# chenxuhao/GraphAIBench

Measured on AMD Instinct MI355X. Metric: GCN-layer fwd+bwd aggregated edges/sec, higher is better.
Workload: dtype f32; 1 GPU; ogbn-products-shaped Chung-Lu graph (seed 42), GCN hidden layer 128->128 fwd+bwd (2 SpMM D=128 + 3 dense products + relu/d_relu; 2 of the products ride on the SpMMs); nv=2449029, ne_with_selfloops=125915443, D=128, parallelism=1 GPU

## Files before the change

graphaibench_amd/build.py:

```python
from __future__ import annotations

import os
import shutil
import subprocess
import sys
from pathlib import Path

ROOT = Path(__file__).resolve().parent.parent
PKG = ROOT / "graphaibench_amd"
CSRC = PKG / "csrc"
HOST = PKG / "host"
LIB = PKG / "lib"
INCLUDE = ROOT / "include"
ORACLE = ROOT / "oracle"
REFERENCE = Path("/root/reference")

HIP_SOURCES = ["runtime.hip", "graph.hip", "spmm.hip", "spmm_part.hip", "spmm_gemm_bf16.hip", "gat.hip", "sgemm.hip", "sgemm_skinny.hip", "elementwise.hip", "probe.hip", "comm.hip"]
HIPCC_FLAGS = [
    "--offload-arch=gfx950",
    "-O3",
    "-std=c++17",
    "-fPIC",
    "-ffp-contract=off",
    "-Wall",
    "-Wno-unused-function",
    "-Werror=pass-failed",
]


def _hipcc() -> str:
    for cand in (os.environ.get("HIPCC"), shutil.which("hipcc"), "/opt/rocm/bin/hipcc"):
        if cand and Path(cand).exists():
            return cand
    raise RuntimeError("hipcc not found (need ROCm at /opt/rocm)")


def _run(cmd, cwd=None):
    print("+", " ".join(str(c) for c in cmd), flush=True)
    subprocess.run([str(c) for c in cmd], cwd=cwd, check=True)


def _stale(target: Path, deps) -> bool:
    if not target.exists():
        return True
    t = target.stat().st_mtime
    return any(Path(d).stat().st_mtime > t for d in deps)


def build_hip(force: bool = False) -> Path:
    LIB.mkdir(exist_ok=True)
    out = LIB / "libgaib_hip.so"
    hipcc = _hipcc()
    headers = [CSRC / "common.h", CSRC / "spmm_core.h", CSRC / "spmm_kernels.h", INCLUDE / "gaib.h"]
    objs, jobs = [], []
    for src in HIP_SOURCES:
        s = CSRC / src
        o = LIB / (src + ".o")
        if force or _stale(o, [s, *headers]):
            jobs.append([hipcc, *HIPCC_FLAGS, f"-I{INCLUDE}", f"-I{CSRC}", "-c", s, "-o", o])
        objs.append(o)
    if jobs:
        from concurrent.futures import ThreadPoolExecutor

        with ThreadPoolExecutor(max_workers=min(4, len(jobs))) as pool:
            list(pool.map(_run, jobs))
    if force or _stale(out, objs):
        _run([hipcc, "--offload-arch=gfx950", "-shared", "-fPIC", *objs, "-o", out])
    return out


def build_host(force: bool = False) -> Path | None:
    srcs = sorted(p for p in HOST.glob("*.cpp") if p.name != "train_main.cpp")
    if not srcs:
        return None
    out = LIB / "libgaib_gnn.so"
    hdrs = list(INCLUDE.rglob("*.h")) + list(INCLUDE.rglob("*.hh"))
    if force or _stale(out, [*srcs, *hdrs, LIB / "libgaib_hip.so"]):
        _run(["g++", "-O2", "-std=c++17", "-fPIC", "-shared", "-fopenmp", "-Wall",
              f"-I{INCLUDE}", f"-I{INCLUDE}/gnn", f"-I{INCLUDE}/layers", f"-I{INCLUDE}/utils",
              *srcs, f"-L{LIB}", "-lgaib_hip", "-Wl,-rpath,$ORIGIN", "-o", out])
    build_drivers(force)
    return out


def build_drivers(force: bool = False) -> None:
    bindir = ROOT / "bin"
    bindir.mkdir(exist_ok=True)
    src = HOST / "train_main.cpp"
    hdrs = list(INCLUDE.rglob("*.h")) + list(INCLUDE.rglob("*.hh"))
    for name, flag in (("gcn", None), ("sage", "-DUSE_SAGE"), ("gat", "-DUSE_GAT")):
        exe = bindir / f"gpu_train_{name}"
        if force or _stale(exe, [src, *hdrs, LIB / "libgaib_gnn.so"]):
            cmd = ["g++", "-O2", "-std=c++17", "-fopenmp", "-Wall", f"-I{INCLUDE}", f"-I{INCLUDE}/gnn",
                   f"-I{INCLUDE}/layers", f"-I{INCLUDE}/utils", src, f"-L{LIB}", "-lgaib_gnn", "-lgaib_hip",
                   "-Wl,-rpath,$ORIGIN/../graphaibench_amd/lib", "-o", exe]
            if flag:
                cmd.insert(1, flag)
            _run(cmd)


# ... 24 lines not shown
```

graphaibench_amd/capi.py:

```python
from __future__ import annotations

import ctypes as C
from pathlib import Path

LIB_DIR = Path(__file__).resolve().parent / "lib"
LIB_PATH = LIB_DIR / "libgaib_hip.so"

W_GCN, W_MEAN, W_MEAN_T, W_EDGE, W_EDGE_T = 0, 1, 2, 3, 4

_vp, _i, _i64, _f, _u64 = C.c_void_p, C.c_int, C.c_int64, C.c_float, C.c_uint64
_pp = C.POINTER(C.c_void_p)

SIGNATURES = {
    "gaib_last_error": (C.c_char_p, []),
    "gaib_version": (C.c_char_p, []),
    "gaib_ctx_create": (_i, [_i, _vp, _pp]),
    "gaib_ctx_destroy": (_i, [_vp]),
    "gaib_ctx_set_stream": (_i, [_vp, _vp]),
    "gaib_ctx_own_stream": (_i, [_vp]),
    "gaib_sync": (_i, [_vp]),
    "gaib_capture_begin": (_i, [_vp]),
    "gaib_capture_end": (_i, [_vp, _pp]),
    "gaib_capture_abort": (_i, [_vp]),
    "gaib_exec_launch": (_i, [_vp, _vp]),
    "gaib_exec_nodes": (_i64, [_vp]),
    "gaib_exec_elapsed_ms": (_i, [_vp, _vp]),
    "gaib_exec_destroy": (_i, [_vp]),
    "gaib_host_alloc": (_i, [_vp, C.c_size_t, _pp]),
    "gaib_host_free": (_i, [_vp, _vp]),
    "gaib_memcpy_d2h_async": (_i, [_vp, _vp, _vp, C.c_size_t]),
    "gaib_masked_avg_loss_dev": (_i, [_vp, _i64, _i64, _vp, _vp, _vp]),
    "gaib_masked_accuracy_single_dev": (_i, [_vp, _i64, _i64, _i, _vp, _vp, _vp, _vp]),
    "gaib_masked_f1_counts_dev": (_i, [_vp, _i64, _i64, _i, _vp, _vp, _vp, _vp]),
    "gaib_adam_step_dev": (_i, [_vp, _i64, _vp, _vp, _vp, _vp, _f, _f, _f, _f, _vp]),
    "gaib_side_begin": (_i, [_vp]),
    "gaib_side_end": (_i, [_vp]),
    "gaib_side_wait": (_i, [_vp]),
    "gaib_malloc": (_i, [_vp, C.c_size_t, _pp]),
    "gaib_free": (_i, [_vp, _vp]),
    "gaib_memcpy_h2d": (_i, [_vp, _vp, _vp, C.c_size_t]),
    "gaib_memcpy_d2h": (_i, [_vp, _vp, _vp, C.c_size_t]),
    "gaib_memcpy_d2d": (_i, [_vp, _vp, _vp, C.c_size_t]),
    "gaib_fill_f32": (_i, [_vp, _i64, _f, _vp]),
    "gaib_scale_f32": (_i, [_vp, _i64, _f, _vp]),
    "gaib_cast_f32_bf16": (_i, [_vp, _i64, _vp, _vp]),
    "gaib_cast_bf16_f32": (_i, [_vp, _i64, _vp, _vp]),
    "gaib_graph_create": (_i, [_vp, _i64, _i64, _vp, _i, _vp, _i, _pp]),
    "gaib_graph_create_rect": (_i, [_vp, _i64, _i64, _i64, _vp, _i, _vp, _i, _pp]),
    "gaib_graph_destroy": (_i, [_vp]),
    "gaib_graph_add_selfloop": (_i, [_vp, _vp, _pp]),
    "gaib_graph_nv": (_i64, [_vp]),
    "gaib_graph_ne": (_i64, [_vp]),
    "gaib_graph_nc": (_i64, [_vp]),
    "gaib_graph_rowptr": (_vp, [_vp]),
    "gaib_graph_colidx": (_vp, [_vp]),
    "gaib_graph_compute_vertex_data": (_i, [_vp, _vp]),
    "gaib_graph_vertex_data": (_vp, [_vp]),
    "gaib_graph_compute_edge_data": (_i, [_vp, _vp]),
    "gaib_graph_edge_data": (_vp, [_vp]),
    "gaib_graph_set_vertex_norm": (_i, [_vp, _vp, _vp, _vp, _vp, _vp]),
    "gaib_graph_device_bytes": (_i64, [_vp]),
    "gaib_spmm": (_i, [_vp, _vp, _i, _vp, _i, _vp, _vp]),
    "gaib_spmm_acc": (_i, [_vp, _vp, _i, _vp, _i, _vp, _vp]),
    "gaib_spmm_ex": (_i, [_vp, _vp, _i, _vp, _i, _vp, _vp, _i]),
    "gaib_spmm_gemm": (_i, [_vp, _vp, _i, _vp, _i, _vp, _vp, _vp, _i, _i, _vp, _i]),
    "gaib_spmm_gemm2": (_i, [_vp, _vp, _i, _vp, _i, _vp, _vp, _vp, _i, _vp, _vp, _i, _vp, _i]),
    "gaib_spmm_mh": (_i, [_vp, _vp, _i, _vp, _i, _i, _vp, _vp, _i]),
    "gaib_spmm_bf16": (_i, [_vp, _vp, _i, _vp, _i, _vp, _vp, _i]),
    "gaib_spmm_gemm_bf16": (_i, [_vp, _vp, _i, _vp, _i, _vp, _vp, _vp, _i, _i, _vp, _i]),
    "gaib_spmm_gemm2_bf16": (_i, [_vp, _vp, _i, _vp, _i, _vp, _vp, _vp, _i, _vp, _vp, _i, _vp, _i]),
    "gaib_graph_split_classes": (_i, [_vp, _vp, _vp, _pp, _pp, _pp, _pp, C.POINTER(_i64), C.POINTER(_i64), _i]),
    "gaib_graph_split_pieces": (_i, [_vp, _vp, _i, _i, C.POINTER(_i64), C.POINTER(_i64), C.POINTER(_i), _pp]),
    "gaib_graph_set_row_map": (_i, [_vp, _vp, _vp, _i64]),
    "gaib_graph_row_map": (_vp, [_vp]),
    "gaib_spmm_2t": (_i, [_vp, _vp, _i, _vp, _i, _vp, _vp, _i64, _vp, _i]),
    "gaib_spmm_gemm_2t": (_i, [_vp, _vp, _i, _vp, _i, _vp, _vp, _i64, _vp, _vp, _i, _vp, _vp, _i, _vp, _i]),
    "gaib_spmm_gemm_fusable": (_i, [_vp, _i, _i, _i, _i]),
    "gaib_gat_scores_mh": (_i, [_vp, _vp, _i, _i, _vp, _vp, _vp, _f, _vp, _vp, _vp]),
    "gaib_sddmm_mh": (_i, [_vp, _vp, _i, _i, _vp, _vp, _vp]),
    "gaib_gat_softmax_bwd_alpha_mh": (_i, [_vp, _vp, _i, _i, _vp, _vp, _vp, _vp, _f, _vp, _vp, _vp]),
    "gaib_gat_softmax_bwd_alpha_ex": (_i, [_vp, _vp, _i, _i, _vp, _vp, _vp, _vp, _f, _vp, _vp, _vp, _vp, _vp, _vp]),
    "gaib_gat_softmax_bwd_alpha_re": (_i, [_vp, _vp, _i, _i, _vp, _vp, _vp, _vp, _vp, _f, _vp, _vp, _vp, _vp, _vp, _vp]),
    "gaib_gat_softmax_bwd_rows": (_i, [_vp, _vp, _i, _vp, _vp, _vp, _f, _vp, _vp]),
    "gaib_edge_gather_perm": (_i, [_vp, _i64, _i, _vp, _vp, _vp]),
    "gaib_edge_rowsum": (_i, [_vp, _vp, _i, _vp, _vp]),
    "gaib_gat_alpha_grads": (_i, [_vp, _i64, _i, _i, _vp, _vp, _vp, _vp, _vp]),
    "gaib_gat_backward_fused": (_i, [_vp, _vp, _i, _i, _vp, _vp, _vp, _vp, _vp, _vp, _vp, _f, _vp, _vp, _vp]),
    "gaib_gat_forward_fused": (_i, [_vp, _vp, _i, _i, _vp, _vp, _vp, _f, _i, _vp, _vp]),
    "gaib_edge_transpose_mh": (_i, [_vp, _vp, _i, _vp, _vp]),
    "gaib_gat_scores": (_i, [_vp, _vp, _i, _vp, _vp, _vp, _f, _vp, _vp, _vp]),
    "gaib_sddmm": (_i, [_vp, _vp, _i, _vp, _vp, _vp]),
    "gaib_gat_softmax_bwd_alpha": (_i, [_vp, _vp, _i, _vp, _vp, _vp, _vp, _f, _vp, _vp, _vp]),
    "gaib_edge_transpose": (_i, [_vp, _vp, _vp, _vp]),
    "gaib_sgemm": (_i, [_vp, _i, _i, _i64, _i64, _i64, _vp, _vp, _i, _vp]),
    "gaib_sgemm_drelu": (_i, [_vp, _i64, _i64, _i64, _vp, _vp, _vp, _i, _vp]),
    "gaib_sgemm_ex": (_i, [_vp, _i, _i, _i64, _i64, _i64, _vp, _vp, _i, _vp]),
    "gaib_bias_add": (_i, [_vp, _i64, _i, _vp, _vp]),
    "gaib_colsum": (_i, [_vp, _i64, _i, _vp, _vp]),
    "gaib_rng_uniform": (_i, [_vp, _i64, _f, _f, _u64, _vp]),
    "gaib_csr2csc": (_i, [_vp, _i, _i, _i, _vp, _vp, _vp, _vp, _vp, _vp]),
    "gaib_relu": (_i, [_vp, _i64, _vp, _vp]),
    "gaib_d_relu": (_i, [_vp, _i64, _vp, _vp, _vp]),
    "gaib_dropout": (_i, [_vp, _i64, _f, _f, _u64, _vp, _vp, _vp]),
    "gaib_d_dropout": (_i, [_vp, _i64, _f, _vp, _vp, _vp]),
    "gaib_softmax_xent": (_i, [_vp, _i, _i64, _i64, _vp, _vp, _vp, _vp, _vp]),
    "gaib_d_softmax_xent": (_i, [_vp, _i, _i64, _i64, _vp, _vp, _vp, _vp]),
    "gaib_sigmoid_xent": (_i, [_vp, _i, _i64, _i64, _vp, _vp, _vp, _vp, _vp]),
    "gaib_d_sigmoid_xent": (_i, [_vp, _i, _i64, _i64, _vp, _vp, _vp, _vp]),
    "gaib_masked_f1_micro": (_i, [_vp, _i64, _i64, _i, _vp, _vp, _vp, C.POINTER(_f), C.POINTER(_i64)]),
    "gaib_masked_avg_loss": (_i, [_vp, _i64, _i64, _vp, _vp, C.POINTER(_f)]),
    "gaib_masked_accuracy_single": (_i, [_vp, _i64, _i64, _i, _vp, _vp, _vp, C.POINTER(_f)]),
    "gaib_l2norm": (_i, [_vp, _i64, _i, _vp, _vp]),
    "gaib_d_l2norm": (_i, [_vp, _i64, _i, _vp, _vp, _vp]),
    "gaib_adam_step": (_i, [_vp, _i64, _vp, _vp, _vp, _vp, _f, _f, _f, _f, _f, _f]),
    "gaib_gather_rows": (_i, [_vp, _i64, _vp, _i, _vp, _vp]),
    "gaib_prof_enable": (_i, [_vp, _i]),
    "gaib_prof_reset": (_i, [_vp]),
    "gaib_prof_get": (_i, [_vp, C.c_char_p, C.POINTER(_i64), C.POINTER(C.c_double)]),
    "gaib_prof_get_work": (_i, [_vp, C.c_char_p, C.POINTER(_i64), C.POINTER(C.c_double), C.POINTER(C.c_double),
                                C.POINTER(C.c_double), C.POINTER(C.c_double)]),
    "gaib_prof_table": (_i, [_vp, C.c_char_p, C.c_size_t, C.POINTER(C.c_size_t)]),
    "gaib_gat_score_signs": (_i, [_vp, _vp, _i, _i, _vp, _vp, _vp, _vp]),
    "gaib_gat_forward_fused_rect": (_i, [_vp, _vp, _i, _i, _vp, _vp, _vp, C.c_float, _i, _vp, _vp, _i]),
    "gaib_gat_backward_rec": (_i, [_vp, _i64, _i, _i, _vp, _vp, _vp, _vp]),
    "gaib_gat_backward_fused_rect": (_i, [_vp, _vp, _i, _i, _vp, _vp, _vp, _vp, _vp, C.c_float, _vp, _vp, _vp, _i]),
    "gaib_gather_scatter_rows": (_i, [_vp, _i64, _vp, _vp, _i, _vp, _vp]),
    "gaib_graph_reorder": (_i, [_vp, _vp, _i, _pp, _vp, _vp]),
    "gaib_graph_sort_rows": (_i, [_vp, _vp]),
    "gaib_graph_locality": (_i, [_vp, _vp, C.POINTER(C.c_float)]),
    "gaib_graph_stats": (_i, [_vp, _vp, C.POINTER(_i64), C.POINTER(_i64), C.POINTER(_i64)]),
    "gaib_set_option": (_i, [_vp, C.c_char_p, _i64]),
    "gaib_get_option": (_i, [_vp, C.c_char_p, C.POINTER(_i64)]),
    "gaib_device_count": (_i, [C.POINTER(_i)]),
    "gaib_comm_transport_available": (_i, [_i]),
    "gaib_comm_unique_id": (_i, [_i, _vp]),
    "gaib_comm_init": (_i, [_vp, _i, _i, _vp, _i, _pp]),
    "gaib_comm_destroy": (_i, [_vp]),
    "gaib_comm_rank": (_i, [_vp]),
    "gaib_comm_size": (_i, [_vp]),
    "gaib_comm_barrier": (_i, [_vp]),
    "gaib_allreduce_f32": (_i, [_vp, _vp, _i64]),
    "gaib_allreduce_host_f64": (_i, [_vp, C.POINTER(C.c_double), _i]),
    "gaib_halo_create": (_i, [_vp, C.POINTER(_i64), _vp, _i, C.POINTER(_i64), _pp]),
    "gaib_halo_destroy": (_i, [_vp]),
    "gaib_halo_rows": (_i64, [_vp]),
    "gaib_halo_send_rows": (_i64, [_vp]),
    "gaib_halo_bytes_sent": (_i64, [_vp]),
    "gaib_halo_send_stats": (_i, [_vp, C.POINTER(_i64), C.POINTER(_i64), C.POINTER(_i)]),
    "gaib_halo_link_rows": (_i64, [_vp]),
    "gaib_halo_exchange_begin": (_i, [_vp, _i, _vp]),
    "gaib_halo_exchange_end": (_i, [_vp, _pp]),
# ... 279 lines not shown
        _check(load().gaib_probe_stream_copy(self.h, nbytes, iters, C.byref(v)), "gaib_probe_stream_copy")
        return v.value

    def graph_stats(self, g: "Graph"):
        a, b, c = _i64(), _i64(), _i64()
        _check(self.lib.gaib_graph_stats(self.h, g.h, C.byref(a), C.byref(b), C.byref(c)), "gaib_graph_stats")
        return dict(n_heavy=a.value, heavy_edges=b.value, max_degree=c.value)

    def graph(self, rowptr, colidx, ncols: int | None = None) -> "Graph":
        return Graph(self, rowptr, colidx, ncols)

    def spmm(self, g: "Graph", kind: int, x, out, edge_w=None, accumulate: bool = False, relu: bool = False,
             heads: int = 1):
        assert x.is_contiguous() and out.is_contiguous() and x.dim() == 2
        flags = (1 if accumulate else 0) | (2 if relu else 0)
        _check(self.lib.gaib_spmm_mh(self.h, g.h, kind, _ptr(edge_w), heads, x.shape[1], _ptr(x), _ptr(out), flags),
               "gaib_spmm")
        return out

    def cast_f32_bf16(self, x, out=None):
        import torch

        assert x.is_contiguous() and x.dtype == torch.float32
        if out is None:
            out = torch.empty(x.shape, dtype=torch.bfloat16, device=x.device)
        assert out.is_contiguous() and out.dtype == torch.bfloat16 and out.numel() == x.numel()
        _check(self.lib.gaib_cast_f32_bf16(self.h, x.numel(), _ptr(x), _ptr(out)), "gaib_cast_f32_bf16")
        return out

    def cast_bf16_f32(self, x, out=None):
        import torch

        assert x.is_contiguous() and x.dtype == torch.bfloat16
        if out is None:
            out = torch.empty(x.shape, dtype=torch.float32, device=x.device)
        assert out.is_contiguous() and out.dtype == torch.float32 and out.numel() == x.numel()
        _check(self.lib.gaib_cast_bf16_f32(self.h, x.numel(), _ptr(x), _ptr(out)), "gaib_cast_bf16_f32")
        return out

    def spmm_bf16(self, g: "Graph", kind: int, x, out, edge_w=None, accumulate: bool = False, relu: bool = False):
        import torch

        assert x.is_contiguous() and out.is_contiguous() and x.dim() == 2 and x.dtype == torch.bfloat16
        flags = (1 if accumulate else 0) | (2 if relu else 0)
        _check(self.lib.gaib_spmm_bf16(self.h, g.h, kind, _ptr(edge_w), x.shape[1], _ptr(x), _ptr(out), flags),
               "gaib_spmm_bf16")
        return out

    def spmm_gemm(self, g: "Graph", kind: int, x, agg, W, out, transW: bool = False, relu: bool = False,
                  agg_scratch: bool = False, edge_w=None, accumulate: bool = False, rows2=None, W2=None):
        assert x.is_contiguous() and agg.is_contiguous() and W.is_contiguous() and out.is_contiguous()
        len_in, len_out = agg.shape[1], out.shape[1]
        assert tuple(W.shape) == ((len_out, len_in) if transW else (len_in, len_out))
        flags = (2 if relu else 0) | (4 if agg_scratch else 0) | (1 if accumulate else 0)
        if rows2 is not None:
            assert rows2.is_contiguous() and W2.is_contiguous() and W2.shape == W.shape and rows2.shape[1] == len_in
            _check(self.lib.gaib_spmm_gemm2(self.h, g.h, kind, _ptr(edge_w), len_in, _ptr(x), _ptr(agg), _ptr(W),
                                            1 if transW else 0, _ptr(rows2), _ptr(W2), len_out, _ptr(out), flags),
                   "gaib_spmm_gemm2")
            return out
        _check(self.lib.gaib_spmm_gemm(self.h, g.h, kind, _ptr(edge_w), len_in, _ptr(x), _ptr(agg), _ptr(W),
                                       1 if transW else 0, len_out, _ptr(out), flags), "gaib_spmm_gemm")
        return out

    def spmm_gemm_bf16(self, g: "Graph", kind: int, x, agg, W, out, transW: bool = False, relu: bool = False,
                       agg_scratch: bool = False, edge_w=None, accumulate: bool = False, rows2=None, W2=None):
        import torch

        assert x.is_contiguous() and agg.is_contiguous() and W.is_contiguous() and out.is_contiguous()
        assert x.dtype == torch.bfloat16 and agg.dtype == torch.float32 and out.dtype == torch.float32
        len_in, len_out = agg.shape[1], out.shape[1]
        assert tuple(W.shape) == ((len_out, len_in) if transW else (len_in, len_out))
        flags = (2 if relu else 0) | (4 if agg_scratch else 0) | (1 if accumulate else 0)
        if rows2 is not None:
            assert rows2.is_contiguous() and W2.is_contiguous() and W2.shape == W.shape and rows2.shape[1] == len_in
            _check(self.lib.gaib_spmm_gemm2_bf16(self.h, g.h, kind, _ptr(edge_w), len_in, _ptr(x), _ptr(agg), _ptr(W),
                                                 1 if transW else 0, _ptr(rows2), _ptr(W2), len_out, _ptr(out), flags),
                   "gaib_spmm_gemm2_bf16")
            return out
        _check(self.lib.gaib_spmm_gemm_bf16(self.h, g.h, kind, _ptr(edge_w), len_in, _ptr(x), _ptr(agg), _ptr(W),
                                            1 if transW else 0, len_out, _ptr(out), flags), "gaib_spmm_gemm_bf16")
        return out

    def spmm_2t(self, g: "Graph", kind: int, x, x2, n_first: int, out, edge_w=None, accumulate: bool = False,
                relu: bool = False):
        assert x.is_contiguous() and out.is_contiguous() and (x2 is None or x2.is_contiguous())
        flags = (1 if accumulate else 0) | (2 if relu else 0)
        _check(self.lib.gaib_spmm_2t(self.h, g.h, kind, _ptr(edge_w), x.shape[1], _ptr(x), _ptr(x2), n_first, _ptr(out),
                                     flags), "gaib_spmm_2t")
        return out

    def spmm_gemm_2t(self, g: "Graph", kind: int, x, x2, n_first: int, agg, W, out, transW: bool = False,
                     relu: bool = False, agg_scratch: bool = False, edge_w=None, accumulate: bool = False, rows2=None,
                     W2=None):
        len_in, len_out = agg.shape[1], out.shape[1]
        flags = (2 if relu else 0) | (4 if agg_scratch else 0) | (1 if accumulate else 0)
        _check(self.lib.gaib_spmm_gemm_2t(self.h, g.h, kind, _ptr(edge_w), len_in, _ptr(x), _ptr(x2), n_first, _ptr(agg),
                                          _ptr(W), 1 if transW else 0, _ptr(rows2), _ptr(W2), len_out, _ptr(out), flags),
               "gaib_spmm_gemm_2t")
        return out

    def spmm_gemm_fusable(self, kind: int, len_in: int, len_out: int, dual: bool = False) -> bool:
        return bool(self.lib.gaib_spmm_gemm_fusable(self.h, kind, len_in, len_out, int(dual)))

    def split_classes(self, g_own: "Graph", g_halo: "Graph", interior=True, bnd_own=True, bnd_halo=True, bnd_full=True,
                      all_boundary: bool = False):
        hs = [C.c_void_p() for _ in range(4)]
        want = [interior, bnd_own, bnd_halo, bnd_full]
        nb, be = _i64(), _i64()
        _check(self.lib.gaib_graph_split_classes(self.h, g_own.h, g_halo.h, *[C.byref(h) if w else None for h, w in zip(hs, want)],
                                                 C.byref(nb), C.byref(be), int(all_boundary)), "gaib_graph_split_classes")
        out = {k: (Graph(self, _handle=h) if w else None)
               for k, h, w in zip(("interior", "bnd_own", "bnd_halo", "bnd_full"), hs, want)}
        out["n_boundary"], out["boundary_edges"] = nb.value, be.value
        return out

    def split_pieces(self, g: "Graph", n_pieces: int, ranges):
        nr = len(ranges)
        b = (C.c_int64 * max(nr, 1))(*[int(r[0]) for r in ranges])
        e = (C.c_int64 * max(nr, 1))(*[int(r[1]) for r in ranges])
        pc = (C.c_int * max(nr, 1))(*[int(r[2]) for r in ranges])
        hs = (C.c_void_p * n_pieces)()
        _check(self.lib.gaib_graph_split_pieces(self.h, g.h, n_pieces, nr, b, e, pc, hs), "gaib_graph_split_pieces")
        return [Graph(self, _handle=C.c_void_p(hs[k])) for k in range(n_pieces)]

    def gat_scores(self, g, h, alpha_l, alpha_r, temp, scores, norm, eps: float = 0.2, heads: int = 1):
        _check(self.lib.gaib_gat_scores_mh(self.h, g.h, h.shape[1], heads, _ptr(h), _ptr(alpha_l), _ptr(alpha_r),
                                           eps, _ptr(temp), _ptr(scores), _ptr(norm)), "gaib_gat_scores")

    def gat_score_signs(self, g, h, alpha_l, alpha_r, heads: int = 1):
        import torch

        out = torch.empty(g.ne, heads, dtype=torch.uint8, device=h.device)
        _check(self.lib.gaib_gat_score_signs(self.h, g.h, h.shape[1], heads, _ptr(h), _ptr(alpha_l), _ptr(alpha_r), _ptr(out)),
               "gaib_gat_score_signs")
        return out

    def sddmm(self, g, grad, feat, out_e, heads: int = 1):
        _check(self.lib.gaib_sddmm_mh(self.h, g.h, grad.shape[1], heads, _ptr(grad), _ptr(feat), _ptr(out_e)),
               "gaib_sddmm")

    def gat_softmax_bwd_alpha(self, g, feat, norm, norm_grad, temp, scores, lgrad, rgrad, eps: float = 0.2,
                              heads: int = 1, grad_rows=None, fwd_out_rows=None, norm_t=None, alpha=None):
        if temp is None:
            _check(self.lib.gaib_gat_softmax_bwd_alpha_re(self.h, g.h, feat.shape[1], heads, _ptr(feat), _ptr(alpha[0]),
                                                          _ptr(alpha[1]), _ptr(norm), _ptr(norm_grad), eps, _ptr(scores),
                                                          _ptr(lgrad), _ptr(rgrad), _ptr(grad_rows),
                                                          _ptr(fwd_out_rows), _ptr(norm_t)), "gaib_gat_softmax_bwd_alpha_re")
            return
        _check(self.lib.gaib_gat_softmax_bwd_alpha_ex(self.h, g.h, feat.shape[1], heads, _ptr(feat), _ptr(norm),
                                                      _ptr(norm_grad), _ptr(temp), eps, _ptr(scores),
                                                      _ptr(lgrad), _ptr(rgrad), _ptr(grad_rows),
                                                      _ptr(fwd_out_rows), _ptr(norm_t)), "gaib_gat_softmax_bwd_alpha")

    def gat_forward_fused(self, g, h, alpha_l, alpha_r, out, row_stats, eps: float = 0.2, heads: int = 1,
                          relu: bool = False) -> bool:
        rc = self.lib.gaib_gat_forward_fused(self.h, g.h, h.shape[1], heads, _ptr(h), _ptr(alpha_l), _ptr(alpha_r), eps,
                                             int(relu), _ptr(out), _ptr(row_stats))
        if rc == -5:
            return False
        _check(rc, "gaib_gat_forward_fused")
        return True

    def gat_backward_fused(self, g, feat, grad, fwd_out, alpha_l, alpha_r, norm, grad_out, lgrad, rgrad, eps: float = 0.2,
                           heads: int = 1, row_stats=None) -> bool:
        rc = self.lib.gaib_gat_backward_fused(self.h, g.h, feat.shape[1], heads, _ptr(feat), _ptr(grad), _ptr(fwd_out),
# ... 247 lines not shown
```

graphaibench_amd/csrc/common.h:

```cpp
#pragma once
#include <hip/hip_runtime.h>
#include <stdint.h>
#include <stdio.h>
#include <string>
#include <string.h>
#include <vector>
#include "gaib.h"

#define GAIB_WAVE 64

void gaib_set_error(const char* fmt, ...);

#define GAIB_HIP(call)                                                                    \
  do {                                                                                    \
    hipError_t e_ = (call);                                                               \
    if (e_ != hipSuccess) {                                                               \
      gaib_set_error("%s:%d: %s -> %s", __FILE__, __LINE__, #call, hipGetErrorString(e_)); \
      return GAIB_ERR_HIP;                                                                \
    }                                                                                     \
  } while (0)

#define GAIB_CHECK(cond, ...)       \
  do {                              \
    if (!(cond)) {                  \
      gaib_set_error(__VA_ARGS__);  \
      return GAIB_ERR_INVALID;      \
    }                               \
  } while (0)

#define GAIB_TRY(call)         \
  do {                         \
    int rc_ = (call);          \
    if (rc_ != GAIB_OK) return rc_; \
  } while (0)

#define GAIB_LAUNCH_CHECK() GAIB_HIP(hipGetLastError())

#define GAIB_NOT_WHILE_CAPTURING(ctx, what)                                                                        \
  GAIB_CHECK(!(ctx)->capturing, "%s inside gaib_capture_begin/end: it waits for the stream or allocates -- run the " \
                                "sequence once before capturing it (buffers and lazily built tables then exist)", what)


#define GAIB_FLAT_RING_DEFAULT 1
#define GAIB_BF16_FUSE_U 32

struct gaib_ctx {
  int device;
  hipStream_t stream;
  int num_cus;
  void* ws;
  size_t ws_bytes;
  void* pad;
  size_t pad_bytes;
  hipStream_t main_stream, side_stream;
  hipEvent_t ev_fork, ev_join;
  void* ws_side;
  size_t ws_side_bytes;
  int forked;
  int spmm_heavy_threshold;
  int spmm_variant;
  int spmm_xcd_swizzle;
  int spmm_chunked;
  int spmm_pad;
  int spmm_fuse;
  int spmm_flat;
  int spmm_flat_ring;
  int comm_reserve_cus;
  int comm_reserve_default;
  int spmm_fuse_cus;
  int spmm_tile_xcd;
  int spmm_prefetch_ids;
  int spmm_unroll;
  int spmm_addr_mode;
  int spmm_gather_mode;
  int spmm_hot_bytes;
  int spmm_bf16_layout;
  int spmm_bf16_fuse_u;
  int agg_bf16;
  int sgemm_variant;
  int gat_fast;
  int gat_chunk_colsum;
  int gat_chunk_sort;
  int gat_row_waves;
  int gat_fused_bwd;
  int gat_fused_fwd;
  int gat_fused_unroll;
  int gat_bwd_pk;
  int gat_interleave;
  int gat_chunk_xcd;
  int graph_rev_search;
  hipStream_t owned_stream;
  int capturing;
  int live_execs;
  std::vector<void*> retired;
  int prof_on;
  struct ProfRec { const char* key; hipEvent_t a, b; double bytes, flops; char tag[28]; };
  std::vector<ProfRec> prof;
};

static inline int gaib_comm_reserve(const gaib_ctx* ctx) {
  const int r = ctx->comm_reserve_cus >= 0 ? ctx->comm_reserve_cus : ctx->comm_reserve_default;
  const int cap = ctx->num_cus > 64 ? ctx->num_cus - 64 : 0;
  return r < 0 ? 0 : (r > cap ? cap : r);
}

constexpr double GAIB_HBM_PEAK_BPS = 8.0e12;
constexpr double GAIB_MFMA_F32_PEAK_FLOPS = 157.3e12;
static inline double gaib_alg_spmm_bytes(double edges, double rows, double cols, double w_bytes_per_edge, double stored,
                                         double elem_bytes = 4.0) {
  return edges * (elem_bytes * cols + 4.0 + w_bytes_per_edge) + stored * rows * 4.0 * cols + (rows + 1.0) * 8.0;
}

struct ProfScope {
  gaib_ctx* c;
  size_t idx;
  ProfScope(gaib_ctx* ctx, const char* key, double bytes = 0.0, double flops = 0.0, int cols = 0, const char* tag = nullptr)
      : c(ctx), idx((size_t)-1) {
    if (!c->prof_on || c->capturing) return;
    gaib_ctx::ProfRec r;
    r.key = key;
    r.bytes = bytes;
    r.flops = flops;
    r.tag[0] = 0;
    if (tag) snprintf(r.tag, sizeof(r.tag), "%s", tag);
    else if (cols > 0) snprintf(r.tag, sizeof(r.tag), "%d", cols);
    if (hipEventCreate(&r.a) != hipSuccess || hipEventCreate(&r.b) != hipSuccess) return;
    (void)hipEventRecord(r.a, c->stream);
    c->prof.push_back(r);
    idx = c->prof.size() - 1;
  }
  ~ProfScope() {
    if (idx != (size_t)-1) (void)hipEventRecord(c->prof[idx].b, c->stream);
  }
};

int gaib_ws_reserve(gaib_ctx* ctx, size_t bytes);
int gaib_pad_reserve(gaib_ctx* ctx, size_t bytes);

struct gaib_graph {
  int device;
  int64_t nv, ne;
  int64_t nc;
  int64_t* rowptr;
  uint32_t* colidx;
  float* vdata;
  float* edata;
  float* inv_deg;
  float* col_vdata;
  float* col_inv_deg;
  float* w_gcn;
  float* w_mean_t;
  uint32_t* rev;
  uint32_t* chunk_row;
  uint32_t* chunk_ebase;
  uint32_t* chunk_start;
  int64_t n_chunks;
  uint32_t* colidx_flagged;
  int64_t hot_threshold;
  int64_t hot_rows;
  uint32_t* heavy_rows;
// ... 66 lines not shown
```

graphaibench_amd/csrc/elementwise.hip:

```cpp
#include "common.h"

namespace {

typedef float f4 __attribute__((ext_vector_type(4)));

inline unsigned stream_grid(int64_t n_items, int block) {
  int64_t b = cdiv64(n_items > 0 ? n_items : 1, block);
  return (unsigned)(b < 2048 ? b : 2048);
}

__global__ void fill_kernel(int64_t n, float v, float* x) {
  const int64_t stride = (int64_t)gridDim.x * blockDim.x;
  for (int64_t i = (int64_t)blockIdx.x * blockDim.x + threadIdx.x; i < n; i += stride) x[i] = v;
}

__global__ void scale_kernel(int64_t n, float a, float* x) {
  const int64_t stride = (int64_t)gridDim.x * blockDim.x;
  for (int64_t i = (int64_t)blockIdx.x * blockDim.x + threadIdx.x; i < n; i += stride) x[i] = a * x[i];
}

__global__ void relu_kernel(int64_t n, const float* in, float* out, int vec_ok) {
  const int64_t stride = (int64_t)gridDim.x * blockDim.x;
  const int64_t tid = (int64_t)blockIdx.x * blockDim.x + threadIdx.x;
  if (vec_ok) {
    const int64_t n4 = n >> 2;
    for (int64_t i = tid; i < n4; i += stride) {
      f4 v = reinterpret_cast<const f4*>(in)[i];
#pragma unroll
      for (int k = 0; k < 4; ++k) v[k] = v[k] > 0.f ? v[k] : 0.f;
      reinterpret_cast<f4*>(out)[i] = v;
    }
    for (int64_t i = (n4 << 2) + tid; i < n; i += stride) out[i] = in[i] > 0.f ? in[i] : 0.f;
  } else {
    for (int64_t i = tid; i < n; i += stride) out[i] = in[i] > 0.f ? in[i] : 0.f;
  }
}

__global__ void d_relu_kernel(int64_t n, const float* in, const float* data, float* out, int vec_ok) {
  const int64_t stride = (int64_t)gridDim.x * blockDim.x;
  const int64_t tid = (int64_t)blockIdx.x * blockDim.x + threadIdx.x;
  if (vec_ok) {
    const int64_t n4 = n >> 2;
    for (int64_t i = tid; i < n4; i += stride) {
      f4 g = reinterpret_cast<const f4*>(in)[i];
      f4 d = reinterpret_cast<const f4*>(data)[i];
#pragma unroll
      for (int k = 0; k < 4; ++k) g[k] = d[k] > 0.f ? g[k] : 0.f;
      reinterpret_cast<f4*>(out)[i] = g;
    }
    for (int64_t i = (n4 << 2) + tid; i < n; i += stride) out[i] = data[i] > 0.f ? in[i] : 0.f;
  } else {
    for (int64_t i = tid; i < n; i += stride) out[i] = data[i] > 0.f ? in[i] : 0.f;
  }
}

__device__ __forceinline__ float u01(uint64_t seed, uint64_t i) {
  uint64_t z = seed + 0x9E3779B97F4A7C15ull * (i + 1);
  z = (z ^ (z >> 30)) * 0xBF58476D1CE4E5B9ull;
  z = (z ^ (z >> 27)) * 0x94D049BB133111EBull;
  z = z ^ (z >> 31);
  return (float)(z >> 40) * (1.0f / 16777216.0f);
}
__global__ void dropout_kernel(int64_t n, float scale, float rate, uint64_t seed, const float* in,
                               uint8_t* masks, float* out) {
  const int64_t stride = (int64_t)gridDim.x * blockDim.x;
  for (int64_t i = (int64_t)blockIdx.x * blockDim.x + threadIdx.x; i < n; i += stride) {
    uint8_t m = u01(seed, (uint64_t)i) > rate ? 1 : 0;
    masks[i] = m;
    out[i] = in[i] * (float)m * scale;
  }
}
__global__ void d_dropout_kernel(int64_t n, float scale, const float* in, const uint8_t* masks,
                                 float* out) {
  const int64_t stride = (int64_t)gridDim.x * blockDim.x;
  for (int64_t i = (int64_t)blockIdx.x * blockDim.x + threadIdx.x; i < n; i += stride)
    out[i] = in[i] * (float)masks[i] * scale;
}

__global__ __launch_bounds__(256) void softmax_xent_kernel(int num_cls, int64_t begin, int64_t end,
                                                           const float* in, const uint8_t* masks,
                                                           const uint8_t* labels, float* loss,
                                                           float* out) {
// ... 329 lines not shown
  a[j] = s;
}
__global__ void rng_uniform_kernel(int64_t n, float a, float range, uint64_t seed, float* r) {
  const int64_t stride = (int64_t)gridDim.x * blockDim.x;
  for (int64_t i = (int64_t)blockIdx.x * blockDim.x + threadIdx.x; i < n; i += stride) r[i] = a + range * u01(seed, (uint64_t)i);
}

__global__ void adam_dev_kernel(int64_t n, const float* dW, float* W, float* m, float* v, float alpha, float b1,
                                float b2, const float* pw, float eps) {
  const float b1_t = pw[0], b2_t = pw[1];
  const int64_t stride = (int64_t)gridDim.x * blockDim.x;
  for (int64_t i = (int64_t)blockIdx.x * blockDim.x + threadIdx.x; i < n; i += stride) {
    const float g = dW[i];
    const float mt = b1 * m[i] + (1.0f - b1) * g;
    const float vt = b2 * v[i] + (1.0f - b2) * g * g;
    m[i] = mt;
    v[i] = vt;
    W[i] -= alpha * (mt / (1.0f - b1_t)) / sqrtf((vt / (1.0f - b2_t)) + eps);
  }
}
__global__ void adam_advance_kernel(float* pw, float b1, float b2) {
  pw[0] *= b1;
  pw[1] *= b2;
}

__device__ __forceinline__ unsigned f32_to_bf16_bits(float f) {
  const unsigned u = __float_as_uint(f);
  if ((u & 0x7fffffffu) > 0x7f800000u) return (u >> 16) | 0x0040u;
  return (u + 0x7fffu + ((u >> 16) & 1u)) >> 16;
}
typedef unsigned u4v __attribute__((ext_vector_type(4)));
__global__ __launch_bounds__(256) void cast_f32_bf16_kernel(int64_t n, const float* __restrict__ in, uint16_t* __restrict__ out,
                                                            int vec) {
  const int64_t n8 = vec ? n / 8 : 0;
  const int64_t stride = (int64_t)gridDim.x * blockDim.x;
  for (int64_t i = (int64_t)blockIdx.x * blockDim.x + threadIdx.x; i <= n8; i += stride) {
    if (i < n8) {
      const f4 a = reinterpret_cast<const f4*>(in)[2 * i], b = reinterpret_cast<const f4*>(in)[2 * i + 1];
      u4v o;
      o[0] = f32_to_bf16_bits(a[0]) | (f32_to_bf16_bits(a[1]) << 16);
      o[1] = f32_to_bf16_bits(a[2]) | (f32_to_bf16_bits(a[3]) << 16);
      o[2] = f32_to_bf16_bits(b[0]) | (f32_to_bf16_bits(b[1]) << 16);
      o[3] = f32_to_bf16_bits(b[2]) | (f32_to_bf16_bits(b[3]) << 16);
      reinterpret_cast<u4v*>(out)[i] = o;
    } else {
      for (int64_t k = 8 * n8; k < n; ++k) out[k] = (uint16_t)f32_to_bf16_bits(in[k]);
    }
  }
}
__global__ __launch_bounds__(256) void cast_f32_bf16_scalar_kernel(int64_t n, const float* __restrict__ in,
                                                                   uint16_t* __restrict__ out) {
  const int64_t stride = (int64_t)gridDim.x * blockDim.x;
  for (int64_t i = (int64_t)blockIdx.x * blockDim.x + threadIdx.x; i < n; i += stride) out[i] = (uint16_t)f32_to_bf16_bits(in[i]);
}
__global__ __launch_bounds__(256) void cast_bf16_f32_scalar_kernel(int64_t n, const uint16_t* __restrict__ in,
                                                                   float* __restrict__ out) {
  const int64_t stride = (int64_t)gridDim.x * blockDim.x;
  for (int64_t i = (int64_t)blockIdx.x * blockDim.x + threadIdx.x; i < n; i += stride) out[i] = __uint_as_float((unsigned)in[i] << 16);
}
__global__ __launch_bounds__(256) void cast_bf16_f32_kernel(int64_t n, const uint16_t* __restrict__ in, float* __restrict__ out,
                                                            int vec) {
  const int64_t n8 = vec ? n / 8 : 0;
  const int64_t stride = (int64_t)gridDim.x * blockDim.x;
  for (int64_t i = (int64_t)blockIdx.x * blockDim.x + threadIdx.x; i <= n8; i += stride) {
    if (i < n8) {
      const u4v w = reinterpret_cast<const u4v*>(in)[i];
      f4 a, b;
      a[0] = __uint_as_float(w[0] << 16);
      a[1] = __uint_as_float(w[0] & 0xffff0000u);
      a[2] = __uint_as_float(w[1] << 16);
      a[3] = __uint_as_float(w[1] & 0xffff0000u);
      b[0] = __uint_as_float(w[2] << 16);
      b[1] = __uint_as_float(w[2] & 0xffff0000u);
      b[2] = __uint_as_float(w[3] << 16);
      b[3] = __uint_as_float(w[3] & 0xffff0000u);
      reinterpret_cast<f4*>(out)[2 * i] = a;
      reinterpret_cast<f4*>(out)[2 * i + 1] = b;
    } else {
      for (int64_t k = 8 * n8; k < n; ++k) out[k] = __uint_as_float((unsigned)in[k] << 16);
    }
  }
}

}

extern "C" int gaib_fill_f32(gaib_ctx* ctx, int64_t n, float value, float* d_x) {
  GAIB_CHECK(ctx && (d_x || n == 0), "gaib_fill_f32: NULL argument");
  if (n <= 0) return GAIB_OK;
  fill_kernel<<<stream_grid(n, 256), 256, 0, ctx->stream>>>(n, value, d_x);
  GAIB_LAUNCH_CHECK();
  return GAIB_OK;
}

extern "C" int gaib_scale_f32(gaib_ctx* ctx, int64_t n, float alpha, float* d_x) {
  GAIB_CHECK(ctx && (d_x || n == 0), "gaib_scale_f32: NULL argument");
  if (n <= 0) return GAIB_OK;
  scale_kernel<<<stream_grid(n, 256), 256, 0, ctx->stream>>>(n, alpha, d_x);
  GAIB_LAUNCH_CHECK();
  return GAIB_OK;
}

extern "C" int gaib_cast_f32_bf16(gaib_ctx* ctx, int64_t n, const float* d_in, uint16_t* d_out) {
  GAIB_CHECK(ctx && ((d_in && d_out) || n == 0), "gaib_cast_f32_bf16: NULL argument");
  GAIB_CHECK(n >= 0, "gaib_cast_f32_bf16: n < 0");
  if (n == 0) return GAIB_OK;
  GAIB_CHECK((const void*)d_in != (const void*)d_out, "gaib_cast_f32_bf16: in and out must not alias");
  const int vec = ((((uintptr_t)d_in | (uintptr_t)d_out) & 15) == 0);
  ProfScope ps(ctx, "cast_f32_bf16", 6.0 * (double)n);
  if (vec) cast_f32_bf16_kernel<<<stream_grid(n / 8 + 1, 256), 256, 0, ctx->stream>>>(n, d_in, d_out, 1);
  else cast_f32_bf16_scalar_kernel<<<stream_grid(n, 256), 256, 0, ctx->stream>>>(n, d_in, d_out);
  GAIB_LAUNCH_CHECK();
  return GAIB_OK;
}

extern "C" int gaib_cast_bf16_f32(gaib_ctx* ctx, int64_t n, const uint16_t* d_in, float* d_out) {
  GAIB_CHECK(ctx && ((d_in && d_out) || n == 0), "gaib_cast_bf16_f32: NULL argument");
  GAIB_CHECK(n >= 0, "gaib_cast_bf16_f32: n < 0");
  if (n == 0) return GAIB_OK;
  GAIB_CHECK((const void*)d_in != (const void*)d_out, "gaib_cast_bf16_f32: in and out must not alias");
  const int vec = ((((uintptr_t)d_in | (uintptr_t)d_out) & 15) == 0);
  ProfScope ps(ctx, "cast_bf16_f32", 6.0 * (double)n);
  if (vec) cast_bf16_f32_kernel<<<stream_grid(n / 8 + 1, 256), 256, 0, ctx->stream>>>(n, d_in, d_out, 1);
  else cast_bf16_f32_scalar_kernel<<<stream_grid(n, 256), 256, 0, ctx->stream>>>(n, d_in, d_out);
  GAIB_LAUNCH_CHECK();
  return GAIB_OK;
}

extern "C" int gaib_relu(gaib_ctx* ctx, int64_t n, const float* d_in, float* d_out) {
  GAIB_CHECK(ctx && ((d_in && d_out) || n == 0), "gaib_relu: NULL argument");
  if (n <= 0) return GAIB_OK;
  const int vec_ok = ((((uintptr_t)d_in | (uintptr_t)d_out) & 15) == 0);
  ProfScope ps(ctx, "relu", 8.0 * (double)n);
  relu_kernel<<<stream_grid(n / 4 + 1, 256), 256, 0, ctx->stream>>>(n, d_in, d_out, vec_ok);
  GAIB_LAUNCH_CHECK();
  return GAIB_OK;
}

extern "C" int gaib_d_relu(gaib_ctx* ctx, int64_t n, const float* d_in_diff, const float* d_data,
                           float* d_out_diff) {
  GAIB_CHECK(ctx && ((d_in_diff && d_data && d_out_diff) || n == 0), "gaib_d_relu: NULL argument");
  if (n <= 0) return GAIB_OK;
  const int vec_ok = ((((uintptr_t)d_in_diff | (uintptr_t)d_data | (uintptr_t)d_out_diff) & 15) == 0);
  ProfScope ps(ctx, "d_relu", 12.0 * (double)n);
  d_relu_kernel<<<stream_grid(n / 4 + 1, 256), 256, 0, ctx->stream>>>(n, d_in_diff, d_data,
                                                                     d_out_diff, vec_ok);
  GAIB_LAUNCH_CHECK();
  return GAIB_OK;
}

extern "C" int gaib_dropout(gaib_ctx* ctx, int64_t n, float scale, float drop_rate, uint64_t seed,
                            const float* d_in, uint8_t* d_masks, float* d_out) {
  GAIB_CHECK(ctx && ((d_in && d_masks && d_out) || n == 0), "gaib_dropout: NULL argument");
  GAIB_CHECK(drop_rate >= 0.f && drop_rate < 1.f, "gaib_dropout: rate must be in [0,1)");
  if (n <= 0) return GAIB_OK;
  dropout_kernel<<<stream_grid(n, 256), 256, 0, ctx->stream>>>(n, scale, drop_rate, seed, d_in,
                                                               d_masks, d_out);
  GAIB_LAUNCH_CHECK();
  return GAIB_OK;
}

extern "C" int gaib_d_dropout(gaib_ctx* ctx, int64_t n, float scale, const float* d_in,
                              const uint8_t* d_masks, float* d_out) {
  GAIB_CHECK(ctx && ((d_in && d_masks && d_out) || n == 0), "gaib_d_dropout: NULL argument");
  if (n <= 0) return GAIB_OK;
  d_dropout_kernel<<<stream_grid(n, 256), 256, 0, ctx->stream>>>(n, scale, d_in, d_masks, d_out);
  GAIB_LAUNCH_CHECK();
  return GAIB_OK;
}

extern "C" int gaib_softmax_xent(gaib_ctx* ctx, int num_cls, int64_t begin, int64_t end,
                                 const float* d_in, const uint8_t* d_masks, const uint8_t* d_labels,
                                 float* d_loss, float* d_out) {
  GAIB_CHECK(ctx && d_in && d_labels && d_loss && d_out, "gaib_softmax_xent: NULL argument");
  GAIB_CHECK(num_cls > 0 && begin >= 0 && end >= begin, "gaib_softmax_xent: bad range");
  if (end == begin) return GAIB_OK;
  softmax_xent_kernel<<<(unsigned)cdiv64(end - begin, 4), 256, 0, ctx->stream>>>(
      num_cls, begin, end, d_in, d_masks, d_labels, d_loss, d_out);
  GAIB_LAUNCH_CHECK();
  return GAIB_OK;
}

extern "C" int gaib_d_softmax_xent(gaib_ctx* ctx, int num_cls, int64_t begin, int64_t end,
                                   const uint8_t* d_masks, const uint8_t* d_labels,
                                   const float* d_out, float* d_diff) {
  GAIB_CHECK(ctx && d_labels && d_out && d_diff, "gaib_d_softmax_xent: NULL argument");
  GAIB_CHECK(num_cls > 0 && begin >= 0 && end >= begin, "gaib_d_softmax_xent: bad range");
  if (end == begin) return GAIB_OK;
  d_softmax_xent_kernel<<<stream_grid((end - begin) * num_cls, 256), 256, 0, ctx->stream>>>(
      num_cls, begin, end, d_masks, d_labels, d_out, d_diff);
  GAIB_LAUNCH_CHECK();
  return GAIB_OK;
}

extern "C" int gaib_sigmoid_xent(gaib_ctx* ctx, int num_cls, int64_t begin, int64_t end,
                                 const float* d_in, const uint8_t* d_masks, const uint8_t* d_labels,
                                 float* d_loss, float* d_out) {
  GAIB_CHECK(ctx && d_in && d_labels && d_loss && d_out, "gaib_sigmoid_xent: NULL argument");
  GAIB_CHECK(num_cls > 0 && begin >= 0 && end >= begin, "gaib_sigmoid_xent: bad range");
  if (end == begin) return GAIB_OK;
  sigmoid_xent_kernel<<<(unsigned)cdiv64(end - begin, 4), 256, 0, ctx->stream>>>(
      num_cls, begin, end, d_in, d_masks, d_labels, d_loss, d_out);
  GAIB_LAUNCH_CHECK();
  return GAIB_OK;
}

extern "C" int gaib_d_sigmoid_xent(gaib_ctx* ctx, int num_cls, int64_t begin, int64_t end,
// ... 247 lines not shown
```

graphaibench_amd/csrc/runtime.hip:

```cpp
#include <algorithm>
#include <stdarg.h>
#include <string.h>
#include <utility>
#include "common.h"
#include <stdlib.h>

static thread_local char g_err[1024] = "";

void gaib_set_error(const char* fmt, ...) {
  va_list ap;
  va_start(ap, fmt);
  vsnprintf(g_err, sizeof(g_err), fmt, ap);
  va_end(ap);
}

extern "C" const char* gaib_last_error(void) { return g_err; }
extern "C" const char* gaib_version(void) { return "graphaibench_amd 0.1 (gfx950)"; }

extern "C" int gaib_device_count(int* h_count) {
  GAIB_CHECK(h_count, "gaib_device_count: h_count is NULL");
  *h_count = 0;
  GAIB_HIP(hipGetDeviceCount(h_count));
  return GAIB_OK;
}

extern "C" int gaib_ctx_create(int device, void* stream, gaib_ctx** out) {
  GAIB_CHECK(out != nullptr, "gaib_ctx_create: out is NULL");
  int ndev = 0;
  GAIB_HIP(hipGetDeviceCount(&ndev));
  GAIB_CHECK(device >= 0 && device < ndev, "gaib_ctx_create: device %d out of range (%d)", device, ndev);
  GAIB_HIP(hipSetDevice(device));
  hipDeviceProp_t prop;
  GAIB_HIP(hipGetDeviceProperties(&prop, device));
  gaib_ctx* c = new gaib_ctx();
  c->device = device;
  c->stream = (hipStream_t)stream;
  c->num_cus = prop.multiProcessorCount;
  c->ws = nullptr;
  c->ws_bytes = 0;
  c->pad = nullptr;
  c->pad_bytes = 0;
  c->main_stream = c->stream;
  c->side_stream = nullptr;
  c->ev_fork = c->ev_join = nullptr;
  c->ws_side = nullptr;
  c->ws_side_bytes = 0;
  c->forked = 0;
  c->spmm_heavy_threshold = 1024;
  c->spmm_variant = 0;
  c->spmm_xcd_swizzle = 2;
  c->spmm_unroll = 0;
  c->spmm_tile_xcd = -1;
  c->spmm_prefetch_ids = 1;
  c->spmm_fuse_cus = 0;
  c->spmm_fuse = 1;
  c->spmm_pad = 1;
  c->spmm_chunked = -1;
  c->spmm_flat = -1;
  c->spmm_addr_mode = 0;
  c->spmm_gather_mode = 0;
  c->spmm_hot_bytes = 3 << 20;
  c->spmm_bf16_layout = 0;
  c->spmm_bf16_fuse_u = 0;
  c->agg_bf16 = 0;
  c->sgemm_variant = 0;
  if (const char* e = getenv("GAIB_SGEMM_VARIANT")) c->sgemm_variant = atoi(e);
  c->gat_fast = 1;
  c->gat_row_waves = 4;
  c->gat_chunk_sort = 1;
  c->gat_chunk_colsum = -1;
  c->graph_rev_search = 0;
  c->gat_fused_bwd = -1;
  c->gat_fused_fwd = -1;
  c->gat_fused_unroll = 4;
  c->spmm_flat_ring = GAIB_FLAT_RING_DEFAULT;
  c->comm_reserve_cus = -1;
  c->comm_reserve_default = 0;
  c->gat_interleave = 0;
  c->gat_bwd_pk = 0;
  c->gat_chunk_xcd = 0;
  c->prof_on = 0;
  c->capturing = 0;
  c->live_execs = 0;
  c->owned_stream = nullptr;
  *out = c;
  return GAIB_OK;
}

extern "C" int gaib_ctx_destroy(gaib_ctx* ctx) {
  if (!ctx) return GAIB_OK;
  GAIB_CHECK(ctx->live_execs == 0, "gaib_ctx_destroy: %d recorded sequence(s) of this context are still alive "
                                   "(gaib_exec_destroy them first: they hold its scratch pointers)", ctx->live_execs);
  (void)hipSetDevice(ctx->device);
  if (ctx->ws) (void)hipFree(ctx->ws);
  if (ctx->pad) (void)hipFree(ctx->pad);
  if (ctx->ws_side) (void)hipFree(ctx->ws_side);
  for (void* p : ctx->retired) (void)hipFree(p);
  if (ctx->side_stream) (void)hipStreamDestroy(ctx->side_stream);
  if (ctx->owned_stream) (void)hipStreamDestroy(ctx->owned_stream);
  if (ctx->ev_fork) (void)hipEventDestroy(ctx->ev_fork);
  if (ctx->ev_join) (void)hipEventDestroy(ctx->ev_join);
  delete ctx;
  return GAIB_OK;
}

extern "C" int gaib_ctx_set_stream(gaib_ctx* ctx, void* stream) {
  GAIB_CHECK(ctx, "gaib_ctx_set_stream: ctx is NULL");
  GAIB_CHECK(!ctx->forked, "gaib_ctx_set_stream: a side section is open");
  ctx->stream = (hipStream_t)stream;
  ctx->main_stream = ctx->stream;
  return GAIB_OK;
}

extern "C" int gaib_ctx_own_stream(gaib_ctx* ctx) {
  GAIB_CHECK(ctx, "gaib_ctx_own_stream: ctx is NULL");
  GAIB_CHECK(!ctx->forked && !ctx->capturing, "gaib_ctx_own_stream: a side section or capture is open");
  if (ctx->owned_stream && ctx->stream == ctx->owned_stream) return GAIB_OK;
  GAIB_HIP(hipSetDevice(ctx->device));
  GAIB_HIP(hipStreamSynchronize(ctx->stream));
  if (!ctx->owned_stream) GAIB_HIP(hipStreamCreateWithFlags(&ctx->owned_stream, hipStreamNonBlocking));
  ctx->stream = ctx->main_stream = ctx->owned_stream;
  return GAIB_OK;
}

extern "C" int gaib_side_begin(gaib_ctx* ctx) {
  GAIB_CHECK(ctx, "gaib_side_begin: ctx is NULL");
  GAIB_CHECK(ctx->forked == 0, "gaib_side_begin: a side section is already open or not waited for");
  GAIB_HIP(hipSetDevice(ctx->device));
  if (!ctx->side_stream) {
    GAIB_HIP(hipStreamCreateWithFlags(&ctx->side_stream, hipStreamNonBlocking));
    GAIB_HIP(hipEventCreateWithFlags(&ctx->ev_fork, hipEventDisableTiming));
    GAIB_HIP(hipEventCreateWithFlags(&ctx->ev_join, hipEventDisableTiming));
  }
  GAIB_HIP(hipEventRecord(ctx->ev_fork, ctx->main_stream));
  GAIB_HIP(hipStreamWaitEvent(ctx->side_stream, ctx->ev_fork, 0));
  ctx->stream = ctx->side_stream;
  std::swap(ctx->ws, ctx->ws_side);
  std::swap(ctx->ws_bytes, ctx->ws_side_bytes);
  ctx->forked = 1;
  return GAIB_OK;
}

extern "C" int gaib_side_end(gaib_ctx* ctx) {
  GAIB_CHECK(ctx, "gaib_side_end: ctx is NULL");
  GAIB_CHECK(ctx->forked == 1, "gaib_side_end: no open side section");
  GAIB_HIP(hipEventRecord(ctx->ev_join, ctx->side_stream));
  ctx->stream = ctx->main_stream;
// ... 268 lines not shown
  int64_t n = 0;
  double ms = 0.0;
  for (auto& r : ctx->prof) {
    if (strcmp(r.key, key) != 0) continue;
    float t = 0.f;
    GAIB_HIP(hipEventElapsedTime(&t, r.a, r.b));
    ms += t;
    n++;
  }
  *h_count = n;
  *h_total_ms = ms;
  return GAIB_OK;
}

extern "C" int gaib_prof_get_work(gaib_ctx* ctx, const char* key, int64_t* h_count, double* h_total_ms, double* h_bytes,
                                  double* h_flops, double* h_roof_ms) {
  GAIB_CHECK(ctx && key && h_count && h_total_ms && h_bytes && h_flops && h_roof_ms, "gaib_prof_get_work: NULL argument");
  GAIB_HIP(hipStreamSynchronize(ctx->stream));
  int64_t n = 0;
  double ms = 0.0, by = 0.0, fl = 0.0, roof = 0.0;
  for (auto& r : ctx->prof) {
    if (strcmp(r.key, key) != 0) continue;
    float t = 0.f;
    GAIB_HIP(hipEventElapsedTime(&t, r.a, r.b));
    ms += t;
    by += r.bytes;
    fl += r.flops;
    roof += 1e3 * std::max(r.bytes / GAIB_HBM_PEAK_BPS, r.flops / GAIB_MFMA_F32_PEAK_FLOPS);
    n++;
  }
  *h_count = n;
  *h_total_ms = ms;
  *h_bytes = by;
  *h_flops = fl;
  *h_roof_ms = roof;
  return GAIB_OK;
}

extern "C" int gaib_prof_table(gaib_ctx* ctx, char* h_buf, size_t cap, size_t* h_needed) {
  GAIB_CHECK(ctx && h_needed && (h_buf || cap == 0), "gaib_prof_table: NULL argument");
  GAIB_HIP(hipStreamSynchronize(ctx->stream));
  struct Row { const char* key; const char* tag; int64_t n; double ms, by, fl, roof; };
  std::vector<Row> rows;
  for (auto& r : ctx->prof) {
    Row* at = nullptr;
    for (auto& q : rows)
      if (strcmp(q.tag, r.tag) == 0 && strcmp(q.key, r.key) == 0) at = &q;
    if (!at) {
      rows.push_back(Row{r.key, r.tag, 0, 0, 0, 0, 0});
      at = &rows.back();
    }
    float t = 0.f;
    GAIB_HIP(hipEventElapsedTime(&t, r.a, r.b));
    at->n++;
    at->ms += t;
    at->by += r.bytes;
    at->fl += r.flops;
    at->roof += 1e3 * std::max(r.bytes / GAIB_HBM_PEAK_BPS, r.flops / GAIB_MFMA_F32_PEAK_FLOPS);
  }
  std::string out;
  char line[320];
  for (auto& q : rows) {
    if (q.tag[0]) snprintf(line, sizeof(line), "%s@%s %lld %.6f %.0f %.0f %.9f\n", q.key, q.tag, (long long)q.n, q.ms, q.by, q.fl, q.roof);
    else snprintf(line, sizeof(line), "%s %lld %.6f %.0f %.0f %.9f\n", q.key, (long long)q.n, q.ms, q.by, q.fl, q.roof);
    out += line;
  }
  *h_needed = out.size() + 1;
  if (cap > 0) {
    const size_t w = out.size() < cap - 1 ? out.size() : cap - 1;
    memcpy(h_buf, out.data(), w);
    h_buf[w] = 0;
  }
  return GAIB_OK;
}

extern "C" int gaib_get_option(gaib_ctx* ctx, const char* key, int64_t* h_value) {
  GAIB_CHECK(ctx && key && h_value, "gaib_get_option: NULL argument");
  if (!strcmp(key, "comm_reserve_cus")) *h_value = gaib_comm_reserve(ctx);
  else if (!strcmp(key, "comm_reserve_cus_raw")) *h_value = ctx->comm_reserve_cus;
  else if (!strcmp(key, "spmm_fuse_cus")) *h_value = ctx->spmm_fuse_cus;
  else if (!strcmp(key, "spmm_flat_ring")) *h_value = ctx->spmm_flat_ring;
  else if (!strcmp(key, "num_cus")) *h_value = ctx->num_cus;
  else if (!strcmp(key, "agg_bf16")) *h_value = ctx->agg_bf16;
  else if (!strcmp(key, "spmm_bf16_layout")) *h_value = ctx->spmm_bf16_layout;
  else if (!strcmp(key, "spmm_bf16_fuse_u")) *h_value = ctx->spmm_bf16_fuse_u;
  else {
    gaib_set_error("gaib_get_option: no readable option '%s'", key);
    return GAIB_ERR_INVALID;
  }
  return GAIB_OK;
}

extern "C" int gaib_set_option(gaib_ctx* ctx, const char* key, int64_t value) {
  GAIB_CHECK(ctx && key, "gaib_set_option: NULL argument");
  if (!strcmp(key, "spmm_heavy_threshold")) {
    GAIB_CHECK(value >= 1 && value <= (1 << 30), "spmm_heavy_threshold out of range");
    ctx->spmm_heavy_threshold = (int)value;
  } else if (!strcmp(key, "spmm_variant"))
    ctx->spmm_variant = (int)value;
  else if (!strcmp(key, "spmm_xcd_swizzle"))
    ctx->spmm_xcd_swizzle = (int)value;
  else if (!strcmp(key, "spmm_fuse"))
    ctx->spmm_fuse = (int)value;
  else if (!strcmp(key, "spmm_chunked"))
    ctx->spmm_chunked = (int)value;
  else if (!strcmp(key, "spmm_pad"))
    ctx->spmm_pad = (int)value;
  else if (!strcmp(key, "spmm_flat"))
    ctx->spmm_flat = (int)value;
  else if (!strcmp(key, "spmm_fuse_cus")) {
    GAIB_CHECK(value >= 0 && value <= ctx->num_cus, "spmm_fuse_cus: 0 (all) .. %d", ctx->num_cus);
    ctx->spmm_fuse_cus = (int)value;
  } else if (!strcmp(key, "spmm_tile_xcd"))
    ctx->spmm_tile_xcd = (int)value;
  else if (!strcmp(key, "spmm_prefetch_ids"))
    ctx->spmm_prefetch_ids = value != 0;
  else if (!strcmp(key, "spmm_unroll"))
    ctx->spmm_unroll = (int)value;
  else if (!strcmp(key, "spmm_addr_mode"))
    ctx->spmm_addr_mode = (int)value;
  else if (!strcmp(key, "spmm_gather_mode"))
    ctx->spmm_gather_mode = (int)value;
  else if (!strcmp(key, "spmm_hot_bytes"))
    ctx->spmm_hot_bytes = (int)value;
  else if (!strcmp(key, "spmm_bf16_layout")) {
    GAIB_CHECK(value == 0 || value == 4 || value == 8, "spmm_bf16_layout must be 0, 4 or 8");
    ctx->spmm_bf16_layout = (int)value;
  } else if (!strcmp(key, "spmm_bf16_fuse_u")) {
    GAIB_CHECK(value == 0 || value == 16 || value == 32, "spmm_bf16_fuse_u must be 0 (default), 16 or 32");
    ctx->spmm_bf16_fuse_u = (int)value;
  } else if (!strcmp(key, "agg_bf16")) {
    GAIB_CHECK(value == 0 || value == 1, "agg_bf16 must be 0 (fp32 tables) or 1 (bf16 tables)");
    ctx->agg_bf16 = (int)value;
  }
  else if (!strcmp(key, "sgemm_variant"))
    ctx->sgemm_variant = (int)value;
  else if (!strcmp(key, "gat_fast"))
    ctx->gat_fast = (int)value;
  else if (!strcmp(key, "gat_chunk_colsum"))
    ctx->gat_chunk_colsum = (int)value;
  else if (!strcmp(key, "gat_chunk_sort"))
    ctx->gat_chunk_sort = (int)value;
  else if (!strcmp(key, "gat_fused_fwd"))
    ctx->gat_fused_fwd = (int)value;
  else if (!strcmp(key, "gat_fused_unroll"))
    ctx->gat_fused_unroll = (int)value;
  else if (!strcmp(key, "comm_reserve_cus"))
    ctx->comm_reserve_cus = value < 0 ? -1 : (int)std::min<int64_t>(value, std::max(0, ctx->num_cus - 64));
  else if (!strcmp(key, "spmm_flat_ring"))
    ctx->spmm_flat_ring = value < 0 ? GAIB_FLAT_RING_DEFAULT : (int)value;
  else if (!strcmp(key, "gat_interleave"))
    ctx->gat_interleave = (int)value;
  else if (!strcmp(key, "gat_bwd_pk"))
    ctx->gat_bwd_pk = (int)value;
  else if (!strcmp(key, "gat_chunk_xcd"))
    ctx->gat_chunk_xcd = (int)value;
  else if (!strcmp(key, "gat_fused_bwd"))
    ctx->gat_fused_bwd = (int)value;
  else if (!strcmp(key, "graph_rev_search"))
    ctx->graph_rev_search = (int)value;
  else if (!strcmp(key, "gat_row_waves")) {
    GAIB_CHECK(value == 1 || value == 2 || value == 4, "gat_row_waves must be 1, 2 or 4");
    ctx->gat_row_waves = (int)value;
  }
  else {
    gaib_set_error("gaib_set_option: unknown key '%s'", key);
    return GAIB_ERR_INVALID;
  }
  return GAIB_OK;
}
```

graphaibench_amd/csrc/spmm.hip:

```cpp
#include <algorithm>
#include "spmm_kernels.h"

namespace {

template <int G, int WMODE, int HT = 0, typename E = float>
__global__ __launch_bounds__(256) void spmm_chunk_kernel(int64_t n_chunks, const uint32_t* chunk_row,
                                                         const uint32_t* chunk_ebase, const uint32_t* chunk_start,
                                                         SpmmArgs a, float* partial) {
  constexpr int U = G < 8 ? G : 8;
  constexpr bool MH = WMODE >= 3;
  constexpr int WS = HT + 1;
  __shared__ float wlds[HT > 0 ? 4 * 64 * WS : 1];
  const int64_t c = (int64_t)blockIdx.x * 4 + (threadIdx.x >> 6);
  if (c >= n_chunks) return;
  const int lane = threadIdx.x & 63;
  const int sl = lane & (G - 1), gbase = lane & ~(G - 1);
  const int64_t row = chunk_row[c];
  const int64_t eb = chunk_ebase[c];
  const int64_t rb = a.rowptr[row];
  const int64_t rem = a.rowptr[row + 1] - eb;
  const int n = rem < 64 ? (int)rem : 64;
  const uint32_t cl = a.col[eb + (lane < n ? lane : 0)];
  float wl = 0.f;
  if (lane < n) {
// ... 174 lines not shown
  a.row_list = nullptr;
  a.row_order = nullptr;
  a.nblocks = 0;
  a.per_xcd = 0;
  a.xcd_chunk = 0;
  a.accumulate = (flags & GAIB_ACCUMULATE) ? 1 : 0;
  a.relu = (flags & GAIB_RELU) ? 1 : 0;
  a.heads = heads;
  a.dh = heads > 0 ? len / heads : len;
  a.col_flagged = nullptr;
  a.compact = 0;
  a.row_map = g->row_map;
  a.in2 = d_in2;
  a.n_first = d_in2 ? (uint32_t)n_first : 0xffffffffu;
  a.in2_bytes = 0;
  if (!part && !bf16 && ctx->spmm_gather_mode == 3 && g->nc == g->nv && !g->col_vdata) {
    GAIB_TRY(gaib_graph_ensure_hot_flags(ctx, g, len));
    a.col_flagged = g->colidx_flagged;
  }
  a.ldo = len;
  {
    const int64_t lp_pad = bf16 ? 0 : pad_stride_floats(ctx, g, len, part);
    if (lp_pad > 0) {
      const int lp = (int)lp_pad;
      GAIB_TRY(gaib_pad_reserve(ctx, (size_t)g->nc * (size_t)lp * 4));
      const int64_t n4 = g->nc * (int64_t)(lp / 4);
      const unsigned grid = (unsigned)std::min<int64_t>(cdiv64(n4, 256), (int64_t)ctx->num_cus * 16);
      pad_rows_kernel<<<grid, 256, 0, ctx->stream>>>(n4, len, lp / 4, d_in, reinterpret_cast<f32x4_t*>(ctx->pad));
      GAIB_LAUNCH_CHECK();
      a.in = reinterpret_cast<const float*>(ctx->pad);
      a.ld = lp;
    }
  }
  const int64_t table_bytes = (d_in2 ? n_first : g->nc) * a.ld * (bf16 ? 2 : 4);
  a.in_bytes = table_bytes < ((int64_t)1 << 32) ? (uint32_t)table_bytes : 0u;
  if (d_in2) {
    const int64_t t2 = (g->nc - n_first) * a.ld * 4;
    a.in2_bytes = t2 < ((int64_t)1 << 32) ? (uint32_t)t2 : 0u;
  }
  switch (weight_kind) {
    case GAIB_W_GCN:
      GAIB_TRY(gaib_graph_ensure_w_gcn(ctx, g));
      a.ew = g->w_gcn;
      *wmode = 1;
      return GAIB_OK;
    case GAIB_W_MEAN:
      GAIB_TRY(gaib_graph_ensure_inv_deg(ctx, g));
      a.rw = g->inv_deg;
      *wmode = 0;
      return GAIB_OK;
    case GAIB_W_MEAN_T:
      GAIB_TRY(gaib_graph_ensure_w_mean_t(ctx, g));
      a.ew = g->w_mean_t;
      *wmode = 1;
      return GAIB_OK;
    case GAIB_W_EDGE:
      GAIB_CHECK(d_edge_w || g->ne == 0, "gaib_spmm: GAIB_W_EDGE needs d_edge_w");
      a.ew = d_edge_w;
      *wmode = heads > 1 ? 3 : 1;
      return GAIB_OK;
    case GAIB_W_EDGE_T:
      GAIB_CHECK(d_edge_w || g->ne == 0, "gaib_spmm: GAIB_W_EDGE_T needs d_edge_w");
      GAIB_TRY(gaib_graph_ensure_rev(ctx, g));
      a.ew = d_edge_w;
      a.rev = g->rev;
      *wmode = heads > 1 ? 4 : 2;
      return GAIB_OK;
    default:
      gaib_set_error("gaib_spmm: unknown weight_kind %d", weight_kind);
      return GAIB_ERR_INVALID;
  }
}

static bool chunk_rule(gaib_ctx* ctx, gaib_graph* g, int64_t ld) {
  if (gaib_graph_ensure_heavy(ctx, g, ctx->spmm_heavy_threshold) != GAIB_OK) return false;
  return g->nc * ld * 4 <= ((int64_t)512 << 20) && 4 * g->heavy_edges >= g->ne && g->ne > 0;
}

int gaib_spmm_part_plain(gaib_ctx* ctx, const gaib_graph* g, const void* spmm_args, int wmode, int len);
int gaib_spmm_part_fused(gaib_ctx* ctx, const gaib_graph* g, const void* spmm_args, const void* fuse_args, float* heavy_scratch,
                         int vec, int wmode);
int gaib_spmm_fused_bf16(gaib_ctx* ctx, const gaib_graph* g, const void* spmm_args, const void* fuse_args, float* heavy_scratch,
                         int vec, int wmode);

static int spmm_impl(gaib_ctx* ctx, gaib_graph* g, int weight_kind, const float* d_edge_w, int len,
                     const float* d_in, float* d_out, int flags, int heads = 1, const float* d_in2 = nullptr,
                     int64_t n_first = 0) {
  GAIB_CHECK(ctx && g, "gaib_spmm: NULL ctx/graph");
  GAIB_CHECK(len >= 0, "gaib_spmm: len < 0");
  GAIB_CHECK(ctx->device == g->device, "gaib_spmm: graph lives on device %d, ctx on %d", g->device,
             ctx->device);
  if (len == 0 || g->nv == 0) return GAIB_OK;
  GAIB_CHECK(d_in && d_out, "gaib_spmm: NULL feature pointer");
  GAIB_CHECK(d_in != d_out, "gaib_spmm: in and out must not alias");
  SpmmArgs a;
  int wmode = 0;
  GAIB_TRY(spmm_setup(ctx, g, weight_kind, d_edge_w, len, d_in, d_out, flags, heads, &a, &wmode, d_in2, n_first));
  if (g->row_map || d_in2) {
    GAIB_CHECK(d_in2 != d_out, "gaib_spmm: in2 and out must not alias");
    GAIB_CHECK(heads == 1 && wmode <= 1, "gaib_spmm: a row class of a partition aggregates with GAIB_W_GCN / _MEAN / _MEAN_T / "
                                          "single-head _EDGE weights (got kind %d, %d heads)", weight_kind, heads);
    return gaib_spmm_part_plain(ctx, g, &a, wmode, len);
  }
  const bool chunk_shape = len % 4 == 0 && len <= 256 && a.ld % 4 == 0 && a.ldo % 4 == 0 && g->ne > 0 &&
                           ((((uintptr_t)a.in | (uintptr_t)a.out) & 15) == 0) && (wmode < 3 || a.dh % 4 == 0);
  const bool chunk_auto = ctx->spmm_chunked < 0 && chunk_rule(ctx, g, a.ld);
  if (chunk_shape && (ctx->spmm_chunked == 1 || (ctx->spmm_chunked < 0 && chunk_auto))) {
    switch (wmode) {
      case 0: return launch_chunked<0>(ctx, g, a);
      case 1: return launch_chunked<1>(ctx, g, a);
      case 2: return launch_chunked<2>(ctx, g, a);
      case 3: return launch_chunked<3>(ctx, g, a);
      default: return launch_chunked<4>(ctx, g, a);
    }
  }
  switch (wmode) {
    case 0: return dispatch_vec<0>(ctx, g, a, len);
    case 1: return dispatch_vec<1>(ctx, g, a, len);
    case 2: return dispatch_vec<2>(ctx, g, a, len);
    case 3: return dispatch_vec<3>(ctx, g, a, len);
    default: return dispatch_vec<4>(ctx, g, a, len);
  }
}

extern "C" int gaib_spmm(gaib_ctx* ctx, gaib_graph* g, int weight_kind, const float* d_edge_w,
                         int len, const float* d_in, float* d_out) {
  return spmm_impl(ctx, g, weight_kind, d_edge_w, len, d_in, d_out, 0);
}

extern "C" int gaib_spmm_acc(gaib_ctx* ctx, gaib_graph* g, int weight_kind, const float* d_edge_w,
                             int len, const float* d_in, float* d_out) {
  return spmm_impl(ctx, g, weight_kind, d_edge_w, len, d_in, d_out, GAIB_ACCUMULATE);
}

extern "C" int gaib_spmm_ex(gaib_ctx* ctx, gaib_graph* g, int weight_kind, const float* d_edge_w,
                            int len, const float* d_in, float* d_out, int flags) {
  return spmm_impl(ctx, g, weight_kind, d_edge_w, len, d_in, d_out, flags);
}

extern "C" int gaib_spmm_2t(gaib_ctx* ctx, gaib_graph* g, int weight_kind, const float* d_edge_w, int len,
                            const float* d_in, const float* d_in2, int64_t n_first, float* d_out, int flags) {
  GAIB_CHECK(ctx && g, "gaib_spmm_2t: NULL ctx/graph");
  GAIB_CHECK(d_in2 || n_first >= g->nc || g->nv == 0 || g->ne == 0, "gaib_spmm_2t: NULL second table with columns beyond n_first");
  return spmm_impl(ctx, g, weight_kind, d_edge_w, len, d_in, d_out, flags, 1, d_in2, n_first);
}

static bool fuse_shape_ok(gaib_ctx* ctx, int weight_kind, int len_in, int len_out, bool dual) {
  if (!ctx->spmm_fuse || len_in < 1 || len_in > 128 || len_out < 1) return false;
  if (len_in > 64 && len_in % 2 != 0) return false;
  if (!(weight_kind == GAIB_W_GCN || weight_kind == GAIB_W_MEAN || weight_kind == GAIB_W_MEAN_T || weight_kind == GAIB_W_EDGE))
    return false;
  return fuse_strip_rows(len_in <= 64 ? 64 : 128, len_out, dual) != 0;
}

extern "C" int gaib_spmm_gemm_fusable(gaib_ctx* ctx, int weight_kind, int len_in, int len_out, int dual) {
  return ctx && fuse_shape_ok(ctx, weight_kind, len_in, len_out, dual != 0) ? 1 : 0;
}

static int spmm_gemm_impl(gaib_ctx* ctx, gaib_graph* g, int weight_kind, const float* d_edge_w, int len_in,
                          const float* d_in, float* d_agg, const float* d_W, int transW, const float* d_rows2,
                          const float* d_W2, int len_out, float* d_out, int flags, const float* d_in2 = nullptr,
                          int64_t n_first = 0, bool bf16 = false) {
  GAIB_CHECK(ctx && g, "gaib_spmm_gemm: NULL ctx/graph");
  GAIB_CHECK(len_in >= 0 && len_out >= 0, "gaib_spmm_gemm: negative length");
  GAIB_CHECK(ctx->device == g->device, "gaib_spmm_gemm: graph lives on device %d, ctx on %d", g->device,
             ctx->device);
  GAIB_CHECK((flags & ~(GAIB_RELU | GAIB_AGG_SCRATCH | GAIB_ACCUMULATE | GAIB_OVERLAPS_TRANSFER)) == 0,
             "gaib_spmm_gemm: unsupported flags %d", flags);
  GAIB_CHECK((d_rows2 == nullptr) == (d_W2 == nullptr), "gaib_spmm_gemm2: rows2 and W2 go together");
  if (g->nv == 0 || len_out == 0) return GAIB_OK;
  GAIB_CHECK(d_in && d_agg && d_W && d_out, "gaib_spmm_gemm: NULL pointer");
  GAIB_CHECK(d_in != d_agg && d_agg != d_out && d_in != d_out && d_rows2 != d_out && d_rows2 != d_agg,
             "gaib_spmm_gemm: buffers must not alias");
  const bool dual = d_rows2 != nullptr;
  const bool part = g->row_map != nullptr || d_in2 != nullptr;
  const uintptr_t al = (bf16 ? (uintptr_t)d_in << 1 : (uintptr_t)d_in) | (uintptr_t)d_agg | (uintptr_t)d_in2;
  const int kpad = len_in <= 64 ? 64 : 128;
  const bool lanes_ok = len_in <= 64 ? true : (len_in % 2 == 0 && (al & 7) == 0);
  const bool dense = !part && ctx->spmm_chunked != 0 && len_in % 4 == 0 && (al & 15) == 0 &&
                     (ctx->spmm_chunked == 1 || chunk_rule(ctx, g, len_in));
  const bool shape_ok = ctx->spmm_fuse != 0 && !dense && len_in >= 1 && len_in <= 128 && lanes_ok && (g->ne > 0 || part) &&
                        g->nv >= 1 &&
                        (weight_kind == GAIB_W_GCN || weight_kind == GAIB_W_MEAN ||
                         weight_kind == GAIB_W_MEAN_T || weight_kind == GAIB_W_EDGE);
  if (!part && shape_ok && dual && fuse_strip_rows(kpad, len_out, true) == 0 && fuse_strip_rows(kpad, len_out, false) != 0) {
    GAIB_TRY(spmm_gemm_impl(ctx, g, weight_kind, d_edge_w, len_in, d_in, d_agg, d_W, transW, nullptr, nullptr, len_out, d_out,
                            flags & ~GAIB_RELU, nullptr, 0, bf16));
    return gaib_sgemm_ex(ctx, 0, transW, g->nv, len_out, len_in, d_rows2, d_W2,
                         GAIB_ACCUMULATE | ((flags & GAIB_RELU) ? GAIB_RELU : 0), d_out);
  }
  const bool fusable = shape_ok && fuse_strip_rows(kpad, len_out, dual) != 0;
  if (part) {
    if (!fusable) {
      gaib_set_error("gaib_spmm_gemm: a row class of a partition needs a fusable shape (len_in %d, len_out %d%s): aggregate "
                     "with gaib_spmm_ex / gaib_spmm_2t and multiply all rows at once", len_in, len_out, dual ? ", two products" : "");
      return GAIB_ERR_UNSUPPORTED;
    }
  }
  const bool kslab = !part && ctx->spmm_fuse != 0 && !dense && len_in > 128 && len_in <= 256 && len_in % 2 == 0 && (al & 7) == 0 &&
                     len_out >= 1 && fuse_strip_rows(128, len_out, false) != 0 && g->ne > 0 &&
                     (weight_kind == GAIB_W_GCN || weight_kind == GAIB_W_MEAN || weight_kind == GAIB_W_MEAN_T ||
                      weight_kind == GAIB_W_EDGE);
  if (kslab) {
    SpmmArgs a0;
    int wmode = 0;
    GAIB_TRY(spmm_setup(ctx, g, weight_kind, d_edge_w, len_in, d_in, d_agg, 0, 1, &a0, &wmode, nullptr, 0, bf16));
    const size_t wt_bytes = (sizeof(float) * (size_t)len_out * len_in + 255) & ~(size_t)255;
    const size_t hv_bytes = (sizeof(float) * (size_t)g->n_heavy * len_in + 255) & ~(size_t)255;
    GAIB_TRY(gaib_ws_reserve(ctx, wt_bytes + hv_bytes + 256));
    float* wt = (float*)ctx->ws;
    float* hv = (float*)((char*)ctx->ws + wt_bytes);
    int* counter = (int*)((char*)hv + hv_bytes);
    const float* wk = d_W;
    if (!transW) {
      const int n = len_in * len_out;
      transpose_small_kernel<<<(n + 255) / 256, 256, 0, ctx->stream>>>(len_in, len_out, d_W, wt);
      GAIB_LAUNCH_CHECK();
      wk = wt;
    }
    for (int k0 = 0; k0 < len_in; k0 += 128) {
      SpmmArgs a = a0;
      a.in = bf16 ? reinterpret_cast<const float*>(reinterpret_cast<const uint16_t*>(a0.in) + k0) : a0.in + k0;
      a.ncols = len_in - k0 < 128 ? len_in - k0 : 128;
      a.accumulate = 0;
      a.out = (flags & GAIB_AGG_SCRATCH) ? nullptr : d_agg + k0;
      if (a.in_bytes) a.in_bytes -= (uint32_t)(k0 * (bf16 ? 2 : 4));
      FuseArgs f;
      f.wt = wk + k0;
      f.wt2 = nullptr;
      f.rows2 = nullptr;
      f.ldw = len_in;
      f.y = d_out;
      f.ldy = len_out;
      f.n_out = len_out;
      f.tile_counter = counter;
      f.agg_in = (flags & GAIB_ACCUMULATE) ? d_agg + k0 : nullptr;
      f.y_accum = k0 > 0;
      f.overlaps_transfer = (flags & GAIB_OVERLAPS_TRANSFER) ? 1 : 0;
      f.tile_xcd = tile_xcd_arg(ctx, g);
      f.relu = ((flags & GAIB_RELU) && !dual && k0 + 128 >= len_in) ? 1 : 0;
      f.heavy_agg = hv + k0;
      f.heavy_rows = g->heavy_rows;
      f.n_heavy = (int)g->n_heavy;
      if (bf16) GAIB_TRY(gaib_spmm_fused_bf16(ctx, g, &a, &f, hv + k0, 2, wmode));
      else GAIB_TRY(wmode == 0 ? (launch_fused<2, 0>(ctx, g, a, f, hv + k0)) : (launch_fused<2, 1>(ctx, g, a, f, hv + k0)));
    }
    if (dual)
      return gaib_sgemm_ex(ctx, 0, transW, g->nv, len_out, len_in, d_rows2, d_W2,
                           GAIB_ACCUMULATE | ((flags & GAIB_RELU) ? GAIB_RELU : 0), d_out);
    return GAIB_OK;
  }
  if (!fusable) {
    const int act = (flags & GAIB_RELU) ? GAIB_RELU : 0;
    if (bf16) GAIB_TRY(gaib_spmm_bf16(ctx, g, weight_kind, d_edge_w, len_in, reinterpret_cast<const uint16_t*>(d_in), d_agg, flags & GAIB_ACCUMULATE));
    else GAIB_TRY(spmm_impl(ctx, g, weight_kind, d_edge_w, len_in, d_in, d_agg, flags & GAIB_ACCUMULATE));
    GAIB_TRY(gaib_sgemm_ex(ctx, 0, transW, g->nv, len_out, len_in, d_agg, d_W, dual ? 0 : act, d_out));
    if (dual) return gaib_sgemm_ex(ctx, 0, transW, g->nv, len_out, len_in, d_rows2, d_W2, GAIB_ACCUMULATE | act, d_out);
    return GAIB_OK;
  }
  SpmmArgs a;
  int wmode = 0;
  GAIB_TRY(spmm_setup(ctx, g, weight_kind, d_edge_w, len_in, d_in, d_agg, 0, 1, &a, &wmode, d_in2, n_first, bf16));
  a.accumulate = 0;
  if (flags & GAIB_AGG_SCRATCH) a.out = nullptr;
  const size_t wt_bytes = (sizeof(float) * (size_t)len_out * len_in + 255) & ~(size_t)255;
  const size_t hv_bytes = (sizeof(float) * (size_t)g->n_heavy * len_in + 255) & ~(size_t)255;
  GAIB_TRY(gaib_ws_reserve(ctx, 2 * wt_bytes + hv_bytes + 256));
  float* wt = (float*)ctx->ws;
  float* wt2 = (float*)((char*)ctx->ws + wt_bytes);
  float* hv = (float*)((char*)ctx->ws + 2 * wt_bytes);
  int* counter = (int*)((char*)hv + hv_bytes);
  FuseArgs f;
  f.wt = d_W;
  f.wt2 = d_W2;
  if (!transW) {
    const int n = len_in * len_out;
    transpose_small_kernel<<<(n + 255) / 256, 256, 0, ctx->stream>>>(len_in, len_out, d_W, wt);
    GAIB_LAUNCH_CHECK();
    f.wt = wt;
    if (dual) {
      transpose_small_kernel<<<(n + 255) / 256, 256, 0, ctx->stream>>>(len_in, len_out, d_W2, wt2);
      GAIB_LAUNCH_CHECK();
      f.wt2 = wt2;
    }
  }
  f.rows2 = d_rows2;
  f.ldw = len_in;
  f.y_accum = 0;
  f.overlaps_transfer = (flags & GAIB_OVERLAPS_TRANSFER) ? 1 : 0;
  f.tile_xcd = tile_xcd_arg(ctx, g);
  f.y = d_out;
  f.ldy = len_out;
  f.n_out = len_out;
  f.tile_counter = counter;
  f.agg_in = (flags & GAIB_ACCUMULATE) ? d_agg : nullptr;
  f.relu = (flags & GAIB_RELU) ? 1 : 0;
  f.heavy_agg = hv;
  f.heavy_rows = g->heavy_rows;
  f.n_heavy = (int)g->n_heavy;
  if (part) return gaib_spmm_part_fused(ctx, g, &a, &f, hv, len_in <= 64 ? 1 : 2, wmode);
  if (bf16) return gaib_spmm_fused_bf16(ctx, g, &a, &f, hv, len_in <= 64 ? 1 : 2, wmode);
  if (len_in <= 64) {
    return wmode == 0 ? launch_fused<1, 0>(ctx, g, a, f, hv) : launch_fused<1, 1>(ctx, g, a, f, hv);
  }
  return wmode == 0 ? launch_fused<2, 0>(ctx, g, a, f, hv) : launch_fused<2, 1>(ctx, g, a, f, hv);
}

extern "C" int gaib_spmm_gemm(gaib_ctx* ctx, gaib_graph* g, int weight_kind, const float* d_edge_w,
                              int len_in, const float* d_in, float* d_agg, const float* d_W, int transW,
                              int len_out, float* d_out, int flags) {
  return spmm_gemm_impl(ctx, g, weight_kind, d_edge_w, len_in, d_in, d_agg, d_W, transW, nullptr, nullptr, len_out,
                        d_out, flags);
}

extern "C" int gaib_spmm_gemm2(gaib_ctx* ctx, gaib_graph* g, int weight_kind, const float* d_edge_w,
                               int len_in, const float* d_in, float* d_agg, const float* d_W, int transW,
                               const float* d_rows2, const float* d_W2, int len_out, float* d_out, int flags) {
  GAIB_CHECK(d_rows2 && d_W2, "gaib_spmm_gemm2: NULL second operand");
  return spmm_gemm_impl(ctx, g, weight_kind, d_edge_w, len_in, d_in, d_agg, d_W, transW, d_rows2, d_W2, len_out,
                        d_out, flags);
}

extern "C" int gaib_spmm_gemm_2t(gaib_ctx* ctx, gaib_graph* g, int weight_kind, const float* d_edge_w, int len_in,
                                 const float* d_in, const float* d_in2, int64_t n_first, float* d_agg, const float* d_W,
                                 int transW, const float* d_rows2, const float* d_W2, int len_out, float* d_out, int flags) {
  GAIB_CHECK(ctx && g, "gaib_spmm_gemm_2t: NULL ctx/graph");
  GAIB_CHECK(d_in2 || n_first >= g->nc || g->nv == 0 || g->ne == 0, "gaib_spmm_gemm_2t: NULL second table with columns beyond n_first");
  GAIB_CHECK(!d_in2 || (d_in2 != d_agg && d_in2 != d_out), "gaib_spmm_gemm_2t: buffers must not alias");
  return spmm_gemm_impl(ctx, g, weight_kind, d_edge_w, len_in, d_in, d_agg, d_W, transW, d_rows2, d_W2, len_out, d_out, flags,
                        d_in2, n_first);
}

extern "C" int gaib_spmm_mh(gaib_ctx* ctx, gaib_graph* g, int weight_kind, const float* d_edge_w,
                            int heads, int len, const float* d_in, float* d_out, int flags) {
  GAIB_CHECK(heads >= 1 && len % heads == 0, "gaib_spmm_mh: heads (%d) must divide len (%d)", heads, len);
  GAIB_CHECK(heads == 1 || weight_kind == GAIB_W_EDGE || weight_kind == GAIB_W_EDGE_T,
             "gaib_spmm_mh: per-head weights need GAIB_W_EDGE or GAIB_W_EDGE_T");
  return spmm_impl(ctx, g, weight_kind, d_edge_w, len, d_in, d_out, flags, heads);
}

namespace {

template <int WMODE>
int dispatch_bf16(gaib_ctx* ctx, gaib_graph* g, const SpmmArgs& a0, int len) {
  typedef uint16_t bf16_t;
  const uintptr_t ai = (uintptr_t)a0.in, ao = (uintptr_t)a0.out;
  int vmax = 1;
  for (int v = 8; v > 1; v >>= 1)
    if (len % v == 0 && (ai & (2 * v - 1)) == 0 && (ao & ((v >= 4 ? 16 : 4 * v) - 1)) == 0) {
      vmax = v;
      break;
    }
  const int layout = ctx->spmm_bf16_layout;
  if ((layout == 4 || layout == 8) && vmax >= layout && (len + layout - 1) / layout <= 32) {
    const int lanes = (len + layout - 1) / layout;
    if (layout == 8) {
      if (lanes <= 1) return launch_sub<8, 1, WMODE, bf16_t>(ctx, g, a0);
      if (lanes <= 2) return launch_sub<8, 2, WMODE, bf16_t>(ctx, g, a0);
      if (lanes <= 4) return launch_sub<8, 4, WMODE, bf16_t>(ctx, g, a0);
      if (lanes <= 8) return launch_sub<8, 8, WMODE, bf16_t>(ctx, g, a0);
      if (lanes <= 16) return launch_sub<8, 16, WMODE, bf16_t>(ctx, g, a0);
      return launch_sub<8, 32, WMODE, bf16_t>(ctx, g, a0);
    }
    if (lanes <= 1) return launch_sub<4, 1, WMODE, bf16_t>(ctx, g, a0);
    if (lanes <= 2) return launch_sub<4, 2, WMODE, bf16_t>(ctx, g, a0);
    if (lanes <= 4) return launch_sub<4, 4, WMODE, bf16_t>(ctx, g, a0);
    if (lanes <= 8) return launch_sub<4, 8, WMODE, bf16_t>(ctx, g, a0);
    if (lanes <= 16) return launch_sub<4, 16, WMODE, bf16_t>(ctx, g, a0);
    return launch_sub<4, 32, WMODE, bf16_t>(ctx, g, a0);
  }
  int vec = vmax;
  for (int v = 1; v < vmax; v <<= 1)
    if ((len + v - 1) / v <= 64) {
      vec = v;
      break;
    }
  const int slab = vec >= 4 ? 512 : 256 * vec;
  for (int c0 = 0; c0 < len; c0 += slab) {
    SpmmArgs a = a0;
    a.in = reinterpret_cast<const float*>(reinterpret_cast<const bf16_t*>(a0.in) + c0);
    a.out = a0.out + c0;
    if (a.in_bytes) a.in_bytes -= (uint32_t)(2 * c0);
    a.ncols = (len - c0 < slab) ? (len - c0) : slab;
    const int lanes = (a.ncols + vec - 1) / vec;
    const int ct = lanes <= 64 ? 1 : (lanes <= 128 ? 2 : 4);
    int rc;
    if (vec == 8) rc = launch_w64<8, 1, WMODE, bf16_t>(ctx, g, a);
    else if (vec == 4) rc = ct == 1 ? launch_w64<4, 1, WMODE, bf16_t>(ctx, g, a) : launch_w64<4, 2, WMODE, bf16_t>(ctx, g, a);
    else if (vec == 2) rc = ct == 1 ? launch_w64<2, 1, WMODE, bf16_t>(ctx, g, a)
                                    : (ct == 2 ? launch_w64<2, 2, WMODE, bf16_t>(ctx, g, a) : launch_w64<2, 4, WMODE, bf16_t>(ctx, g, a));
    else rc = ct == 1 ? launch_w64<1, 1, WMODE, bf16_t>(ctx, g, a)
                      : (ct == 2 ? launch_w64<1, 2, WMODE, bf16_t>(ctx, g, a) : launch_w64<1, 4, WMODE, bf16_t>(ctx, g, a));
    if (rc != GAIB_OK) return rc;
  }
  return GAIB_OK;
}

}

extern "C" int gaib_spmm_bf16(gaib_ctx* ctx, gaib_graph* g, int weight_kind, const float* d_edge_w, int len,
                              const uint16_t* d_in, float* d_out, int flags) {
  GAIB_CHECK(ctx && g, "gaib_spmm_bf16: NULL ctx/graph");
  GAIB_CHECK(len >= 0, "gaib_spmm_bf16: len < 0");
// ... 59 lines not shown
```

graphaibench_amd/csrc/spmm_core.h:

```cpp
#pragma once
#include <type_traits>
#include "common.h"

namespace {

struct SpmmArgs {
  const int64_t* rowptr;
  const uint32_t* col;
  const float* rw;
  const float* ew;
  const uint32_t* rev;
  const float* in;
  float* out;
  int64_t ld;
  int64_t ldo;
  int ncols;
  int n_rows;
  int heavy_thr;
  const uint32_t* row_list;
  const uint32_t* row_order;
  int nblocks;
  int per_xcd;
  int xcd_chunk;
  uint32_t in_bytes;
// ... 24 lines not shown
template <int VEC>
__device__ __forceinline__ typename VecT<VEC>::type vzero() {
  typename VecT<VEC>::type z;
  if constexpr (VEC == 1) z = 0.f;
  else
    for (int i = 0; i < VEC; ++i) z[i] = 0.f;
  return z;
}
template <int VEC>
__device__ __forceinline__ typename VecT<VEC>::type vrelu(typename VecT<VEC>::type v) {
  if constexpr (VEC == 1) return v > 0.f ? v : 0.f;
  else {
#pragma unroll
    for (int i = 0; i < VEC; ++i) v[i] = v[i] > 0.f ? v[i] : 0.f;
    return v;
  }
}
template <int VEC>
__device__ __forceinline__ void vacc(typename VecT<VEC>::type& acc, float w,
                                     const typename VecT<VEC>::type& x) {
  if constexpr (VEC == 1) {
    float t = w * x;
    acc = acc + t;
  } else {
#pragma unroll
    for (int i = 0; i < VEC; ++i) {
      float t = w * x[i];
      acc[i] = acc[i] + t;
    }
  }
}

__device__ __forceinline__ int logical_block(const SpmmArgs& a) {
  int b = blockIdx.x;
  if (a.per_xcd > 0) {
    const int x = b & 7, k = b >> 3;
    if (a.xcd_chunk > 0) b = ((k / a.xcd_chunk) * 8 + x) * a.xcd_chunk + (k % a.xcd_chunk);
    else b = x * a.per_xcd + k;
  }
  return b;
}

template <int WMODE>
__device__ __forceinline__ float load_edge_w(const SpmmArgs& a, int64_t e, int head = 0) {
  if constexpr (WMODE == 1) return a.ew[e];
  else if constexpr (WMODE == 2) return a.ew[a.rev[e]];
  else if constexpr (WMODE == 3) return a.ew[e * a.heads + head];
  else if constexpr (WMODE == 4) return a.ew[(int64_t)a.rev[e] * a.heads + head];
  else return 0.f;
}

typedef unsigned u2_t __attribute__((ext_vector_type(2)));
typedef unsigned u4_t __attribute__((ext_vector_type(4)));

__device__ __forceinline__ float bf16_lo(unsigned w) { return __uint_as_float(w << 16); }
__device__ __forceinline__ float bf16_hi(unsigned w) { return __uint_as_float(w & 0xffff0000u); }
template <int VEC> struct Bf16Raw;
template <> struct Bf16Raw<1> { typedef unsigned short type; };
template <> struct Bf16Raw<2> { typedef unsigned type; };
template <> struct Bf16Raw<4> { typedef u2_t type; };
template <> struct Bf16Raw<8> { typedef u4_t type; };
template <int VEC>
__device__ __forceinline__ typename VecT<VEC>::type widen_bf16(typename Bf16Raw<VEC>::type r) {
  typename VecT<VEC>::type v;
  if constexpr (VEC == 1) v = __uint_as_float((unsigned)r << 16);
  else if constexpr (VEC == 2) {
    v[0] = bf16_lo(r);
    v[1] = bf16_hi(r);
  } else {
#pragma unroll
    for (int i = 0; i < VEC / 2; ++i) {
      v[2 * i] = bf16_lo(r[i]);
      v[2 * i + 1] = bf16_hi(r[i]);
    }
  }
  return v;
}
template <int VEC, typename E>
__device__ __forceinline__ typename VecT<VEC>::type load_elems(const char* p) {
  if constexpr (sizeof(E) == 4) return *reinterpret_cast<const typename VecT<VEC>::type*>(p);
  else return widen_bf16<VEC>(*reinterpret_cast<const typename Bf16Raw<VEC>::type*>(p));
}

template <int VEC, int GM, bool PART = false, typename E = float>
struct RowGather {
  static constexpr bool BUF = GM != 0;
  static_assert(!PART || sizeof(E) == 4, "two-table gathers: fp32 tables only");
  __amdgpu_buffer_rsrc_t rsrc, rsrc2;
  const char *inb, *inb2;
  int64_t ldb;
  uint32_t n_first;
  __device__ __forceinline__ RowGather(const SpmmArgs& a) {
    inb = reinterpret_cast<const char*>(a.in);
    ldb = a.ld * (int64_t)sizeof(E);
    if constexpr (BUF) rsrc = __builtin_amdgcn_make_buffer_rsrc((void*)a.in, 0, (int)a.in_bytes, 0x00020000);
    if constexpr (PART) {
      n_first = a.in2 ? a.n_first : 0xffffffffu;
      inb2 = reinterpret_cast<const char*>(a.in2) - (int64_t)a.n_first * ldb;
      if constexpr (BUF) rsrc2 = __builtin_amdgcn_make_buffer_rsrc((void*)a.in2, 0, (int)a.in2_bytes, 0x00020000);
    }
  }
  typedef typename std::conditional<sizeof(E) == 2, typename Bf16Raw<VEC>::type, typename VecT<VEC>::type>::type raw_t;
  static __device__ __forceinline__ typename VecT<VEC>::type widen(const raw_t& r) {
    if constexpr (sizeof(E) == 2) return widen_bf16<VEC>(r);
    else return r;
  }
  __device__ __forceinline__ typename VecT<VEC>::type load(uint32_t cj, uint32_t voff) const { return widen(load_raw(cj, voff)); }
  __device__ __forceinline__ raw_t load_raw(uint32_t cj, uint32_t voff) const {
    typedef typename VecT<VEC>::type vec_t;
    if constexpr (PART) {
      static_assert(GM == 0 || GM == 1, "two-table gathers: plain buffer or global loads");
      const bool second = cj >= n_first;
      if constexpr (GM == 1) {
        const int soff = (int)((second ? cj - n_first : cj) * (uint32_t)ldb);
        return load_rsrc<0>(second ? rsrc2 : rsrc, soff, voff);
      } else {
        const char* rowp = (second ? inb2 : inb) + (int64_t)cj * ldb;
        return *reinterpret_cast<const vec_t*>(rowp + voff);
      }
    } else if constexpr (GM == 3) {
      const uint32_t c = cj & 0x7fffffffu;
      if (cj & 0x80000000u) return load_buf<2>(c, voff);
      return load_buf<0>(c, voff);
    } else if constexpr (GM == 2) {
      return load_buf<2>(cj, voff);
    } else if constexpr (GM == 1) {
      return load_buf<0>(cj, voff);
    } else {
      const char* rowp = inb + (int64_t)cj * ldb;
      if constexpr (sizeof(E) == 2) return *reinterpret_cast<const raw_t*>(rowp + voff);
      else return *reinterpret_cast<const vec_t*>(rowp + voff);
    }
  }
  template <int AUX>
  __device__ __forceinline__ raw_t load_buf(uint32_t cj, uint32_t voff) const {
    return load_rsrc<AUX>(rsrc, (int)(cj * (uint32_t)ldb), voff);
  }
  template <int AUX>
  __device__ __forceinline__ raw_t load_rsrc(__amdgpu_buffer_rsrc_t rsrc, int soff, uint32_t voff) const {
    typedef typename VecT<VEC>::type vec_t;
    if constexpr (sizeof(E) == 2) {
      if constexpr (VEC == 1) return __builtin_amdgcn_raw_buffer_load_b16(rsrc, (int)voff, soff, AUX);
      else if constexpr (VEC == 2) return __builtin_amdgcn_raw_buffer_load_b32(rsrc, (int)voff, soff, AUX);
      else if constexpr (VEC == 4) return __builtin_amdgcn_raw_buffer_load_b64(rsrc, (int)voff, soff, AUX);
      else return __builtin_amdgcn_raw_buffer_load_b128(rsrc, (int)voff, soff, AUX);
    } else if constexpr (VEC == 1) {
      return __uint_as_float(__builtin_amdgcn_raw_buffer_load_b32(rsrc, (int)voff, soff, AUX));
    } else if constexpr (VEC == 2) {
      u2_t r = __builtin_amdgcn_raw_buffer_load_b64(rsrc, (int)voff, soff, AUX);
      vec_t v;
      v[0] = __uint_as_float(r[0]);
      v[1] = __uint_as_float(r[1]);
      return v;
    } else {
      u4_t r = __builtin_amdgcn_raw_buffer_load_b128(rsrc, (int)voff, soff, AUX);
      vec_t v;
#pragma unroll
      for (int i = 0; i < 4; ++i) v[i] = __uint_as_float(r[i]);
      return v;
    }
  }
};

template <int VEC, int CT, int WMODE, int U, int BUF, bool PART = false, bool PRE = false, typename E = float>
__device__ __forceinline__ void wave_accumulate(const SpmmArgs& a, int lane, int64_t eb, int64_t ee,
                                                int64_t chunk_stride, float roww,
                                                const uint32_t (&voff)[CT],
                                                typename VecT<VEC>::type (&acc)[CT], uint32_t c_first = 0u,
                                                float w_first = 0.f) {
  static_assert(sizeof(E) == 4 || WMODE < 3, "bf16 tables: single-head weights");
  typedef RowGather<VEC, BUF, PART, E> gather_t;
  const gather_t gather(a);
  typename gather_t::raw_t x[U][CT];
  constexpr bool MH = WMODE >= 3;
  int hd[CT];
  float wv[MH ? U : 1][CT];
#pragma unroll
  for (int ct = 0; ct < CT; ++ct) hd[ct] = MH ? (int)((voff[ct] >> 2) / (uint32_t)a.dh) : 0;
  for (int64_t base = eb; base < ee; base += chunk_stride) {
    const int64_t rem = ee - base;
    const int n = rem < 64 ? (int)rem : 64;
    uint32_t c = 0;
    float w = 0.f;
    if (PRE && base == eb) {
      c = c_first;
      w = w_first;
    } else if (lane < n) {
      c = a.col[base + lane];
      if constexpr (WMODE == 1 || WMODE == 2) w = load_edge_w<WMODE>(a, base + lane);
    }
    int j = 0;
    for (; j + U <= n; j += U) {
#pragma unroll
      for (int u = 0; u < U; ++u) {
        const uint32_t cj = (uint32_t)__builtin_amdgcn_readlane((int)c, j + u);
#pragma unroll
        for (int ct = 0; ct < CT; ++ct) {
          x[u][ct] = gather.load_raw(cj, voff[ct]);
          if constexpr (MH) wv[u][ct] = load_edge_w<WMODE>(a, base + j + u, hd[ct]);
        }
      }
      __builtin_amdgcn_sched_barrier(0);
#pragma unroll
      for (int u = 0; u < U; ++u) {
        const float wj = (WMODE == 0) ? roww : (MH ? 0.f : readlane_f(w, j + u));
#pragma unroll
        for (int ct = 0; ct < CT; ++ct) {
          float wsel = wj;
          if constexpr (MH) wsel = wv[u][ct];
          vacc<VEC>(acc[ct], wsel, gather_t::widen(x[u][ct]));
        }
      }
    }
    const int r = n - j;
    if (r > 0) {
      int jj = j;
#pragma unroll
      for (int p = U / 2; p >= 1; p >>= 1) {
        if (r & p) {
#pragma unroll
          for (int u = 0; u < p; ++u) {
            const uint32_t cj = (uint32_t)__builtin_amdgcn_readlane((int)c, jj + u);
#pragma unroll
            for (int ct = 0; ct < CT; ++ct) x[p + u][ct] = gather.load_raw(cj, voff[ct]);
          }
          jj += p;
        }
      }
      __builtin_amdgcn_sched_barrier(0);
      jj = j;
#pragma unroll
      for (int p = U / 2; p >= 1; p >>= 1) {
        if (r & p) {
#pragma unroll
          for (int u = 0; u < p; ++u) {
            const float wj = (WMODE == 0) ? roww : (MH ? 0.f : readlane_f(w, jj + u));
#pragma unroll
            for (int ct = 0; ct < CT; ++ct) {
              float wh = wj;
              if constexpr (MH) wh = load_edge_w<WMODE>(a, base + jj + u, hd[ct]);
              vacc<VEC>(acc[ct], wh, gather_t::widen(x[p + u][ct]));
            }
          }
          jj += p;
        }
      }
    }
  }
}

}
```

graphaibench_amd/host/aggregators.cpp:

```cpp
#include "aggregator.h"
#include "host_util.h"

using gaib_host::OpTimer;
static inline void count_edges(Graph& g) { gpu_context::add_aggregated_edges((uint64_t)g.sizeEdges()); }
static inline gaib_ctx* C() { return gpu_context::get(); }

static gaib_graph* dev(Graph& g) {
  if (!g.device_graph()) g.copy_to_gpu();
  return g.device_graph();
}

bool aggregator::bf16_tables() {
  int64_t v = 0;
  GAIB_OR_DIE(gaib_get_option(C(), "agg_bf16", &v));
  return v != 0;
}
static uint16_t* g_bf16_tab = nullptr;
static size_t g_bf16_cap = 0;
static gaib_ctx* g_bf16_ctx = nullptr;
static std::vector<uint16_t*> g_bf16_retired;
static uint16_t* bf16_table(size_t elems) {
  if (g_bf16_ctx != C()) {
    if (g_bf16_tab) g_bf16_retired.push_back(g_bf16_tab);
    g_bf16_tab = nullptr;
    g_bf16_cap = 0;
    g_bf16_ctx = C();
  }
  if (elems > g_bf16_cap) {
    if (g_bf16_tab) g_bf16_retired.push_back(g_bf16_tab);
    g_bf16_tab = nullptr;
    g_bf16_cap = 0;
    GAIB_OR_DIE(gaib_malloc(C(), elems * sizeof(uint16_t), (void**)&g_bf16_tab));
    g_bf16_cap = elems;
  }
  return g_bf16_tab;
}

static const uint16_t* to_bf16(size_t rows, int len, const float* in) {
  const size_t n = rows * (size_t)len;
  uint16_t* t = bf16_table(n);
  GAIB_OR_DIE(gaib_cast_f32_bf16(C(), (int64_t)n, in, t));
  return t;
}
static void no_bf16_halo(Graph& g) {
  if (!g.has_halo()) return;
  fprintf(stderr, "GPU error: agg_bf16 (GAIB_AGG_DTYPE=bf16) covers whole graphs only; this graph has a halo (partitioned run)\n");
  exit(EXIT_FAILURE);
}

template <class Plain, class Last>
static void halo_half(Graph& g, gaib_graph* whole, int len, Plain plain, Last last) {
  const int K = g.halo_pieces(len);
  if (K <= 1) {
    last(whole, g.halo_end(len));
    return;
  }
  int last_k = 0;
  for (int k = 0; k < K; k++)
    if (gaib_graph_ne(g.halo_piece_graph(k)) > 0) last_k = k;
  for (int k = 0; k < last_k; k++)
    if (gaib_graph_ne(g.halo_piece_graph(k)) > 0) plain(g.halo_piece_graph(k), g.halo_wait_piece(k));
  last(g.halo_piece_graph(last_k), g.halo_end(len));
}

static void aggregate_rows(Graph& g, int kind, int len, const float* in, float* out, bool relu = false, bool count = true) {
  if (count) count_edges(g);
  const int act = relu ? GAIB_RELU : 0;
  if (aggregator::bf16_tables()) {
    no_bf16_halo(g);
    gaib_graph* dg = dev(g);
    GAIB_OR_DIE(gaib_spmm_bf16(C(), dg, kind, NULL, len, to_bf16((size_t)gaib_graph_nc(dg), len, in), out, act));
    return;
  }
  if (!g.has_halo()) {
    GAIB_OR_DIE(gaib_spmm_ex(C(), dev(g), kind, NULL, len, in, out, act));
    return;
  }
  const int mode = g.partition_mode(len);
  auto acc = [&](gaib_graph* gh, const float* halo) {
    GAIB_OR_DIE(gaib_spmm_ex(C(), gh, kind, NULL, len, halo, out, GAIB_ACCUMULATE));
  };
  auto acc_act = [&](gaib_graph* gh, const float* halo) {
    GAIB_OR_DIE(gaib_spmm_ex(C(), gh, kind, NULL, len, halo, out, GAIB_ACCUMULATE | act));
  };
  if (mode != Graph::PART_SPLIT) {
    g.halo_begin(len, in);
    GAIB_OR_DIE(gaib_spmm_ex(C(), g.class_interior(), kind, NULL, len, in, out, act));
    if (mode == Graph::PART_CLASSES) {
      const bool have_halo_edges = gaib_graph_ne(g.class_boundary_halo()) > 0;
      GAIB_OR_DIE(gaib_spmm_ex(C(), g.class_boundary_own(), kind, NULL, len, in, out, have_halo_edges ? 0 : act));
      if (have_halo_edges) halo_half(g, g.class_boundary_halo(), len, acc, acc_act);
      else g.halo_end(len);
    } else {
      const float* halo = g.halo_end(len);
      GAIB_OR_DIE(gaib_spmm_2t(C(), g.class_boundary_full(), kind, NULL, len, in, halo, (int64_t)g.size(), out, act));
    }
    return;
  }
  g.halo_begin(len, in);
  const bool have_halo_edges = gaib_graph_ne(g.halo_graph()) > 0;
  GAIB_OR_DIE(gaib_spmm_ex(C(), dev(g), kind, NULL, len, in, out, have_halo_edges ? 0 : act));
  if (!have_halo_edges) {
    g.halo_end(len);
    return;
  }
  halo_half(g, g.halo_graph(), len, acc, acc_act);
}

void aggregator::aggregate_then_matmul(int kind, int len, Graph& g, const float* in, float* agg, bool keep_agg,
                                       const float* W, bool transW, int len_out, float* out, bool relu,
                                       const float* rows2, const float* W2) {
  OpTimer t(OP_SPARSEMM);
  count_edges(g);
  if (bf16_tables()) {
    no_bf16_halo(g);
    gaib_graph* dg = dev(g);
    const int fl = (relu ? GAIB_RELU : 0) | (keep_agg ? 0 : GAIB_AGG_SCRATCH);
    const uint16_t* tab = to_bf16((size_t)gaib_graph_nc(dg), len, in);
    if (rows2)
      GAIB_OR_DIE(gaib_spmm_gemm2_bf16(C(), dg, kind, NULL, len, tab, agg, W, transW ? 1 : 0, rows2, W2, len_out, out, fl));
    else
      GAIB_OR_DIE(gaib_spmm_gemm_bf16(C(), dg, kind, NULL, len, tab, agg, W, transW ? 1 : 0, len_out, out, fl));
    return;
  }
  const int flags = (relu ? GAIB_RELU : 0) | (keep_agg ? 0 : GAIB_AGG_SCRATCH);
  auto fused = [&](gaib_graph* dg, const float* src, int fl) {
    if (rows2)
      GAIB_OR_DIE(gaib_spmm_gemm2(C(), dg, kind, NULL, len, src, agg, W, transW ? 1 : 0, rows2, W2, len_out, out, fl));
    else
      GAIB_OR_DIE(gaib_spmm_gemm(C(), dg, kind, NULL, len, src, agg, W, transW ? 1 : 0, len_out, out, fl));
  };
  auto plain_acc = [&](gaib_graph* gh, const float* halo) {
    GAIB_OR_DIE(gaib_spmm_ex(C(), gh, kind, NULL, len, halo, agg, GAIB_ACCUMULATE));
  };
  const int mode = g.has_halo() ? g.partition_mode(len) : Graph::PART_SPLIT;
  if (mode != Graph::PART_SPLIT) {
    if (!gaib_spmm_gemm_fusable(C(), kind, len, len_out, rows2 ? 1 : 0)) {
      aggregate_rows(g, kind, len, in, agg, false, false);
      const int act = relu ? GAIB_RELU : 0;
      GAIB_OR_DIE(gaib_sgemm_ex(C(), 0, transW ? 1 : 0, (int64_t)g.size(), len_out, len, agg, W, rows2 ? 0 : act, out));
      if (rows2)
        GAIB_OR_DIE(gaib_sgemm_ex(C(), 0, transW ? 1 : 0, (int64_t)g.size(), len_out, len, rows2, W2, GAIB_ACCUMULATE | act, out));
      return;
    }
    g.halo_begin(len, in);
    fused(g.class_interior(), in, flags | GAIB_OVERLAPS_TRANSFER);
    if (mode == Graph::PART_CLASSES) {
      if (gaib_graph_ne(g.class_boundary_halo()) == 0) {
        g.halo_end(len);
        return;
      }
      GAIB_OR_DIE(gaib_spmm_ex(C(), g.class_boundary_own(), kind, NULL, len, in, agg, 0));
      halo_half(g, g.class_boundary_halo(), len, plain_acc,
                [&](gaib_graph* gh, const float* halo) { fused(gh, halo, flags | GAIB_ACCUMULATE); });
    } else {
      const float* halo = g.halo_end(len);
      GAIB_OR_DIE(gaib_spmm_gemm_2t(C(), g.class_boundary_full(), kind, NULL, len, in, halo, (int64_t)g.size(), agg, W,
                                    transW ? 1 : 0, rows2, W2, len_out, out, flags));
    }
    return;
  }
  if (g.has_halo()) {
    g.halo_begin(len, in);
    if (gaib_graph_ne(g.halo_graph()) == 0) {
      fused(dev(g), in, flags | GAIB_OVERLAPS_TRANSFER);
      g.halo_end(len);
      return;
    }
    GAIB_OR_DIE(gaib_spmm_ex(C(), dev(g), kind, NULL, len, in, agg, 0));
    halo_half(g, g.halo_graph(), len, plain_acc,
              [&](gaib_graph* gh, const float* halo) { fused(gh, halo, flags | GAIB_ACCUMULATE); });
    return;
  }
  fused(dev(g), in, flags);
}

void GCN_Aggregator::aggregate_matmul(int len, Graph& g, const float* in, float* agg, bool keep_agg,
                                      const float* W, bool transW, int len_out, float* out, bool relu) {
  aggregate_then_matmul(GAIB_W_GCN, len, g, in, agg, keep_agg, W, transW, len_out, out, relu);
}
void GCN_Aggregator::d_aggregate_matmul(int len, Graph& g, const float* grad_in, float* agg, bool keep_agg,
                                        const float* W, bool transW, int len_out, float* out) {
  aggregate_then_matmul(GAIB_W_GCN, len, g, grad_in, agg, keep_agg, W, transW, len_out, out, false);
}
void SAGE_Aggregator::aggregate_matmul(int len, Graph& g, const float* in, float* agg, bool keep_agg,
                                       const float* W, bool transW, int len_out, float* out, bool relu,
                                       const float* rows_self, const float* W_self) {
  aggregate_then_matmul(GAIB_W_MEAN, len, g, in, agg, keep_agg, W, transW, len_out, out, relu, rows_self, W_self);
}
void SAGE_Aggregator::d_aggregate_matmul(int len, Graph& g, const float* grad_in, float* agg, bool keep_agg,
                                         const float* W, bool transW, int len_out, float* out,
                                         const float* rows_self, const float* W_self) {
  aggregate_then_matmul(GAIB_W_MEAN_T, len, g, grad_in, agg, keep_agg, W, transW, len_out, out, false, rows_self,
                        W_self);
}
void GCN_Aggregator::init(int l, int nv, int, float, float) {
  length = l;
  n = nv;
}
void GCN_Aggregator::aggregate(int len, Graph& g, const float* in, float* out) {
  OpTimer t(OP_SPARSEMM);
  aggregate_rows(g, GAIB_W_GCN, len, in, out, fuse_relu);
  fuse_relu = false;
}
void GCN_Aggregator::d_aggregate(int len, Graph& g, const float*, const float* grad_in, float* grad_out) {
  OpTimer t(OP_SPARSEMM);
  aggregate_rows(g, GAIB_W_GCN, len, grad_in, grad_out);
}

void SAGE_Aggregator::init(int l, int nv, int, float, float) {
  length = l;
  n = nv;
}
void SAGE_Aggregator::aggregate(int len, Graph& g, const float* in, float* out) {
  OpTimer t(OP_SPARSEMM);
  aggregate_rows(g, GAIB_W_MEAN, len, in, out, fuse_relu);
  fuse_relu = false;
}
void SAGE_Aggregator::d_aggregate(int len, Graph& g, const float*, const float* grad_in, float* grad_out) {
  OpTimer t(OP_SPARSEMM);
  aggregate_rows(g, GAIB_W_MEAN_T, len, grad_in, grad_out);
}

GAT_Aggregator::GAT_Aggregator()
    : epsilon(0.2f), attn_drop(0.f), attn_scale(1.f), training(true), dropped_last(false), d_norm_scores_drop(NULL),
      d_attn_masks(NULL), drop_cap(0), drop_seed(0xA77E0000ull), num_edges(0), heads(1), d_alpha_l(NULL), d_alpha_r(NULL), d_alpha_lgrad(NULL),
      d_alpha_rgrad(NULL), d_temp_scores(NULL), d_norm_scores(NULL),
      d_norm_scores_grad(NULL), d_norm_scores_t(NULL), fwd_out(NULL), d_tbuf(NULL), tbuf_floats(0), d_ptab(NULL), d_pout(NULL),
      d_prs(NULL), d_pcs(NULL), ptab_floats(0), pvec_floats(0), d_pgrad(NULL), d_prec(NULL), pgrad_floats(0), prec_floats(0),
      part_fused_last(false), d_row_stats(NULL), stats_floats(0), stats_valid(false),
      last_graph(NULL), last_in(NULL), last_len(0), alpha_opt(NULL) {}

void GAT_Aggregator::init(int l, int nv, int ne, float lr, float drop_rate) {
  length = l;
  n = nv;
  attn_drop = drop_rate;
  assert(attn_drop >= 0. && attn_drop < 1.);
  attn_scale = 1.f / (1.f - attn_drop);
  num_edges = (size_t)ne;
  vec_t al, ar;
  init_glorot(l, 1, al, 2);
  init_glorot(l, 1, ar, 3);
  d_alpha_l = gaib_host::dmalloc<float>(l);
  d_alpha_r = gaib_host::dmalloc<float>(l);
  d_alpha_lgrad = gaib_host::dmalloc<float>(l);
  d_alpha_rgrad = gaib_host::dmalloc<float>(l);
  copy_float_device(l, al.data(), d_alpha_l);
  copy_float_device(l, ar.data(), d_alpha_r);
  GAIB_OR_DIE(gaib_fill_f32(C(), l, 0.f, d_alpha_lgrad));
  GAIB_OR_DIE(gaib_fill_f32(C(), l, 0.f, d_alpha_rgrad));
  d_temp_scores = gaib_host::dmalloc<float>(num_edges);
  d_norm_scores = gaib_host::dmalloc<float>(num_edges);
  d_norm_scores_grad = gaib_host::dmalloc<float>(num_edges);
  d_norm_scores_t = gaib_host::dmalloc<float>(num_edges);
  epsilon = 0.2f;
  alpha_opt = new adam(lr);
}

const float* GAT_Aggregator::apply_attn_dropout(size_t n_scores) {
  if (n_scores > drop_cap) {
    if (d_norm_scores_drop) float_free_device(d_norm_scores_drop);
    if (d_attn_masks) GAIB_OR_DIE(gaib_free(C(), d_attn_masks));
    float_malloc_device64(n_scores, d_norm_scores_drop);
    d_attn_masks = gaib_host::dmalloc<mask_t>(n_scores);
    drop_cap = n_scores;
  }
  OpTimer t(OP_DROPOUT);
  GAIB_OR_DIE(gaib_dropout(C(), (int64_t)n_scores, attn_scale, attn_drop, drop_seed++, d_norm_scores, d_attn_masks,
                           d_norm_scores_drop));
  dropped_last = true;
  return d_norm_scores_drop;
}

void GAT_Aggregator::release() {
  gaib_ctx* c = C();
  float** owned[] = {&d_alpha_l, &d_alpha_r, &d_alpha_lgrad, &d_alpha_rgrad, &d_temp_scores, &d_norm_scores, &d_norm_scores_grad,
                     &d_norm_scores_t, &d_norm_scores_drop, &d_tbuf, &d_ptab, &d_pout, &d_prs, &d_pcs, &d_pgrad, &d_prec,
// ... 303 lines not shown
```

graphaibench_amd/host/layers.cpp:

```cpp
#include "graph_conv_layer.h"
#include "host_util.h"
#include "math_functions.hh"

static inline gaib_ctx* C() { return gpu_context::get(); }

gconv_state::gconv_state(int id, int nv, int din, int dout, Graph* g, bool act, bool concat, float lr,
                         float feat_drop, float score_drop)
    : level_(id), num_samples(nv), dim_in(din), dim_out(dout), graph(g), is_act(act), is_bias(false),
      use_concat(concat), feat_dropout_rate(feat_drop), score_dropout_rate(score_drop),
      phase_(net_phase::TRAIN), capacity_((size_t)nv), dropout_calls(0), feat_in(NULL), grad_in(NULL),
      d_in_temp(NULL), d_in_temp1(NULL), d_out_temp(NULL), d_W_neigh(NULL), d_W_neigh_grad(NULL),
      d_W_self(NULL), d_W_self_grad(NULL), dropout_mask(NULL), optm(NULL) {
  assert(feat_dropout_rate >= 0. && feat_dropout_rate < 1.);
  assert(score_dropout_rate >= 0. && score_dropout_rate < 1.);
  feat_scale = 1. / (1. - feat_dropout_rate);
  const size_t nin = (size_t)nv * din, nout = (size_t)nv * dout, nw = (size_t)din * dout;
  vec_t w;
  init_glorot(din, dout, w, 1);
  d_W_neigh = gaib_host::dmalloc<float>(nw);
  d_W_neigh_grad = gaib_host::dmalloc<float>(nw);
  GAIB_OR_DIE(gaib_memcpy_h2d(C(), d_W_neigh, w.data(), sizeof(float) * nw));
  GAIB_OR_DIE(gaib_fill_f32(C(), nw, 0.f, d_W_neigh_grad));
  if (concat) {
    init_glorot(din, dout, w, 2);
// ... 21 lines not shown
}

void gconv_state::release() {
  gaib_ctx* c = C();
  float** owned[] = {&grad_in, &d_in_temp, &d_in_temp1, &d_out_temp, &d_W_neigh, &d_W_neigh_grad, &d_W_self, &d_W_self_grad};
  for (float** p : owned) {
    if (*p) GAIB_OR_DIE(gaib_free(c, *p));
    *p = NULL;
  }
  if (level_ > 0 && feat_in) GAIB_OR_DIE(gaib_free(c, feat_in));
  feat_in = NULL;
  if (dropout_mask) GAIB_OR_DIE(gaib_free(c, dropout_mask));
  dropout_mask = NULL;
  if (optm) {
    optm->reset();
    delete optm;
    optm = NULL;
  }
  capacity_ = 0;
  agg_valid_ = false;
}

void gconv_state::update_dim_size(size_t x) {
  if (x > capacity_) {
    const size_t nin = x * dim_in, nout = x * dim_out;
    auto regrow = [&](float*& p, size_t n) {
      if (!p) return;
      GAIB_OR_DIE(gaib_free(C(), p));
      p = gaib_host::dmalloc<float>(n);
      GAIB_OR_DIE(gaib_fill_f32(C(), n, 0.f, p));
    };
    regrow(d_in_temp, nin);
    regrow(d_in_temp1, nin);
    regrow(d_out_temp, nout);
    if (level_ > 0) regrow(feat_in, nin);
    regrow(grad_in, nout);
    if (dropout_mask) {
      GAIB_OR_DIE(gaib_free(C(), dropout_mask));
      dropout_mask = gaib_host::dmalloc<mask_t>(nin);
    }
    capacity_ = x;
  }
  num_samples = (int)x;
  agg_valid_ = false;
}

template class graph_conv_layer<GCN_Aggregator>;
template class graph_conv_layer<SAGE_Aggregator>;
template class graph_conv_layer<GAT_Aggregator>;

void GCN_layer::forward(float* feat_out) {
  const size_t x = num_samples, y = dim_in, z = dim_out;
  float* in_data = feat_in;
  if (feat_dropout_rate > 0. && phase_ == net_phase::TRAIN) {
    dropout_gpu(x * y, feat_scale, feat_dropout_rate, in_data, dropout_mask, d_in_temp);
    in_data = d_in_temp;
  }
  if (y > z) {
    matmul(x, z, y, in_data, d_W_neigh, d_out_temp);
    if (is_act) aggr.fuse_relu_once();
    aggr.aggregate(z, *graph, d_out_temp, feat_out);
  } else if (input_constant_ && agg_valid_ && in_data == feat_in) {
    if (is_act) matmul_relu(x, z, y, d_in_temp1, d_W_neigh, feat_out);
    else matmul(x, z, y, d_in_temp1, d_W_neigh, feat_out);
  } else {
    aggr.aggregate_matmul(y, *graph, in_data, d_in_temp1, true, d_W_neigh, false, z, feat_out, is_act);
    agg_valid_ = input_constant_ && in_data == feat_in;
  }
}

void GCN_layer::backward(float* feat_out, float* grad_out) {
  const size_t x = num_samples, y = dim_in, z = dim_out;
  if (y > z) {
    if (is_act) d_relu_gpu(x * z, grad_in, feat_out, grad_in);
    if (level_ > 0) aggr.d_aggregate_matmul(z, *graph, grad_in, d_out_temp, true, d_W_neigh, true, y, grad_out);
    else aggr.d_aggregate(z, *graph, NULL, grad_in, d_out_temp);
    float* in_data = feat_dropout_rate > 0. ? d_in_temp : feat_in;
    matmul(y, z, x, in_data, d_out_temp, d_W_neigh_grad, true, false);
  } else {
    if (is_act) matmul_drelu(y, z, x, d_in_temp1, grad_in, feat_out, d_W_neigh_grad);
    else matmul(y, z, x, d_in_temp1, grad_in, d_W_neigh_grad, true, false);
    if (level_ > 0) {
      if (y == z) {
        aggr.d_aggregate_matmul(z, *graph, grad_in, d_in_temp, false, d_W_neigh, true, y, grad_out);
      } else {
        matmul(x, y, z, grad_in, d_W_neigh, d_in_temp, false, true);
        aggr.d_aggregate(y, *graph, NULL, d_in_temp, grad_out);
      }
    }
  }
  if (level_ != 0 && feat_dropout_rate > 0.)
    d_dropout_gpu(x * y, feat_scale, grad_out, dropout_mask, grad_out);
}

void GCN_layer::update_weight(optimizer* opt) {
  opt->update_gpu((size_t)dim_in * dim_out, d_W_neigh_grad, d_W_neigh);
}

void SAGE_layer::forward(float* feat_out) {
  const size_t x = num_samples, y = dim_in, z = dim_out;
  float* in_data = feat_in;
  if (feat_dropout_rate > 0. && phase_ == net_phase::TRAIN) {
    dropout_gpu(x * y, feat_scale, feat_dropout_rate, in_data, dropout_mask, d_in_temp);
    in_data = d_in_temp;
  }
  if (y > z) {
    matmul(x, z, y, in_data, d_W_neigh, d_out_temp);
    aggr.aggregate(z, *graph, d_out_temp, feat_out);
    if (is_act) matmul_relu(x, z, y, in_data, d_W_self, feat_out, false, false, true);
    else matmul(x, z, y, in_data, d_W_self, feat_out, false, false, true);
  } else if (input_constant_ && agg_valid_ && in_data == feat_in) {
    matmul(x, z, y, d_in_temp1, d_W_neigh, feat_out);
    if (is_act) matmul_relu(x, z, y, in_data, d_W_self, feat_out, false, false, true);
    else matmul(x, z, y, in_data, d_W_self, feat_out, false, false, true);
  } else {
    aggr.aggregate_matmul(y, *graph, in_data, d_in_temp1, true, d_W_neigh, false, z, feat_out, is_act, in_data,
                          d_W_self);
    agg_valid_ = input_constant_ && in_data == feat_in;
  }
}

void SAGE_layer::backward(float* feat_out, float* grad_out) {
  const size_t x = num_samples, y = dim_in, z = dim_out;
  float* in_data = feat_dropout_rate > 0. ? d_in_temp : feat_in;
  if (is_act) matmul_drelu(y, z, x, in_data, grad_in, feat_out, d_W_self_grad);
  else matmul(y, z, x, in_data, grad_in, d_W_self_grad, true, false);
  if (y > z) {
    if (level_ > 0)
      aggr.d_aggregate_matmul(z, *graph, grad_in, d_out_temp, true, d_W_neigh, true, y, grad_out, grad_in, d_W_self);
    else aggr.d_aggregate(z, *graph, NULL, grad_in, d_out_temp);
    matmul(y, z, x, in_data, d_out_temp, d_W_neigh_grad, true, false);
  } else {
    matmul(y, z, x, d_in_temp1, grad_in, d_W_neigh_grad, true, false);
    if (level_ > 0) {
      if (y == z) {
        aggr.d_aggregate_matmul(z, *graph, grad_in, d_in_temp, false, d_W_neigh, true, y, grad_out, grad_in, d_W_self);
      } else {
        matmul(x, y, z, grad_in, d_W_neigh, d_in_temp, false, true);
        aggr.d_aggregate(y, *graph, NULL, d_in_temp, grad_out);
        matmul(x, y, z, grad_in, d_W_self, grad_out, false, true, true);
      }
    }
  }
  if (level_ != 0 && feat_dropout_rate > 0.)
    d_dropout_gpu(x * y, feat_scale, grad_out, dropout_mask, grad_out);
}

void SAGE_layer::update_weight(optimizer*) {
  optm->update_gpu((size_t)dim_in * dim_out, d_W_neigh_grad, d_W_neigh);
  optm->update_gpu((size_t)dim_in * dim_out, d_W_self_grad, d_W_self);
}

void GAT_layer::forward(float* feat_out) {
  const size_t x = num_samples, y = dim_in, z = dim_out;
  float* in_data = feat_in;
  if (feat_dropout_rate > 0. && phase_ == net_phase::TRAIN) {
    dropout_gpu(x * y, feat_scale, feat_dropout_rate, in_data, dropout_mask, d_in_temp);
    in_data = d_in_temp;
  }
  matmul(x, z, y, in_data, d_W_neigh, d_out_temp);
  aggr.set_training(phase_ == net_phase::TRAIN);
  if (is_act) aggr.fuse_relu_once();
  aggr.aggregate(z, *graph, d_out_temp, feat_out);
}

void GAT_layer::backward(float* feat_out, float* grad_out) {
  const size_t x = num_samples, y = dim_in, z = dim_out;
  if (is_act) d_relu_gpu(x * z, grad_in, feat_out, grad_in);
  float* in_data = feat_dropout_rate > 0. ? d_in_temp : feat_in;
  aggr.use_forward_output_once(feat_out);
  aggr.d_aggregate(z, *graph, d_out_temp, grad_in, d_out_temp);
  if (level_ != 0) {
    matmul(x, y, z, d_out_temp, d_W_neigh, grad_out, false, true);
    if (feat_dropout_rate > 0.) d_dropout_gpu(x * y, feat_scale, grad_out, dropout_mask, grad_out);
  }
  matmul(y, z, x, in_data, d_out_temp, d_W_neigh_grad, true);
}

void GAT_layer::update_weight(optimizer* opt) {
  opt->update_gpu((size_t)dim_in * dim_out, d_W_neigh_grad, d_W_neigh);
  aggr.update_weights(opt);
}
```

graphaibench_amd/host/train_main.cpp:

```cpp
#include <omp.h>
#include <algorithm>
#include <string>
#include <vector>
#include <fcntl.h>
#include <signal.h>
#include <sys/stat.h>
#include <sys/wait.h>
#include <time.h>
#include <unistd.h>
#include "partition.h"
#include "cutils.h"
#include "dense_layer.h"
#include "graph_conv_layer.h"
#include "l2norm_layer.h"
#include "math_functions.hh"
#include "reader.h"
#include "sampler.h"
#include "softmax_loss_layer.h"

#if defined(USE_GAT)
typedef GAT_layer gconv_t;
static const gnn_arch ARCH = gnn_arch::GAT;
static const char* ARCH_NAME = "Graph Attention Network";
#elif defined(USE_SAGE)
// ... 57 lines not shown
  void init_comm() {
    rank = env_int("GAIB_RANK", "RANK", 0);
    world = env_int("GAIB_WORLD", "WORLD_SIZE", 1);
    if (world <= 1) return;
    const char* tr = getenv("GAIB_COMM");
    int transport = (tr && std::string(tr) == "ipc") ? GAIB_COMM_IPC : GAIB_COMM_RCCL;
    int ndev = 0;
    GAIB_OR_DIE(gaib_device_count(&ndev));
    if (!tr && world > ndev) {
      transport = GAIB_COMM_IPC;
      if (rank == 0) std::cerr << world << " ranks on " << ndev << " device(s): GAIB_COMM=ipc\n";
    }
    std::string path = getenv("GAIB_COMM_ID_FILE") ? getenv("GAIB_COMM_ID_FILE")
                                                  : std::string("/dev/shm/gaib_id_") +
                                                        (getenv("MASTER_PORT") ? getenv("MASTER_PORT") : "default");
    unsigned char id[GAIB_COMM_ID_BYTES];
    const time_t started = time(nullptr);
    if (rank == 0) {
      unlink(path.c_str());
      GAIB_OR_DIE(gaib_comm_unique_id(transport, id));
      const std::string tmp = path + ".tmp";
      FILE* f = fopen(tmp.c_str(), "wb");
      if (!f || fwrite(id, 1, sizeof(id), f) != sizeof(id)) {
        std::cerr << "cannot write " << tmp << "\n";
        exit(EXIT_FAILURE);
      }
      fclose(f);
      rename(tmp.c_str(), path.c_str());
    } else {
      const double deadline = omp_get_wtime() + 120.0;
      size_t got = 0;
      while (omp_get_wtime() < deadline) {
        struct stat st;
        FILE* f = (stat(path.c_str(), &st) == 0 && st.st_mtime + 60 >= started) ? fopen(path.c_str(), "rb") : nullptr;
        if (f) {
          got = fread(id, 1, sizeof(id), f);
          fclose(f);
          if (got == sizeof(id)) break;
        }
        usleep(2000);
      }
      if (got != sizeof(id)) {
        std::cerr << "rank " << rank << ": no communicator id at " << path << " after 120 s\n";
        exit(EXIT_FAILURE);
      }
    }
    GAIB_OR_DIE(gaib_comm_init(gpu_context::get(), rank, world, id, transport, &comm));
    if (rank == 0) unlink(path.c_str());
    gpu_context::set_comm(comm);
  }

  void local_range(size_t gb, size_t ge, size_t& b, size_t& e) const {
    const size_t lo = (size_t)part.lo, hi = (size_t)part.hi;
    const size_t x = std::max(gb, lo), y = std::min(ge, hi);
    b = x < y ? x - lo : 0;
    e = x < y ? y - lo : 0;
  }

  void parse(int argc, char** argv) {
    dataset = argv[1];
    num_epochs = atoi(argv[2]);
    num_threads = atoi(argv[3]);
    omp_set_num_threads(num_threads);
    is_sigmoid = std::string(argv[4]) == "sigmoid";
    if (argc >= 6) dim_hid = atoi(argv[5]);
    if (argc >= 7) score_drop = atof(argv[6]);
    if (argc >= 8) feat_drop = atof(argv[7]);
    if (argc >= 9) lrate = atof(argv[8]);
    if (argc > 9) {
      assert(argc == 13);
      num_layers = atoi(argv[9]);
      subg_size = atoi(argv[10]);
      val_interval = atoi(argv[11]);
      inductive = atoi(argv[12]);
    }
    assert(num_layers >= 2);
    if (subg_size > 0 || ARCH == gnn_arch::GAT) use_l2norm = use_dense = true;
    if (subg_size > 0) inductive = 1;
    init_comm();
    const bool bf16 = aggregator::bf16_tables();
    if (root())
      std::cout << "aggregation tables: " << (bf16 ? (ARCH == gnn_arch::GAT ? "fp32 (bf16 asked; GAT gathers fp32)" : "bf16") : "fp32")
                << "\n";
    if (bf16 && world > 1) {
      std::cerr << "GAIB_AGG_DTYPE=bf16 runs on one GPU only (a partitioned run gathers fp32 tables)\n";
      exit(EXIT_FAILURE);
    }
    if (world > 1 && (subg_size > 0 || inductive)) {
      std::cerr << "subgraph sampling / inductive training run on one GPU only\n";
      exit(EXIT_FAILURE);
    }
  }

  void relabel(const char* how, std::vector<float>& feats, std::vector<label_t>& labels, std::vector<mask_t>& mtrain,
               std::vector<mask_t>& mval, std::vector<mask_t>& mtest) {
    const std::string m(how);
    if (m != "bfs" && m != "degree" && m != "cm") {
      std::cerr << "GAIB_REORDER=" << m << ": cm, bfs or degree\n";
      exit(EXIT_FAILURE);
    }
    const size_t n = graph->size(), ne = graph->sizeEdges();
    gaib_ctx* c = gpu_context::get();
    gaib_graph *g0 = nullptr, *g1 = nullptr;
    GAIB_OR_DIE(gaib_graph_create(c, (int64_t)n, (int64_t)ne, graph->row_start_host_ptr(), 32, graph->edge_dst_host_ptr(), 0, &g0));
    int64_t *d_no = nullptr, *d_on = nullptr;
    GAIB_OR_DIE(gaib_malloc(c, sizeof(int64_t) * n, (void**)&d_no));
    GAIB_OR_DIE(gaib_malloc(c, sizeof(int64_t) * n, (void**)&d_on));
    GAIB_OR_DIE(gaib_graph_reorder(c, g0, m == "cm" ? GAIB_ORDER_CM : (m == "bfs" ? GAIB_ORDER_BFS : GAIB_ORDER_DEGREE), &g1, d_no, d_on));
    std::vector<int64_t> no(n), on(n);
    GAIB_OR_DIE(gaib_memcpy_d2h(c, no.data(), d_no, sizeof(int64_t) * n));
    GAIB_OR_DIE(gaib_memcpy_d2h(c, on.data(), d_on, sizeof(int64_t) * n));
    GAIB_OR_DIE(gaib_free(c, d_no));
    GAIB_OR_DIE(gaib_free(c, d_on));
    GAIB_OR_DIE(gaib_graph_destroy(g0));
    GAIB_OR_DIE(gaib_graph_destroy(g1));
    {
      std::vector<size_t> cuts = {0, n, train_begin, train_end, val_begin, val_end, test_begin, test_end};
      for (auto& c2 : cuts) c2 = std::min(c2, n);
      std::sort(cuts.begin(), cuts.end());
      cuts.erase(std::unique(cuts.begin(), cuts.end()), cuts.end());
      std::vector<int64_t> on2(n);
      for (size_t s2 = 0; s2 + 1 < cuts.size(); s2++) {
        const size_t a = cuts[s2], b = cuts[s2 + 1];
        for (size_t v = a; v < b; v++) on2[v] = (int64_t)v;
        std::sort(on2.begin() + a, on2.begin() + b, [&](int64_t x, int64_t y) { return no[x] < no[y]; });
      }
      on.swap(on2);
      for (size_t k = 0; k < n; k++) no[on[k]] = (int64_t)k;
    }
    index_t* rp = graph->row_start_host_ptr();
    index_t* ci = graph->edge_dst_host_ptr();
    std::vector<index_t> rp2(n + 1, 0), ci2(ne);
    for (size_t k = 0; k < n; k++) rp2[k + 1] = rp2[k] + (rp[on[k] + 1] - rp[on[k]]);
#pragma omp parallel for schedule(dynamic, 256)
    for (size_t k = 0; k < n; k++) {
      const size_t v = (size_t)on[k];
      index_t* dst = ci2.data() + rp2[k];
      const size_t deg = rp[v + 1] - rp[v];
      for (size_t e = 0; e < deg; e++) dst[e] = (index_t)no[ci[rp[v] + e]];
      std::sort(dst, dst + deg);
    }
    std::copy(rp2.begin(), rp2.end(), rp);
    std::copy(ci2.begin(), ci2.end(), ci);
    auto rows = [&](auto& vec, size_t width) {
      typename std::remove_reference<decltype(vec)>::type out(vec.size());
      for (size_t k = 0; k < n; k++) std::copy(vec.begin() + (size_t)on[k] * width, vec.begin() + ((size_t)on[k] + 1) * width, out.begin() + k * width);
      vec.swap(out);
    };
    rows(feats, (size_t)dim_init);
    rows(labels, label_width);
    rows(mtrain, 1), rows(mval, 1), rows(mtest, 1);
    graph->degree_counting();
    if (root()) std::cout << "GAIB_REORDER=" << m << ": vertices relabelled (" << n << " vertices, " << ne << " edges)\n";
  }

  void load() {
    graph = new Graph(true);
    Reader reader(dataset);
    std::vector<float> feats;
    std::vector<label_t> labels;
    reader.bin_read_graph(graph);
    num_samples = graph->size();
    dim_init = reader.bin_read_features(feats);
    num_cls = reader.bin_read_vlabels(labels, !is_sigmoid);
    label_width = is_sigmoid ? (size_t)num_cls : 1;
    if (ARCH != gnn_arch::SAGE) graph->add_selfloop();
// ... 581 lines not shown
```

include/gaib.h:

```cpp
#ifndef GAIB_H
#define GAIB_H

#include <stddef.h>
#include <stdint.h>

#ifdef __cplusplus
extern "C" {
#endif

typedef enum {
  GAIB_OK = 0,
  GAIB_ERR_INVALID = -1,
  GAIB_ERR_HIP = -2,
  GAIB_ERR_NOMEM = -3,
  GAIB_ERR_ASYMMETRIC = -4,
  GAIB_ERR_UNSUPPORTED = -5,
  GAIB_ERR_COMM = -6
} gaib_status;

typedef struct gaib_ctx gaib_ctx;
typedef struct gaib_graph gaib_graph;

const char* gaib_last_error(void);
const char* gaib_version(void);

int gaib_device_count(int* h_count);
int gaib_ctx_create(int device, void* stream, gaib_ctx** out);
int gaib_ctx_destroy(gaib_ctx* ctx);
int gaib_ctx_set_stream(gaib_ctx* ctx, void* stream);
int gaib_ctx_own_stream(gaib_ctx* ctx);
int gaib_sync(gaib_ctx* ctx);
int gaib_side_begin(gaib_ctx* ctx);
int gaib_side_end(gaib_ctx* ctx);
int gaib_side_wait(gaib_ctx* ctx);
typedef struct gaib_exec gaib_exec;
int gaib_capture_begin(gaib_ctx* ctx);
int gaib_capture_end(gaib_ctx* ctx, gaib_exec** out);
int gaib_capture_abort(gaib_ctx* ctx);
int gaib_exec_launch(gaib_ctx* ctx, gaib_exec* exec);
int gaib_exec_elapsed_ms(gaib_exec* exec, float* h_ms);
int64_t gaib_exec_nodes(const gaib_exec* exec);
int gaib_exec_destroy(gaib_exec* exec);

int gaib_malloc(gaib_ctx* ctx, size_t bytes, void** d_ptr);
int gaib_free(gaib_ctx* ctx, void* d_ptr);
int gaib_memcpy_h2d(gaib_ctx* ctx, void* d_dst, const void* h_src, size_t bytes);
int gaib_memcpy_d2h(gaib_ctx* ctx, void* h_dst, const void* d_src, size_t bytes);
int gaib_memcpy_d2d(gaib_ctx* ctx, void* d_dst, const void* d_src, size_t bytes);
int gaib_host_alloc(gaib_ctx* ctx, size_t bytes, void** h_ptr);
int gaib_host_free(gaib_ctx* ctx, void* h_ptr);
int gaib_memcpy_d2h_async(gaib_ctx* ctx, void* h_pinned_dst, const void* d_src, size_t bytes);
int gaib_fill_f32(gaib_ctx* ctx, int64_t n, float value, float* d_x);
int gaib_scale_f32(gaib_ctx* ctx, int64_t n, float alpha, float* d_x);
int gaib_cast_f32_bf16(gaib_ctx* ctx, int64_t n, const float* d_in, uint16_t* d_out);
int gaib_cast_bf16_f32(gaib_ctx* ctx, int64_t n, const uint16_t* d_in, float* d_out);

int gaib_graph_create(gaib_ctx* ctx, int64_t nv, int64_t ne, const void* rowptr, int rowptr_bits,
                      const uint32_t* colidx, int src_on_device, gaib_graph** out);
int gaib_graph_create_rect(gaib_ctx* ctx, int64_t nv, int64_t nc, int64_t ne, const void* rowptr,
                           int rowptr_bits, const uint32_t* colidx, int src_on_device,
                           gaib_graph** out);
int gaib_graph_set_vertex_norm(gaib_ctx* ctx, gaib_graph* g, const float* d_row_vdata,
                               const float* d_row_inv_deg, const float* d_col_vdata,
                               const float* d_col_inv_deg);
int gaib_graph_destroy(gaib_graph* g);
int gaib_graph_add_selfloop(gaib_ctx* ctx, const gaib_graph* g, gaib_graph** out);
#define GAIB_ORDER_DEGREE 1
#define GAIB_ORDER_BFS 2
#define GAIB_ORDER_CM 3
int gaib_graph_reorder(gaib_ctx* ctx, gaib_graph* g, int method, gaib_graph** out, int64_t* d_new_of_old,
                       int64_t* d_old_of_new);
int gaib_graph_sort_rows(gaib_ctx* ctx, gaib_graph* g);
int64_t gaib_graph_nv(const gaib_graph* g);
int64_t gaib_graph_ne(const gaib_graph* g);
int64_t gaib_graph_nc(const gaib_graph* g);
const int64_t* gaib_graph_rowptr(const gaib_graph* g);
const uint32_t* gaib_graph_colidx(const gaib_graph* g);
int gaib_graph_compute_vertex_data(gaib_ctx* ctx, gaib_graph* g);
const float* gaib_graph_vertex_data(const gaib_graph* g);
int gaib_graph_compute_edge_data(gaib_ctx* ctx, gaib_graph* g);
const float* gaib_graph_edge_data(const gaib_graph* g);
int64_t gaib_graph_device_bytes(const gaib_graph* g);

typedef enum {
  GAIB_W_GCN = 0,
  GAIB_W_MEAN = 1,
  GAIB_W_MEAN_T = 2,
  GAIB_W_EDGE = 3,
  GAIB_W_EDGE_T = 4
} gaib_weight_kind;
int gaib_spmm(gaib_ctx* ctx, gaib_graph* g, int weight_kind, const float* d_edge_w, int len,
              const float* d_in, float* d_out);
int gaib_spmm_acc(gaib_ctx* ctx, gaib_graph* g, int weight_kind, const float* d_edge_w, int len,
                  const float* d_in, float* d_out);
#define GAIB_ACCUMULATE 1
#define GAIB_RELU 2
#define GAIB_AGG_SCRATCH 4
#define GAIB_OVERLAPS_TRANSFER 8
int gaib_spmm_ex(gaib_ctx* ctx, gaib_graph* g, int weight_kind, const float* d_edge_w, int len,
                 const float* d_in, float* d_out, int flags);
int gaib_spmm_bf16(gaib_ctx* ctx, gaib_graph* g, int weight_kind, const float* d_edge_w, int len, const uint16_t* d_in,
                   float* d_out, int flags);
int gaib_spmm_mh(gaib_ctx* ctx, gaib_graph* g, int weight_kind, const float* d_edge_w, int heads,
                 int len, const float* d_in, float* d_out, int flags);

int gaib_gat_scores(gaib_ctx* ctx, gaib_graph* g, int len, const float* d_h, const float* d_alpha_l,
                    const float* d_alpha_r, float epsilon, float* d_temp_scores, float* d_scores,
                    float* d_norm_scores);
int gaib_gat_scores_mh(gaib_ctx* ctx, gaib_graph* g, int len, int heads, const float* d_h,
                       const float* d_alpha_l, const float* d_alpha_r, float epsilon,
                       float* d_temp_scores, float* d_scores, float* d_norm_scores);
int gaib_sddmm_mh(gaib_ctx* ctx, gaib_graph* g, int len, int heads, const float* d_grad,
                  const float* d_feat, float* d_out_e);
int gaib_gat_softmax_bwd_alpha_mh(gaib_ctx* ctx, gaib_graph* g, int len, int heads, const float* d_feat,
                                  const float* d_norm_scores, const float* d_norm_scores_grad,
                                  const float* d_temp_scores, float epsilon, float* d_scores,
                                  float* d_alpha_lgrad, float* d_alpha_rgrad);
int gaib_edge_transpose_mh(gaib_ctx* ctx, gaib_graph* g, int heads, const float* d_in_e, float* d_out_e);
int gaib_sddmm(gaib_ctx* ctx, gaib_graph* g, int len, const float* d_grad, const float* d_feat,
               float* d_out_e);
int gaib_gat_softmax_bwd_alpha(gaib_ctx* ctx, gaib_graph* g, int len, const float* d_feat,
                               const float* d_norm_scores, const float* d_norm_scores_grad,
                               const float* d_temp_scores, float epsilon, float* d_scores,
                               float* d_alpha_lgrad, float* d_alpha_rgrad);
int gaib_gat_softmax_bwd_alpha_ex(gaib_ctx* ctx, gaib_graph* g, int len, int heads, const float* d_feat,
                                  const float* d_norm_scores, const float* d_norm_scores_grad,
                                  const float* d_temp_scores, float epsilon, float* d_scores,
                                  float* d_alpha_lgrad, float* d_alpha_rgrad, const float* d_grad_rows,
                                  const float* d_fwd_out_rows, float* d_norm_scores_t);
int gaib_gat_softmax_bwd_alpha_re(gaib_ctx* ctx, gaib_graph* g, int len, int heads, const float* d_feat,
                                  const float* d_alpha_l, const float* d_alpha_r, const float* d_norm_scores,
                                  const float* d_norm_scores_grad, float epsilon, float* d_scores,
                                  float* d_alpha_lgrad, float* d_alpha_rgrad, const float* d_grad_rows,
                                  const float* d_fwd_out_rows, float* d_norm_scores_t);
int gaib_gat_backward_fused(gaib_ctx* ctx, gaib_graph* g, int len, int heads, const float* d_feat, const float* d_grad,
                            const float* d_fwd_out, const float* d_alpha_l, const float* d_alpha_r,
                            const float* d_norm_scores, const float* d_row_stats, float epsilon, float* d_grad_out,
                            float* d_alpha_lgrad, float* d_alpha_rgrad);
int gaib_gat_forward_fused(gaib_ctx* ctx, gaib_graph* g, int len, int heads, const float* d_h, const float* d_alpha_l,
                           const float* d_alpha_r, float epsilon, int relu, float* d_out, float* d_row_stats);
int gaib_gat_score_signs(gaib_ctx* ctx, gaib_graph* g, int len, int heads, const float* d_h, const float* d_alpha_l,
                         const float* d_alpha_r, uint8_t* d_sign_out);
int gaib_gat_forward_fused_rect(gaib_ctx* ctx, gaib_graph* g, int len, int heads, const float* d_tab, const float* d_alpha_l,
                                const float* d_alpha_r, float epsilon, int relu, float* d_out, float* d_row_stats, int phase);
int gaib_gat_backward_rec(gaib_ctx* ctx, int64_t nv, int len, int heads, const float* d_grad, const float* d_fwd_out,
                          const float* d_row_stats, float* d_rec);
int gaib_gat_backward_fused_rect(gaib_ctx* ctx, gaib_graph* g, int len, int heads, const float* d_feat_tab,
                                 const float* d_grad_tab, const float* d_rec_tab, const float* d_alpha_l,
                                 const float* d_alpha_r, float epsilon, float* d_grad_out, float* d_alpha_lgrad,
                                 float* d_alpha_rgrad, int phase);
int gaib_gat_softmax_bwd_rows(gaib_ctx* ctx, gaib_graph* g, int heads, const float* d_norm_scores,
                              const float* d_norm_scores_grad, const float* d_temp_scores, float epsilon,
                              float* d_g_out, float* d_rs_out);
int gaib_edge_gather_perm(gaib_ctx* ctx, int64_t ne, int heads, const uint32_t* d_perm, const float* d_in_e,
                          float* d_out_e);
int gaib_edge_rowsum(gaib_ctx* ctx, gaib_graph* g, int heads, const float* d_in_e, float* d_out_rows);
int gaib_gat_alpha_grads(gaib_ctx* ctx, int64_t nv, int len, int heads, const float* d_x, const float* d_rs,
                         const float* d_cs, float* d_alpha_lgrad, float* d_alpha_rgrad);
int gaib_edge_transpose(gaib_ctx* ctx, gaib_graph* g, const float* d_in_e, float* d_out_e);

#define GAIB_SPLIT_ALL_BOUNDARY 1
int gaib_graph_split_classes(gaib_ctx* ctx, const gaib_graph* g_own, const gaib_graph* g_halo, gaib_graph** interior,
                             gaib_graph** bnd_own, gaib_graph** bnd_halo, gaib_graph** bnd_full, int64_t* h_n_boundary,
                             int64_t* h_boundary_edges, int flags);
#define GAIB_GRAPH_MAX_PIECES 16
int gaib_graph_split_pieces(gaib_ctx* ctx, const gaib_graph* g, int n_pieces, int n_ranges, const int64_t* h_range_begin,
                            const int64_t* h_range_end, const int* h_range_piece, gaib_graph** out);
int gaib_graph_set_row_map(gaib_ctx* ctx, gaib_graph* g, const uint32_t* d_row_map, int64_t n_out_rows);
const uint32_t* gaib_graph_row_map(const gaib_graph* g);
int gaib_spmm_2t(gaib_ctx* ctx, gaib_graph* g, int weight_kind, const float* d_edge_w, int len, const float* d_in,
                 const float* d_in2, int64_t n_first, float* d_out, int flags);
int gaib_spmm_gemm_2t(gaib_ctx* ctx, gaib_graph* g, int weight_kind, const float* d_edge_w, int len_in, const float* d_in,
                      const float* d_in2, int64_t n_first, float* d_agg, const float* d_W, int transW, const float* d_rows2,
                      const float* d_W2, int len_out, float* d_out, int flags);
int gaib_spmm_gemm_fusable(gaib_ctx* ctx, int weight_kind, int len_in, int len_out, int dual);

int gaib_spmm_gemm(gaib_ctx* ctx, gaib_graph* g, int weight_kind, const float* d_edge_w,
                   int len_in, const float* d_in, float* d_agg, const float* d_W, int transW,
                   int len_out, float* d_out, int flags);

int gaib_spmm_gemm2(gaib_ctx* ctx, gaib_graph* g, int weight_kind, const float* d_edge_w,
                    int len_in, const float* d_in, float* d_agg, const float* d_W, int transW,
                    const float* d_rows2, const float* d_W2, int len_out, float* d_out, int flags);

int gaib_spmm_gemm_bf16(gaib_ctx* ctx, gaib_graph* g, int weight_kind, const float* d_edge_w, int len_in,
                        const uint16_t* d_in, float* d_agg, const float* d_W, int transW, int len_out, float* d_out,
                        int flags);
int gaib_spmm_gemm2_bf16(gaib_ctx* ctx, gaib_graph* g, int weight_kind, const float* d_edge_w, int len_in,
                         const uint16_t* d_in, float* d_agg, const float* d_W, int transW, const float* d_rows2,
                         const float* d_W2, int len_out, float* d_out, int flags);

int gaib_sgemm(gaib_ctx* ctx, int transA, int transB, int64_t M, int64_t N, int64_t K,
               const float* d_A, const float* d_B, int accum, float* d_C);
int gaib_sgemm_ex(gaib_ctx* ctx, int transA, int transB, int64_t M, int64_t N, int64_t K,
                  const float* d_A, const float* d_B, int flags, float* d_C);

int gaib_sgemm_drelu(gaib_ctx* ctx, int64_t M, int64_t N, int64_t K, const float* d_A, float* d_G,
                     const float* d_mask, int accum, float* d_C);

int gaib_relu(gaib_ctx* ctx, int64_t n, const float* d_in, float* d_out);
int gaib_d_relu(gaib_ctx* ctx, int64_t n, const float* d_in_diff, const float* d_data,
                float* d_out_diff);
int gaib_dropout(gaib_ctx* ctx, int64_t n, float scale, float drop_rate, uint64_t seed,
                 const float* d_in, uint8_t* d_masks, float* d_out);
int gaib_d_dropout(gaib_ctx* ctx, int64_t n, float scale, const float* d_in,
                   const uint8_t* d_masks, float* d_out);

int gaib_bias_add(gaib_ctx* ctx, int64_t n, int len, float* d_x, const float* d_b);
int gaib_colsum(gaib_ctx* ctx, int64_t n, int len, const float* d_x, float* d_a);
int gaib_rng_uniform(gaib_ctx* ctx, int64_t n, float a, float b, uint64_t seed, float* d_r);
int gaib_csr2csc(gaib_ctx* ctx, int nrows, int ncols, int nnz, const float* d_values, const int* d_rowptr,
                 const int* d_colidx, float* d_valuesT, int* d_rowptrT, int* d_colidxT);

int gaib_softmax_xent(gaib_ctx* ctx, int num_cls, int64_t begin, int64_t end,
                      const float* d_in, const uint8_t* d_masks, const uint8_t* d_labels,
                      float* d_loss, float* d_out);
int gaib_d_softmax_xent(gaib_ctx* ctx, int num_cls, int64_t begin, int64_t end,
                        const uint8_t* d_masks, const uint8_t* d_labels, const float* d_out,
                        float* d_diff);
int gaib_sigmoid_xent(gaib_ctx* ctx, int num_cls, int64_t begin, int64_t end,
                      const float* d_in, const uint8_t* d_masks, const uint8_t* d_labels,
                      float* d_loss, float* d_out);
int gaib_d_sigmoid_xent(gaib_ctx* ctx, int num_cls, int64_t begin, int64_t end,
                        const uint8_t* d_masks, const uint8_t* d_labels,
                        const float* d_out, float* d_diff);
int gaib_masked_f1_micro(gaib_ctx* ctx, int64_t begin, int64_t end, int num_cls,
                         const uint8_t* d_masks, const float* d_preds, const uint8_t* d_labels,
                         float* h_result, int64_t* h_counts);
int gaib_masked_avg_loss(gaib_ctx* ctx, int64_t begin, int64_t end, const uint8_t* d_masks,
                         const float* d_loss, float* h_result);
int gaib_masked_accuracy_single(gaib_ctx* ctx, int64_t begin, int64_t end, int num_cls,
                                const uint8_t* d_masks, const float* d_preds,
                                const uint8_t* d_labels, float* h_result);
int gaib_masked_avg_loss_dev(gaib_ctx* ctx, int64_t begin, int64_t end, const uint8_t* d_masks,
                             const float* d_loss, float* d_result);
int gaib_masked_accuracy_single_dev(gaib_ctx* ctx, int64_t begin, int64_t end, int num_cls,
                                    const uint8_t* d_masks, const float* d_preds,
                                    const uint8_t* d_labels, float* d_result);
int gaib_masked_f1_counts_dev(gaib_ctx* ctx, int64_t begin, int64_t end, int num_cls,
                              const uint8_t* d_masks, const float* d_preds, const uint8_t* d_labels,
                              uint64_t* d_counts);

int gaib_l2norm(gaib_ctx* ctx, int64_t n, int dim, const float* d_in, float* d_out);
int gaib_d_l2norm(gaib_ctx* ctx, int64_t n, int dim, const float* d_feat_in,
                  const float* d_grad_in, float* d_grad_out);

int gaib_adam_step(gaib_ctx* ctx, int64_t n, const float* d_dW, float* d_W, float* d_m,
                   float* d_v, float alpha, float b1, float b2, float b1_t, float b2_t, float eps);
int gaib_adam_step_dev(gaib_ctx* ctx, int64_t n, const float* d_dW, float* d_W, float* d_m, float* d_v,
                       float alpha, float b1, float b2, float eps, float* d_pow);

int gaib_gather_rows(gaib_ctx* ctx, int64_t n_idx, const int64_t* d_idx, int len,
                     const float* d_in, float* d_out);
int gaib_gather_scatter_rows(gaib_ctx* ctx, int64_t n_idx, const int64_t* d_src_idx, const int64_t* d_dst_idx, int len,
                             const float* d_in, float* d_out);

typedef struct gaib_comm gaib_comm;
typedef struct gaib_halo gaib_halo;
#define GAIB_COMM_ID_BYTES 128
#define GAIB_COMM_RCCL 0
#define GAIB_COMM_IPC 1
int gaib_comm_transport_available(int transport);
int gaib_comm_unique_id(int transport, void* h_id);
int gaib_comm_init(gaib_ctx* ctx, int rank, int nranks, const void* h_id, int transport, gaib_comm** out);
int gaib_comm_destroy(gaib_comm* comm);
int gaib_comm_rank(const gaib_comm* comm);
int gaib_comm_size(const gaib_comm* comm);
// ... 43 lines not shown
```

include/gnn/aggregator.h:

```cpp
#pragma once
#include "lgraph.h"
#include "math_functions.hh"
#include "optimizer.h"

class aggregator {
 public:
  aggregator() : n(0), length(0), fuse_relu(false) {}
  static bool bf16_tables();
  void set_vlen(int vlen) { length = vlen; }
  void fuse_relu_once() { fuse_relu = true; }
  void release() {}

 protected:
  void aggregate_then_matmul(int kind, int len, Graph& g, const float* in, float* agg, bool keep_agg,
                             const float* W, bool transW, int len_out, float* out, bool relu,
                             const float* rows2 = NULL, const float* W2 = NULL);

  int n;
  int length;
  bool fuse_relu;
};

class GCN_Aggregator : public aggregator {
 public:
  void init(int length, int nv, int ne = 0, float lr = 0.01, float drop_rate = 0.);
  void aggregate(int len, Graph& g, const float* in, float* out);
  void d_aggregate(int len, Graph& g, const float* feat_in, const float* grad_in, float* grad_out);
  void aggregate_matmul(int len, Graph& g, const float* in, float* agg, bool keep_agg, const float* W,
                        bool transW, int len_out, float* out, bool relu);
  void d_aggregate_matmul(int len, Graph& g, const float* grad_in, float* agg, bool keep_agg, const float* W,
                          bool transW, int len_out, float* out);
};

class SAGE_Aggregator : public aggregator {
 public:
  void init(int length, int nv, int ne = 0, float lr = 0.01, float drop_rate = 0.);
  void aggregate(int len, Graph& g, const float* in, float* out);
  void d_aggregate(int len, Graph& g, const float* feat_in, const float* grad_in, float* grad_out);
  void aggregate_matmul(int len, Graph& g, const float* in, float* agg, bool keep_agg, const float* W,
                        bool transW, int len_out, float* out, bool relu, const float* rows_self = NULL,
                        const float* W_self = NULL);
  void d_aggregate_matmul(int len, Graph& g, const float* grad_in, float* agg, bool keep_agg, const float* W,
                          bool transW, int len_out, float* out, const float* rows_self = NULL,
                          const float* W_self = NULL);
};

class GAT_Aggregator : public aggregator {
 public:
  GAT_Aggregator();
  void init(int length, int nv, int ne = 0, float lr = 0.01, float drop_rate = 0.);
  void aggregate(int len, Graph& g, const float* in, float* out);
  void d_aggregate(int len, Graph& g, const float* feat_in, const float* grad_in, float* grad_out);
  void update_weights(optimizer* opt);
  void release();
  void set_num_heads(int h);
  int num_heads() const { return heads; }
  void use_forward_output_once(const float* out) { fwd_out = out; fwd_out_given = true; }
  void set_training(bool on) { training = on; }
  float* alpha_l_ptr() { return d_alpha_l; }
  float* alpha_r_ptr() { return d_alpha_r; }
  float* alpha_lgrad_ptr() { return d_alpha_lgrad; }
  float* alpha_rgrad_ptr() { return d_alpha_rgrad; }
  float* norm_scores_ptr();
  float* temp_scores_ptr() { return d_temp_scores; }
  float* scores_ptr() { return NULL; }
  float* norm_scores_grad_ptr() { return d_norm_scores_grad; }
  float* norm_scores_dropped_ptr() { return d_norm_scores_drop; }
  mask_t* attn_masks_ptr() { return d_attn_masks; }

 private:
  bool needs_temp() const { return !(heads == 4 || heads == 8 || heads == 16); }
  float epsilon;
  float attn_drop, attn_scale;
  bool training, dropped_last;
  float* d_norm_scores_drop;
  mask_t* d_attn_masks;
  size_t drop_cap;
  uint64_t drop_seed;
  bool dropping() const { return attn_drop > 0.f && training; }
  const float* apply_attn_dropout(size_t n_scores);
  size_t num_edges;
  int heads;
  float *d_alpha_l, *d_alpha_r, *d_alpha_lgrad, *d_alpha_rgrad;
  float *d_temp_scores, *d_norm_scores, *d_norm_scores_grad, *d_norm_scores_t;
  const float* fwd_out;
  bool fwd_out_given = false;
  float* d_tbuf;
  size_t tbuf_floats;
  float *d_ptab, *d_pout, *d_prs, *d_pcs;
  size_t ptab_floats, pvec_floats;
  float *d_pgrad, *d_prec;
  size_t pgrad_floats, prec_floats;
  bool part_fused_last;
  void ensure_partition_buffers(Graph& g, int len);
  void aggregate_partition(int len, Graph& g, const float* in, float* out);
  void d_aggregate_partition(int len, Graph& g, const float* grad_in, float* grad_out);
  float* d_row_stats;
  size_t stats_floats;
  bool stats_valid;
  Graph* last_graph;
  const float* last_in;
  int last_len;
  void materialise_scores();
  optimizer* alpha_opt;
};
```

Before: 13.73 billion edges/s.

## Gather relu-masked gradients from a zero-suppressed packed table in fused SpMM-GEMM

Adds a zero-suppressed row format (bitmasks plus the packed nonzeros, 384 bytes per 128-column row) for relu-masked gradient tables. The backward fused SpMM+GEMM gathers from this compact image instead of the dense fp32 table, with rows that overflow the cap falling back to the dense table. The aim is to cut the bytes read per edge in the bandwidth-bound gather. The cost is an extra pack kernel per call, and a host-side guard that pauses the path when overflow is frequent and probes it again periodically. It is enabled by default.

```diff
diff --git a/graphaibench_amd/build.py b/graphaibench_amd/build.py
--- a/graphaibench_amd/build.py
+++ b/graphaibench_amd/build.py
@@ -15,7 +15,7 @@
 ORACLE = ROOT / "oracle"
 REFERENCE = Path("/root/reference")
 
-HIP_SOURCES = ["runtime.hip", "graph.hip", "spmm.hip", "spmm_part.hip", "spmm_gemm_bf16.hip", "gat.hip", "sgemm.hip", "sgemm_skinny.hip", "elementwise.hip", "probe.hip", "comm.hip"]
+HIP_SOURCES = ["runtime.hip", "graph.hip", "spmm.hip", "spmm_part.hip", "spmm_gemm_bf16.hip", "spmm_gemm_zs.hip", "gat.hip", "sgemm.hip", "sgemm_skinny.hip", "elementwise.hip", "probe.hip", "comm.hip"]
 HIPCC_FLAGS = [
     "--offload-arch=gfx950",
     "-O3",
diff --git a/graphaibench_amd/capi.py b/graphaibench_amd/capi.py
--- a/graphaibench_amd/capi.py
+++ b/graphaibench_amd/capi.py
@@ -45,6 +45,8 @@
     "gaib_scale_f32": (_i, [_vp, _i64, _f, _vp]),
     "gaib_cast_f32_bf16": (_i, [_vp, _i64, _vp, _vp]),
     "gaib_cast_bf16_f32": (_i, [_vp, _i64, _vp, _vp]),
+    "gaib_pack_zs": (_i, [_vp, _i64, _i, _vp, _vp, _vp]),
+    "gaib_unpack_zs": (_i, [_vp, _i64, _i, _vp, _vp, _vp]),
     "gaib_graph_create": (_i, [_vp, _i64, _i64, _vp, _i, _vp, _i, _pp]),
     "gaib_graph_create_rect": (_i, [_vp, _i64, _i64, _i64, _vp, _i, _vp, _i, _pp]),
     "gaib_graph_destroy": (_i, [_vp]),
@@ -67,6 +69,9 @@
     "gaib_spmm_gemm2": (_i, [_vp, _vp, _i, _vp, _i, _vp, _vp, _vp, _i, _vp, _vp, _i, _vp, _i]),
     "gaib_spmm_mh": (_i, [_vp, _vp, _i, _vp, _i, _i, _vp, _vp, _i]),
     "gaib_spmm_bf16": (_i, [_vp, _vp, _i, _vp, _i, _vp, _vp, _i]),
+    "gaib_spmm_gemm_zs_route": (_i, [_vp, _vp, _i, _i, _vp, _vp, _vp, _vp, _i, _vp]),
+    "gaib_spmm_gemm_zs": (_i, [_vp, _vp, _i, _vp, _i, _vp, _vp, _vp, _vp, _i, _i, _vp, _i]),
+    "gaib_spmm_gemm2_zs": (_i, [_vp, _vp, _i, _vp, _i, _vp, _vp, _vp, _vp, _i, _vp, _vp, _i, _vp, _i]),
     "gaib_spmm_gemm_bf16": (_i, [_vp, _vp, _i, _vp, _i, _vp, _vp, _vp, _i, _i, _vp, _i]),
     "gaib_spmm_gemm2_bf16": (_i, [_vp, _vp, _i, _vp, _i, _vp, _vp, _vp, _i, _vp, _vp, _i, _vp, _i]),
     "gaib_graph_split_classes": (_i, [_vp, _vp, _vp, _pp, _pp, _pp, _pp, C.POINTER(_i64), C.POINTER(_i64), _i]),
@@ -512,6 +517,45 @@
                                             1 if transW else 0, len_out, _ptr(out), flags), "gaib_spmm_gemm_bf16")
         return out
 
+    def pack_zs(self, x, out=None, overflow=None):
+        import torch
+
+        assert x.is_contiguous() and x.dtype == torch.float32 and x.dim() == 2
+        if out is None:
+            out = torch.empty((x.shape[0], 96), dtype=torch.int32, device=x.device)
+        assert out.is_contiguous() and out.dtype == torch.int32 and out.numel() == x.shape[0] * 96
+        _check(self.lib.gaib_pack_zs(self.h, x.shape[0], x.shape[1], _ptr(x), _ptr(out), _ptr(overflow)), "gaib_pack_zs")
+        return out
+
+    def unpack_zs(self, zs, dense, out=None):
+        import torch
+
+        assert zs.is_contiguous() and dense.is_contiguous() and dense.dtype == torch.float32
+        if out is None:
+            out = torch.empty_like(dense)
+        _check(self.lib.gaib_unpack_zs(self.h, dense.shape[0], dense.shape[1], _ptr(zs), _ptr(dense), _ptr(out)), "gaib_unpack_zs")
+        return out
+
+    def spmm_gemm_zs(self, g: "Graph", kind: int, x, zs, agg, W, out, transW: bool = False, relu: bool = False,
+                     agg_scratch: bool = False, edge_w=None, accumulate: bool = False, rows2=None, W2=None) -> bool:
+        assert x.is_contiguous() and zs.is_contiguous() and agg.is_contiguous() and W.is_contiguous() and out.is_contiguous()
+        len_in, len_out = agg.shape[1], out.shape[1]
+        assert tuple(W.shape) == ((len_out, len_in) if transW else (len_in, len_out))
+        flags = (2 if relu else 0) | (4 if agg_scratch else 0) | (1 if accumulate else 0)
+        if rows2 is not None:
+            assert rows2.is_contiguous() and W2.is_contiguous() and W2.shape == W.shape and rows2.shape[1] == len_in
+            rc = self.lib.gaib_spmm_gemm2_zs(self.h, g.h, kind, _ptr(edge_w), len_in, _ptr(x), _ptr(zs), _ptr(agg), _ptr(W),
+                                             1 if transW else 0, _ptr(rows2), _ptr(W2), len_out, _ptr(out), flags)
+            what = "gaib_spmm_gemm2_zs"
+        else:
+            rc = self.lib.gaib_spmm_gemm_zs(self.h, g.h, kind, _ptr(edge_w), len_in, _ptr(x), _ptr(zs), _ptr(agg), _ptr(W),
+                                            1 if transW else 0, len_out, _ptr(out), flags)
+            what = "gaib_spmm_gemm_zs"
+        if rc == -5:
+            return False
+        _check(rc, what)
+        return True
+
     def spmm_2t(self, g: "Graph", kind: int, x, x2, n_first: int, out, edge_w=None, accumulate: bool = False,
                 relu: bool = False):
         assert x.is_contiguous() and out.is_contiguous() and (x2 is None or x2.is_contiguous())
diff --git a/graphaibench_amd/csrc/common.h b/graphaibench_amd/csrc/common.h
--- a/graphaibench_amd/csrc/common.h
+++ b/graphaibench_amd/csrc/common.h
@@ -76,6 +76,8 @@
   int spmm_hot_bytes;
   int spmm_bf16_layout;
   int spmm_bf16_fuse_u;
+  int agg_zs;
+  int agg_zs_paused;
   int agg_bf16;
   int sgemm_variant;
   int gat_fast;
diff --git a/graphaibench_amd/csrc/elementwise.hip b/graphaibench_amd/csrc/elementwise.hip
--- a/graphaibench_amd/csrc/elementwise.hip
+++ b/graphaibench_amd/csrc/elementwise.hip
@@ -1,3 +1,4 @@
+#include <algorithm>
 #include "common.h"
 
 namespace {
@@ -493,6 +494,71 @@
   }
 }
 
+constexpr int ZS_ROW_DW = 96;
+constexpr int ZS_CAP = 46;
+typedef unsigned zs_u2 __attribute__((ext_vector_type(2)));
+
+__global__ __launch_bounds__(256) void pack_zs_kernel(int64_t rows, const float* __restrict__ in, unsigned* __restrict__ out,
+                                                       unsigned* __restrict__ overflow) {
+  __shared__ __attribute__((aligned(16))) unsigned buf[4][ZS_ROW_DW];
+  const int lane = threadIdx.x & 63, wave = threadIdx.x >> 6;
+  unsigned* w = buf[wave];
+  unsigned over = 0;
+  for (int64_t r = (int64_t)blockIdx.x * 4 + wave; r < rows; r += (int64_t)gridDim.x * 4) {
+    const zs_u2 x = __builtin_nontemporal_load(reinterpret_cast<const zs_u2*>(in + r * 128) + lane);
+    const bool b0 = x[0] != 0u, b1 = x[1] != 0u;
+    const unsigned long long m0 = __ballot(b0), m1 = __ballot(b1);
+    const int n0 = __builtin_popcountll(m0), n1 = __builtin_popcountll(m1);
+    const bool fits = n0 <= ZS_CAP && n1 <= ZS_CAP;
+    if (lane < ZS_ROW_DW / 2) {
+      zs_u2 z = {0u, 0u};
+      if (lane == 0) z = zs_u2{(unsigned)m0, (unsigned)(m0 >> 32)};
+      if (lane == 1) z = zs_u2{(unsigned)m1, (unsigned)(m1 >> 32)};
+      *reinterpret_cast<zs_u2*>(w + 2 * lane) = z;
+    }
+    asm volatile("s_waitcnt lgkmcnt(0)" ::: "memory");
+    if (fits) {
+      const unsigned k0 = __builtin_amdgcn_mbcnt_hi((unsigned)(m0 >> 32), __builtin_amdgcn_mbcnt_lo((unsigned)m0, 0u));
+      const unsigned k1 = __builtin_amdgcn_mbcnt_hi((unsigned)(m1 >> 32), __builtin_amdgcn_mbcnt_lo((unsigned)m1, 0u));
+      if (b0) w[4 + 2 * k0] = x[0];
+      if (b1) w[5 + 2 * k1] = x[1];
+    } else {
+      ++over;
+    }
+    asm volatile("s_waitcnt lgkmcnt(0)" ::: "memory");
+    if (lane < ZS_ROW_DW / 2) {
+      const zs_u2 o = *reinterpret_cast<const zs_u2*>(w + 2 * lane);
+      __builtin_nontemporal_store(o, reinterpret_cast<zs_u2*>(out + r * ZS_ROW_DW) + lane);
+    }
+    asm volatile("s_waitcnt lgkmcnt(0)" ::: "memory");
+  }
+  if (overflow && over > 0 && lane == 0) atomicAdd(overflow, over);
+}
+
+__global__ __launch_bounds__(256) void unpack_zs_kernel(int64_t rows, const unsigned* __restrict__ zs, const float* __restrict__ dense,
+                                                         float* __restrict__ out) {
+  __shared__ __attribute__((aligned(16))) unsigned buf[4][ZS_ROW_DW];
+  const int lane = threadIdx.x & 63, wave = threadIdx.x >> 6;
+  unsigned* w = buf[wave];
+  for (int64_t r = (int64_t)blockIdx.x * 4 + wave; r < rows; r += (int64_t)gridDim.x * 4) {
+    if (lane < ZS_ROW_DW / 2) *reinterpret_cast<zs_u2*>(w + 2 * lane) = reinterpret_cast<const zs_u2*>(zs + r * ZS_ROW_DW)[lane];
+    asm volatile("s_waitcnt lgkmcnt(0)" ::: "memory");
+    const unsigned long long m0 = ((unsigned long long)w[1] << 32) | w[0], m1 = ((unsigned long long)w[3] << 32) | w[2];
+    const int n0 = __builtin_popcountll(m0), n1 = __builtin_popcountll(m1);
+    zs_u2 v;
+    if (n0 > ZS_CAP || n1 > ZS_CAP) {
+      v = reinterpret_cast<const zs_u2*>(dense + r * 128)[lane];
+    } else {
+      const unsigned p0 = 4u + 2u * (unsigned)__builtin_popcountll(m0 & ((1ull << lane) - 1ull));
+      const unsigned p1 = 5u + 2u * (unsigned)__builtin_popcountll(m1 & ((1ull << lane) - 1ull));
+      v[0] = ((m0 >> lane) & 1ull) ? w[p0 < (unsigned)ZS_ROW_DW ? p0 : 0u] : 0u;
+      v[1] = ((m1 >> lane) & 1ull) ? w[p1 < (unsigned)ZS_ROW_DW ? p1 : 0u] : 0u;
+    }
+    reinterpret_cast<zs_u2*>(out + r * 128)[lane] = v;
+    asm volatile("s_waitcnt lgkmcnt(0)" ::: "memory");
+  }
+}
+
 }
 
 extern "C" int gaib_fill_f32(gaib_ctx* ctx, int64_t n, float value, float* d_x) {
@@ -533,6 +599,39 @@
   ProfScope ps(ctx, "cast_bf16_f32", 6.0 * (double)n);
   if (vec) cast_bf16_f32_kernel<<<stream_grid(n / 8 + 1, 256), 256, 0, ctx->stream>>>(n, d_in, d_out, 1);
   else cast_bf16_f32_scalar_kernel<<<stream_grid(n, 256), 256, 0, ctx->stream>>>(n, d_in, d_out);
+  GAIB_LAUNCH_CHECK();
+  return GAIB_OK;
+}
+
+extern "C" int gaib_pack_zs(gaib_ctx* ctx, int64_t rows, int len, const float* d_in, void* d_zs, uint32_t* d_overflow) {
+  GAIB_CHECK(ctx && ((d_in && d_zs) || rows == 0), "gaib_pack_zs: NULL argument");
+  GAIB_CHECK(rows >= 0, "gaib_pack_zs: rows < 0");
+  if (len != 128) {
+    gaib_set_error("gaib_pack_zs: rows of %d columns (the zero-suppressed format holds rows of 128)", len);
+    return GAIB_ERR_UNSUPPORTED;
+  }
+  if (rows == 0) return GAIB_OK;
+  GAIB_CHECK(((uintptr_t)d_in & 7) == 0 && ((uintptr_t)d_zs & 127) == 0, "gaib_pack_zs: the table must sit on an 8-B, the image on a 128-B boundary");
+  GAIB_CHECK((const void*)d_in != (const void*)d_zs, "gaib_pack_zs: in and out must not alias");
+  ProfScope ps(ctx, "pack_zs", (512.0 + 384.0) * (double)rows);
+  const unsigned grid = (unsigned)std::min<int64_t>(cdiv64(rows, 4), (int64_t)ctx->num_cus * 32);
+  pack_zs_kernel<<<grid, 256, 0, ctx->stream>>>(rows, d_in, static_cast<unsigned*>(d_zs), d_overflow);
+  GAIB_LAUNCH_CHECK();
+  return GAIB_OK;
+}
+
+extern "C" int gaib_unpack_zs(gaib_ctx* ctx, int64_t rows, int len, const void* d_zs, const float* d_dense, float* d_out) {
+  GAIB_CHECK(ctx && ((d_zs && d_dense && d_out) || rows == 0), "gaib_unpack_zs: NULL argument");
+  GAIB_CHECK(rows >= 0, "gaib_unpack_zs: rows < 0");
+  if (len != 128) {
+    gaib_set_error("gaib_unpack_zs: rows of %d columns (the zero-suppressed format holds rows of 128)", len);
+    return GAIB_ERR_UNSUPPORTED;
+  }
+  if (rows == 0) return GAIB_OK;
+  GAIB_CHECK((((uintptr_t)d_dense | (uintptr_t)d_out | (uintptr_t)d_zs) & 7) == 0, "gaib_unpack_zs: tables must sit on 8-B boundaries");
+  GAIB_CHECK(d_dense != d_out, "gaib_unpack_zs: dense and out must not alias");
+  const unsigned grid = (unsigned)std::min<int64_t>(cdiv64(rows, 4), (int64_t)ctx->num_cus * 32);
+  unpack_zs_kernel<<<grid, 256, 0, ctx->stream>>>(rows, static_cast<const unsigned*>(d_zs), d_dense, d_out);
   GAIB_LAUNCH_CHECK();
   return GAIB_OK;
 }
diff --git a/graphaibench_amd/csrc/runtime.hip b/graphaibench_amd/csrc/runtime.hip
--- a/graphaibench_amd/csrc/runtime.hip
+++ b/graphaibench_amd/csrc/runtime.hip
@@ -63,6 +63,8 @@
   c->spmm_bf16_layout = 0;
   c->spmm_bf16_fuse_u = 0;
   c->agg_bf16 = 0;
+  c->agg_zs = 1;
+  c->agg_zs_paused = 0;
   c->sgemm_variant = 0;
   if (const char* e = getenv("GAIB_SGEMM_VARIANT")) c->sgemm_variant = atoi(e);
   c->gat_fast = 1;
@@ -497,6 +499,9 @@
   else if (!strcmp(key, "spmm_flat_ring")) *h_value = ctx->spmm_flat_ring;
   else if (!strcmp(key, "num_cus")) *h_value = ctx->num_cus;
   else if (!strcmp(key, "agg_bf16")) *h_value = ctx->agg_bf16;
+  else if (!strcmp(key, "agg_zs")) *h_value = ctx->agg_zs;
+  else if (!strcmp(key, "capturing")) *h_value = ctx->capturing;
+  else if (!strcmp(key, "agg_zs_paused")) *h_value = ctx->agg_zs_paused;
   else if (!strcmp(key, "spmm_bf16_layout")) *h_value = ctx->spmm_bf16_layout;
   else if (!strcmp(key, "spmm_bf16_fuse_u")) *h_value = ctx->spmm_bf16_fuse_u;
   else {
@@ -547,6 +552,12 @@
   } else if (!strcmp(key, "agg_bf16")) {
     GAIB_CHECK(value == 0 || value == 1, "agg_bf16 must be 0 (fp32 tables) or 1 (bf16 tables)");
     ctx->agg_bf16 = (int)value;
+  } else if (!strcmp(key, "agg_zs")) {
+    GAIB_CHECK(value == 0 || value == 1, "agg_zs must be 0 (dense gradient tables) or 1 (zero-suppressed)");
+    ctx->agg_zs = (int)value;
+  } else if (!strcmp(key, "agg_zs_paused")) {
+    GAIB_CHECK(value == 0 || value == 1, "agg_zs_paused must be 0 or 1");
+    ctx->agg_zs_paused = (int)value;
   }
   else if (!strcmp(key, "sgemm_variant"))
     ctx->sgemm_variant = (int)value;
diff --git a/graphaibench_amd/csrc/spmm.hip b/graphaibench_amd/csrc/spmm.hip
--- a/graphaibench_amd/csrc/spmm.hip
+++ b/graphaibench_amd/csrc/spmm.hip
@@ -280,6 +280,8 @@
                          int vec, int wmode);
 int gaib_spmm_fused_bf16(gaib_ctx* ctx, const gaib_graph* g, const void* spmm_args, const void* fuse_args, float* heavy_scratch,
                          int vec, int wmode);
+int gaib_spmm_fused_zs(gaib_ctx* ctx, const gaib_graph* g, const void* spmm_args, const void* fuse_args, float* heavy_scratch,
+                       int wmode);
 
 static int spmm_impl(gaib_ctx* ctx, gaib_graph* g, int weight_kind, const float* d_edge_w, int len,
                      const float* d_in, float* d_out, int flags, int heads = 1, const float* d_in2 = nullptr,
@@ -358,7 +360,7 @@
 static int spmm_gemm_impl(gaib_ctx* ctx, gaib_graph* g, int weight_kind, const float* d_edge_w, int len_in,
                           const float* d_in, float* d_agg, const float* d_W, int transW, const float* d_rows2,
                           const float* d_W2, int len_out, float* d_out, int flags, const float* d_in2 = nullptr,
-                          int64_t n_first = 0, bool bf16 = false) {
+                          int64_t n_first = 0, bool bf16 = false, const void* d_zs = nullptr, bool zs_query = false) {
   GAIB_CHECK(ctx && g, "gaib_spmm_gemm: NULL ctx/graph");
   GAIB_CHECK(len_in >= 0 && len_out >= 0, "gaib_spmm_gemm: negative length");
   GAIB_CHECK(ctx->device == g->device, "gaib_spmm_gemm: graph lives on device %d, ctx on %d", g->device,
@@ -381,6 +383,21 @@
                         g->nv >= 1 &&
                         (weight_kind == GAIB_W_GCN || weight_kind == GAIB_W_MEAN ||
                          weight_kind == GAIB_W_MEAN_T || weight_kind == GAIB_W_EDGE);
+  if (d_zs) {
+    const int strip = shape_ok ? fuse_strip_rows(kpad, len_out, dual) : 0;
+    const int64_t dense_bytes = g->nc * (int64_t)len_in * 4;
+    bool ok = !part && len_in == 128 && strip == (dual ? 2 : 8) && dense_bytes < ((int64_t)1 << 32) && ctx->spmm_addr_mode != 2 &&
+              ((uintptr_t)d_zs & 127) == 0;
+    if (ok && !dual && (ctx->spmm_flat >= 1 || (ctx->spmm_flat < 0 && g->ne < 12 * g->nv))) ok = false;
+    if (ok && tile_xcd_arg(ctx, g) != 0) ok = false;
+    if (!ok) {
+      gaib_set_error("gaib_spmm_gemm_zs: no zero-suppressed gather for this call (whole graph, 128 columns, the one-launch fused route "
+                     "in its row form -- 8-row strip or two products, no edge stream, global tile counter --, table below 4 GB, "
+                     "buffer addressing, image on a 128-B boundary)");
+      return GAIB_ERR_UNSUPPORTED;
+    }
+    if (zs_query) return GAIB_OK;
+  }
   if (!part && shape_ok && dual && fuse_strip_rows(kpad, len_out, true) == 0 && fuse_strip_rows(kpad, len_out, false) != 0) {
     GAIB_TRY(spmm_gemm_impl(ctx, g, weight_kind, d_edge_w, len_in, d_in, d_agg, d_W, transW, nullptr, nullptr, len_out, d_out,
                             flags & ~GAIB_RELU, nullptr, 0, bf16));
@@ -498,6 +515,14 @@
   f.n_heavy = (int)g->n_heavy;
   if (part) return gaib_spmm_part_fused(ctx, g, &a, &f, hv, len_in <= 64 ? 1 : 2, wmode);
   if (bf16) return gaib_spmm_fused_bf16(ctx, g, &a, &f, hv, len_in <= 64 ? 1 : 2, wmode);
+  if (d_zs) {
+    a.in2 = a.in;
+    a.in2_bytes = a.in_bytes;
+    a.in = static_cast<const float*>(d_zs);
+    a.ld = GAIB_ZS_ROW_BYTES / 4;
+    a.in_bytes = (uint32_t)(g->nc * (int64_t)GAIB_ZS_ROW_BYTES);
+    return gaib_spmm_fused_zs(ctx, g, &a, &f, hv, wmode);
+  }
   if (len_in <= 64) {
     return wmode == 0 ? launch_fused<1, 0>(ctx, g, a, f, hv) : launch_fused<1, 1>(ctx, g, a, f, hv);
   }
@@ -517,6 +542,32 @@
   GAIB_CHECK(d_rows2 && d_W2, "gaib_spmm_gemm2: NULL second operand");
   return spmm_gemm_impl(ctx, g, weight_kind, d_edge_w, len_in, d_in, d_agg, d_W, transW, d_rows2, d_W2, len_out,
                         d_out, flags);
+}
+
+extern "C" int gaib_spmm_gemm_zs_route(gaib_ctx* ctx, gaib_graph* g, int weight_kind, int len_in, const float* d_in, const void* d_zs,
+                                       float* d_agg, const float* d_rows2, int len_out, float* d_out) {
+  GAIB_CHECK(d_zs, "gaib_spmm_gemm_zs_route: NULL packed table");
+  return spmm_gemm_impl(ctx, g, weight_kind, nullptr, len_in, d_in, d_agg, d_in, 1, d_rows2, d_rows2 ? d_in : nullptr, len_out, d_out,
+                        0, nullptr, 0, false, d_zs, true);
+}
+
+extern "C" int gaib_spmm_gemm_zs(gaib_ctx* ctx, gaib_graph* g, int weight_kind, const float* d_edge_w, int len_in,
+                                 const float* d_in, const void* d_zs, float* d_agg, const float* d_W, int transW, int len_out,
+                                 float* d_out, int flags) {
+  GAIB_CHECK(d_zs, "gaib_spmm_gemm_zs: NULL packed table");
+  GAIB_CHECK(!(flags & GAIB_OVERLAPS_TRANSFER), "gaib_spmm_gemm_zs: GAIB_OVERLAPS_TRANSFER belongs to partitioned runs, which gather dense tables");
+  return spmm_gemm_impl(ctx, g, weight_kind, d_edge_w, len_in, d_in, d_agg, d_W, transW, nullptr, nullptr, len_out, d_out, flags,
+                        nullptr, 0, false, d_zs);
+}
+
+extern "C" int gaib_spmm_gemm2_zs(gaib_ctx* ctx, gaib_graph* g, int weight_kind, const float* d_edge_w, int len_in,
+                                  const float* d_in, const void* d_zs, float* d_agg, const float* d_W, int transW,
+                                  const float* d_rows2, const float* d_W2, int len_out, float* d_out, int flags) {
+  GAIB_CHECK(d_zs, "gaib_spmm_gemm2_zs: NULL packed table");
+  GAIB_CHECK(d_rows2 && d_W2, "gaib_spmm_gemm2_zs: NULL second operand");
+  GAIB_CHECK(!(flags & GAIB_OVERLAPS_TRANSFER), "gaib_spmm_gemm2_zs: GAIB_OVERLAPS_TRANSFER belongs to partitioned runs, which gather dense tables");
+  return spmm_gemm_impl(ctx, g, weight_kind, d_edge_w, len_in, d_in, d_agg, d_W, transW, d_rows2, d_W2, len_out, d_out, flags,
+                        nullptr, 0, false, d_zs);
 }
 
 extern "C" int gaib_spmm_gemm_2t(gaib_ctx* ctx, gaib_graph* g, int weight_kind, const float* d_edge_w, int len_in,
diff --git a/graphaibench_amd/csrc/spmm_core.h b/graphaibench_amd/csrc/spmm_core.h
--- a/graphaibench_amd/csrc/spmm_core.h
+++ b/graphaibench_amd/csrc/spmm_core.h
@@ -130,10 +130,16 @@
   else return widen_bf16<VEC>(*reinterpret_cast<const typename Bf16Raw<VEC>::type*>(p));
 }
 
+struct zs_t { uint32_t bits; };
+constexpr int GAIB_ZS_ROW_BYTES = 384;
+constexpr int GAIB_ZS_CAP = 46;
+
 template <int VEC, int GM, bool PART = false, typename E = float>
 struct RowGather {
   static constexpr bool BUF = GM != 0;
-  static_assert(!PART || sizeof(E) == 4, "two-table gathers: fp32 tables only");
+  static constexpr bool ZS = std::is_same<E, zs_t>::value;
+  static_assert(!PART || (sizeof(E) == 4 && !ZS), "two-table gathers: fp32 tables only");
+  static_assert(!ZS || (VEC == 2 && GM == 1), "zero-suppressed tables: 8-byte lanes (128 columns), buffer addressing");
   __amdgpu_buffer_rsrc_t rsrc, rsrc2;
   const char *inb, *inb2;
   int64_t ldb;
@@ -147,11 +153,37 @@
       inb2 = reinterpret_cast<const char*>(a.in2) - (int64_t)a.n_first * ldb;
       if constexpr (BUF) rsrc2 = __builtin_amdgcn_make_buffer_rsrc((void*)a.in2, 0, (int)a.in2_bytes, 0x00020000);
     }
-  }
-  typedef typename std::conditional<sizeof(E) == 2, typename Bf16Raw<VEC>::type, typename VecT<VEC>::type>::type raw_t;
+    if constexpr (ZS) rsrc2 = __builtin_amdgcn_make_buffer_rsrc((void*)a.in2, 0, (int)a.in2_bytes, 0x00020000);
+  }
+  typedef typename std::conditional<ZS, u2_t, typename std::conditional<sizeof(E) == 2, typename Bf16Raw<VEC>::type,
+                                                                           typename VecT<VEC>::type>::type>::type raw_t;
   static __device__ __forceinline__ typename VecT<VEC>::type widen(const raw_t& r) {
+    static_assert(!ZS, "zero-suppressed tables are expanded by widen_zs");
     if constexpr (sizeof(E) == 2) return widen_bf16<VEC>(r);
     else return r;
+  }
+  __device__ __forceinline__ typename VecT<VEC>::type widen_zs(const raw_t& r, uint32_t cvec, int idx, uint32_t voff) const {
+    typedef unsigned long long u64;
+    const u64 m0 = ((u64)(uint32_t)__builtin_amdgcn_readlane((int)r[1], 0) << 32) | (uint32_t)__builtin_amdgcn_readlane((int)r[0], 0);
+    const u64 m1 = ((u64)(uint32_t)__builtin_amdgcn_readlane((int)r[1], 1) << 32) | (uint32_t)__builtin_amdgcn_readlane((int)r[0], 1);
+    typename VecT<VEC>::type v;
+    if (__builtin_expect(__builtin_popcountll(m0) > GAIB_ZS_CAP || __builtin_popcountll(m1) > GAIB_ZS_CAP, 0)) {
+      const uint32_t cj = (uint32_t)__builtin_amdgcn_readlane((int)cvec, idx);
+      const u2_t d = __builtin_amdgcn_raw_buffer_load_b64(rsrc2, (int)voff, (int)(cj * 512u), 0);
+      v[0] = __uint_as_float(d[0]);
+      v[1] = __uint_as_float(d[1]);
+      return v;
+    }
+    const uint32_t l0 = __builtin_amdgcn_mbcnt_hi((uint32_t)(m0 >> 32), __builtin_amdgcn_mbcnt_lo((uint32_t)m0, 2u));
+    const uint32_t l1 = __builtin_amdgcn_mbcnt_hi((uint32_t)(m1 >> 32), __builtin_amdgcn_mbcnt_lo((uint32_t)m1, 2u));
+    const uint32_t x0 = (uint32_t)__builtin_amdgcn_ds_bpermute((int)(l0 << 2), (int)r[0]);
+    const uint32_t x1 = (uint32_t)__builtin_amdgcn_ds_bpermute((int)(l1 << 2), (int)r[1]);
+    uint32_t k0, k1;
+    asm("v_cndmask_b32_e64 %0, 0, %1, %2" : "=v"(k0) : "v"(x0), "s"(m0));
+    asm("v_cndmask_b32_e64 %0, 0, %1, %2" : "=v"(k1) : "v"(x1), "s"(m1));
+    v[0] = __uint_as_float(k0);
+    v[1] = __uint_as_float(k1);
+    return v;
   }
   __device__ __forceinline__ typename VecT<VEC>::type load(uint32_t cj, uint32_t voff) const { return widen(load_raw(cj, voff)); }
   __device__ __forceinline__ raw_t load_raw(uint32_t cj, uint32_t voff) const {
@@ -172,6 +204,9 @@
       return load_buf<0>(c, voff);
     } else if constexpr (GM == 2) {
       return load_buf<2>(cj, voff);
+    } else if constexpr (ZS) {
+      return __builtin_amdgcn_raw_buffer_load_b64(rsrc, (int)(voff < (uint32_t)GAIB_ZS_ROW_BYTES ? voff : 0u),
+                                                  (int)(cj * (uint32_t)GAIB_ZS_ROW_BYTES), 0);
     } else if constexpr (GM == 1) {
       return load_buf<0>(cj, voff);
     } else {
@@ -216,7 +251,7 @@
                                                 const uint32_t (&voff)[CT],
                                                 typename VecT<VEC>::type (&acc)[CT], uint32_t c_first = 0u,
                                                 float w_first = 0.f) {
-  static_assert(sizeof(E) == 4 || WMODE < 3, "bf16 tables: single-head weights");
+  static_assert((sizeof(E) == 4 && !std::is_same<E, zs_t>::value) || WMODE < 3, "bf16 and zero-suppressed tables: single-head weights");
   typedef RowGather<VEC, BUF, PART, E> gather_t;
   const gather_t gather(a);
   typename gather_t::raw_t x[U][CT];
@@ -256,7 +291,10 @@
         for (int ct = 0; ct < CT; ++ct) {
           float wsel = wj;
           if constexpr (MH) wsel = wv[u][ct];
-          vacc<VEC>(acc[ct], wsel, gather_t::widen(x[u][ct]));
+          if constexpr (gather_t::ZS)
+            vacc<VEC>(acc[ct], wsel, gather.widen_zs(x[u][ct], c, j + u, voff[ct]));
+          else
+            vacc<VEC>(acc[ct], wsel, gather_t::widen(x[u][ct]));
         }
       }
     }
@@ -287,7 +325,10 @@
             for (int ct = 0; ct < CT; ++ct) {
               float wh = wj;
               if constexpr (MH) wh = load_edge_w<WMODE>(a, base + jj + u, hd[ct]);
-              vacc<VEC>(acc[ct], wh, gather_t::widen(x[p + u][ct]));
+              if constexpr (gather_t::ZS)
+                vacc<VEC>(acc[ct], wh, gather.widen_zs(x[p + u][ct], c, jj + u, voff[ct]));
+              else
+                vacc<VEC>(acc[ct], wh, gather_t::widen(x[p + u][ct]));
             }
           }
           jj += p;
diff --git a/graphaibench_amd/csrc/spmm_gemm_zs.hip b/graphaibench_amd/csrc/spmm_gemm_zs.hip
--- /dev/null
+++ b/graphaibench_amd/csrc/spmm_gemm_zs.hip
@@ -0,0 +1,56 @@
+#include "spmm_kernels.h"
+
+namespace {
+
+template <int WMODE>
+int launch_fused_zs(gaib_ctx* ctx, const gaib_graph* g, SpmmArgs a, FuseArgs f, float* heavy_scratch) {
+  constexpr int U = 16;
+  constexpr int K = 128;
+  if (g->n_heavy > 0) {
+    SpmmArgs h = a;
+    h.row_list = g->heavy_rows;
+    h.row_order = g->heavy_rows + g->n_heavy;
+    h.out = heavy_scratch;
+    h.compact = 1;
+    h.relu = 0;
+    h.accumulate = 0;
+    const size_t lds = sizeof(float) * HEAVY_WAVES * K;
+    ProfScope ps(ctx, "spmm_heavy", gaib_alg_spmm_bytes((double)g->heavy_edges, (double)g->n_heavy, a.ncols, WMODE == 0 ? 0 : 4, 1),
+                 2.0 * g->heavy_edges * a.ncols, a.ncols);
+    spmm_heavy_kernel<2, 1, WMODE, U, 1, false, zs_t><<<dim3((unsigned)g->n_heavy), HEAVY_WAVES * 64, lds, ctx->stream>>>(h);
+    GAIB_LAUNCH_CHECK();
+  }
+  f.tile_xcd = 0;
+  const bool dual = f.wt2 != nullptr;
+  const int strip = dual ? 2 : 8;
+  const size_t lds = fuse_lds_bytes(K, f.n_out, dual, strip);
+  const int64_t ntiles = cdiv64(a.n_rows, FUSE_ROWS);
+  const int cus = ctx->spmm_fuse_cus > 0 ? ctx->spmm_fuse_cus : ctx->num_cus;
+  const unsigned grid = (unsigned)std::min<int64_t>(cus, cdiv64(ntiles, FUSE_WAVES));
+  GAIB_HIP(hipMemsetAsync(f.tile_counter, 0, 8 * sizeof(int), ctx->stream));
+  const double e_l = (double)g->ne - (g->n_heavy > 0 ? (double)g->heavy_edges : 0.0), r_all = (double)a.n_rows;
+  const double fused_bytes = gaib_alg_spmm_bytes(e_l, r_all, a.ncols, WMODE == 0 ? 0 : 4, (a.out ? 1 : 0) + (f.agg_in ? 1 : 0) + (dual ? 1 : 0)) +
+                             r_all * 4.0 * f.n_out;
+  const double fused_flops = 2.0 * e_l * a.ncols + 2.0 * r_all * a.ncols * f.n_out * (dual ? 2 : 1);
+  ProfScope ps(ctx, "spmm_gemm_fused", fused_bytes, fused_flops, a.ncols);
+  if (dual) {
+    auto kern = spmm_gemm_kernel<2, WMODE, U, 1, 2, true, false, false, false, false, false, false, zs_t>;
+    GAIB_HIP(hipFuncSetAttribute((const void*)kern, hipFuncAttributeMaxDynamicSharedMemorySize, 160 * 1024));
+    kern<<<dim3(grid), FUSE_WAVES * 64, lds, ctx->stream>>>(a, f);
+  } else {
+    auto kern = spmm_gemm_kernel<2, WMODE, U, 1, 8, false, false, false, false, false, false, false, zs_t>;
+    GAIB_HIP(hipFuncSetAttribute((const void*)kern, hipFuncAttributeMaxDynamicSharedMemorySize, 160 * 1024));
+    kern<<<dim3(grid), FUSE_WAVES * 64, lds, ctx->stream>>>(a, f);
+  }
+  GAIB_LAUNCH_CHECK();
+  return GAIB_OK;
+}
+
+}
+
+int gaib_spmm_fused_zs(gaib_ctx* ctx, const gaib_graph* g, const void* spmm_args, const void* fuse_args, float* heavy_scratch,
+                       int wmode) {
+  const SpmmArgs& a = *static_cast<const SpmmArgs*>(spmm_args);
+  const FuseArgs& f = *static_cast<const FuseArgs*>(fuse_args);
+  return wmode == 0 ? launch_fused_zs<0>(ctx, g, a, f, heavy_scratch) : launch_fused_zs<1>(ctx, g, a, f, heavy_scratch);
+}
diff --git a/graphaibench_amd/host/aggregators.cpp b/graphaibench_amd/host/aggregators.cpp
--- a/graphaibench_amd/host/aggregators.cpp
+++ b/graphaibench_amd/host/aggregators.cpp
@@ -46,6 +46,87 @@
   if (!g.has_halo()) return;
   fprintf(stderr, "GPU error: agg_bf16 (GAIB_AGG_DTYPE=bf16) covers whole graphs only; this graph has a halo (partitioned run)\n");
   exit(EXIT_FAILURE);
+}
+
+static const double ZS_GUARD_SHARE = 0.05;
+static const unsigned ZS_PROBE_EVERY = 8;
+static const bool ZS_TWO_PRODUCTS = false;
+bool aggregator::zs_tables() {
+  int64_t v = 0;
+  GAIB_OR_DIE(gaib_get_option(C(), "agg_zs", &v));
+  return v != 0;
+}
+bool aggregator::zs_paused() {
+  int64_t v = 0;
+  GAIB_OR_DIE(gaib_get_option(C(), "agg_zs_paused", &v));
+  return v != 0;
+}
+static const int ZS_SLOTS = 16;
+struct ZsWatch {
+  const float* table = nullptr;
+  size_t counted_rows = 0;
+  bool paused = false;
+  unsigned since_probe = 0;
+};
+static struct {
+  gaib_ctx* ctx = nullptr;
+  void* tab = nullptr;
+  size_t cap_rows = 0;
+  uint32_t* d_over = nullptr;
+  volatile uint32_t* h_over = nullptr;
+  ZsWatch watch[ZS_SLOTS];
+  int n_watch = 0, next_evict = 0;
+  std::vector<void*> retired;
+} g_zs;
+static void* zs_table(size_t rows) {
+  if (g_zs.ctx != C()) {
+    if (g_zs.h_over) GAIB_OR_DIE(gaib_host_free(C(), const_cast<uint32_t*>(g_zs.h_over)));
+    g_zs.retired.clear();
+    g_zs.tab = nullptr;
+    g_zs.cap_rows = 0;
+    g_zs.ctx = C();
+    g_zs.n_watch = g_zs.next_evict = 0;
+    GAIB_OR_DIE(gaib_malloc(C(), sizeof(uint32_t) * ZS_SLOTS, (void**)&g_zs.d_over));
+    void* h = nullptr;
+    GAIB_OR_DIE(gaib_host_alloc(C(), sizeof(uint32_t) * ZS_SLOTS, &h));
+    g_zs.h_over = static_cast<volatile uint32_t*>(h);
+    for (int i = 0; i < ZS_SLOTS; i++) g_zs.h_over[i] = 0;
+  }
+  if (rows > g_zs.cap_rows) {
+    if (g_zs.tab) g_zs.retired.push_back(g_zs.tab);
+    g_zs.tab = nullptr;
+    g_zs.cap_rows = 0;
+    GAIB_OR_DIE(gaib_malloc(C(), rows * (size_t)384, &g_zs.tab));
+    g_zs.cap_rows = rows;
+  }
+  return g_zs.tab;
+}
+static int zs_slot(const float* table) {
+  for (int i = 0; i < g_zs.n_watch; i++)
+    if (g_zs.watch[i].table == table) return i;
+  int i;
+  if (g_zs.n_watch < ZS_SLOTS) i = g_zs.n_watch++;
+  else i = g_zs.next_evict++ % ZS_SLOTS;
+  g_zs.watch[i] = ZsWatch();
+  g_zs.watch[i].table = table;
+  return i;
+}
+static const void* zs_pack(int slot, size_t rows, const float* in) {
+  void* t = zs_table(rows);
+  GAIB_OR_DIE(gaib_fill_f32(C(), 1, 0.f, reinterpret_cast<float*>(g_zs.d_over + slot)));
+  GAIB_OR_DIE(gaib_pack_zs(C(), (int64_t)rows, 128, in, t, g_zs.d_over + slot));
+  GAIB_OR_DIE(gaib_memcpy_d2h_async(C(), const_cast<uint32_t*>(g_zs.h_over + slot), g_zs.d_over + slot, sizeof(uint32_t)));
+  g_zs.watch[slot].counted_rows = rows;
+  return t;
+}
+static void zs_set_paused(int slot, bool p) {
+  ZsWatch& w = g_zs.watch[slot];
+  if (p == w.paused) return;
+  w.paused = p;
+  w.since_probe = 0;
+  bool any = false;
+  for (int i = 0; i < g_zs.n_watch; i++) any = any || g_zs.watch[i].paused;
+  GAIB_OR_DIE(gaib_set_option(C(), "agg_zs_paused", any ? 1 : 0));
 }
 
 template <class Plain, class Last>
@@ -109,7 +190,7 @@
 
 void aggregator::aggregate_then_matmul(int kind, int len, Graph& g, const float* in, float* agg, bool keep_agg,
                                        const float* W, bool transW, int len_out, float* out, bool relu,
-                                       const float* rows2, const float* W2) {
+                                       const float* rows2, const float* W2, bool relu_masked) {
   OpTimer t(OP_SPARSEMM);
   count_edges(g);
   if (bf16_tables()) {
@@ -172,6 +253,34 @@
               [&](gaib_graph* gh, const float* halo) { fused(gh, halo, flags | GAIB_ACCUMULATE); });
     return;
   }
+  if (relu_masked && len == 128 && (!rows2 || ZS_TWO_PRODUCTS) && zs_tables()) {
+    gaib_graph* dg = dev(g);
+    const size_t rows = (size_t)gaib_graph_nc(dg);
+    int64_t capturing = 0;
+    GAIB_OR_DIE(gaib_get_option(C(), "capturing", &capturing));
+    if (g_zs.ctx != C()) zs_table(0);
+    int route = gaib_spmm_gemm_zs_route(C(), dg, kind, len, in, g_zs.d_over, agg, rows2, len_out, out);
+    if (route != GAIB_OK && route != GAIB_ERR_UNSUPPORTED) GAIB_OR_DIE(route);
+    if (route == GAIB_OK && rows > g_zs.cap_rows) {
+      if (capturing) route = GAIB_ERR_UNSUPPORTED;
+      else zs_table(rows);
+    }
+    if (route == GAIB_OK) {
+      const int slot = zs_slot(in);
+      ZsWatch& w = g_zs.watch[slot];
+      if (w.counted_rows > 0) zs_set_paused(slot, (double)g_zs.h_over[slot] > ZS_GUARD_SHARE * (double)w.counted_rows);
+      if (w.paused) {
+        if (!capturing && ++w.since_probe % ZS_PROBE_EVERY == 0) zs_pack(slot, rows, in);
+      } else {
+        const void* tab = zs_pack(slot, rows, in);
+        if (rows2)
+          GAIB_OR_DIE(gaib_spmm_gemm2_zs(C(), dg, kind, NULL, len, in, tab, agg, W, transW ? 1 : 0, rows2, W2, len_out, out, flags));
+        else
+          GAIB_OR_DIE(gaib_spmm_gemm_zs(C(), dg, kind, NULL, len, in, tab, agg, W, transW ? 1 : 0, len_out, out, flags));
+        return;
+      }
+    }
+  }
   fused(dev(g), in, flags);
 }
 
@@ -180,8 +289,8 @@
   aggregate_then_matmul(GAIB_W_GCN, len, g, in, agg, keep_agg, W, transW, len_out, out, relu);
 }
 void GCN_Aggregator::d_aggregate_matmul(int len, Graph& g, const float* grad_in, float* agg, bool keep_agg,
-                                        const float* W, bool transW, int len_out, float* out) {
-  aggregate_then_matmul(GAIB_W_GCN, len, g, grad_in, agg, keep_agg, W, transW, len_out, out, false);
+                                        const float* W, bool transW, int len_out, float* out, bool relu_masked) {
+  aggregate_then_matmul(GAIB_W_GCN, len, g, grad_in, agg, keep_agg, W, transW, len_out, out, false, NULL, NULL, relu_masked);
 }
 void SAGE_Aggregator::aggregate_matmul(int len, Graph& g, const float* in, float* agg, bool keep_agg,
                                        const float* W, bool transW, int len_out, float* out, bool relu,
@@ -190,9 +299,9 @@
 }
 void SAGE_Aggregator::d_aggregate_matmul(int len, Graph& g, const float* grad_in, float* agg, bool keep_agg,
                                          const float* W, bool transW, int len_out, float* out,
-                                         const float* rows_self, const float* W_self) {
+                                         const float* rows_self, const float* W_self, bool relu_masked) {
   aggregate_then_matmul(GAIB_W_MEAN_T, len, g, grad_in, agg, keep_agg, W, transW, len_out, out, false, rows_self,
-                        W_self);
+                        W_self, relu_masked);
 }
 void GCN_Aggregator::init(int l, int nv, int, float, float) {
   length = l;
diff --git a/graphaibench_amd/host/layers.cpp b/graphaibench_amd/host/layers.cpp
--- a/graphaibench_amd/host/layers.cpp
+++ b/graphaibench_amd/host/layers.cpp
@@ -127,7 +127,7 @@
     else matmul(y, z, x, d_in_temp1, grad_in, d_W_neigh_grad, true, false);
     if (level_ > 0) {
       if (y == z) {
-        aggr.d_aggregate_matmul(z, *graph, grad_in, d_in_temp, false, d_W_neigh, true, y, grad_out);
+        aggr.d_aggregate_matmul(z, *graph, grad_in, d_in_temp, false, d_W_neigh, true, y, grad_out, is_act);
       } else {
         matmul(x, y, z, grad_in, d_W_neigh, d_in_temp, false, true);
         aggr.d_aggregate(y, *graph, NULL, d_in_temp, grad_out);
@@ -179,7 +179,7 @@
     matmul(y, z, x, d_in_temp1, grad_in, d_W_neigh_grad, true, false);
     if (level_ > 0) {
       if (y == z) {
-        aggr.d_aggregate_matmul(z, *graph, grad_in, d_in_temp, false, d_W_neigh, true, y, grad_out, grad_in, d_W_self);
+        aggr.d_aggregate_matmul(z, *graph, grad_in, d_in_temp, false, d_W_neigh, true, y, grad_out, grad_in, d_W_self, is_act);
       } else {
         matmul(x, y, z, grad_in, d_W_neigh, d_in_temp, false, true);
         aggr.d_aggregate(y, *graph, NULL, d_in_temp, grad_out);
diff --git a/graphaibench_amd/host/train_main.cpp b/graphaibench_amd/host/train_main.cpp
--- a/graphaibench_amd/host/train_main.cpp
+++ b/graphaibench_amd/host/train_main.cpp
@@ -163,6 +163,8 @@
     if (root())
       std::cout << "aggregation tables: " << (bf16 ? (ARCH == gnn_arch::GAT ? "fp32 (bf16 asked; GAT gathers fp32)" : "bf16") : "fp32")
                 << "\n";
+    if (world == 1 && !bf16 && ARCH != gnn_arch::GAT && root())
+      std::cout << "relu-masked gradients of 128 columns are gathered " << (aggregator::zs_tables() ? "zero-suppressed (agg_zs = 1)" : "dense (agg_zs = 0)") << "\n";
     if (bf16 && world > 1) {
       std::cerr << "GAIB_AGG_DTYPE=bf16 runs on one GPU only (a partitioned run gathers fp32 tables)\n";
       exit(EXIT_FAILURE);
diff --git a/include/gaib.h b/include/gaib.h
--- a/include/gaib.h
+++ b/include/gaib.h
@@ -54,6 +54,9 @@
 int gaib_scale_f32(gaib_ctx* ctx, int64_t n, float alpha, float* d_x);
 int gaib_cast_f32_bf16(gaib_ctx* ctx, int64_t n, const float* d_in, uint16_t* d_out);
 int gaib_cast_bf16_f32(gaib_ctx* ctx, int64_t n, const uint16_t* d_in, float* d_out);
+
+int gaib_pack_zs(gaib_ctx* ctx, int64_t rows, int len, const float* d_in, void* d_zs, uint32_t* d_overflow);
+int gaib_unpack_zs(gaib_ctx* ctx, int64_t rows, int len, const void* d_zs, const float* d_dense, float* d_out);
 
 int gaib_graph_create(gaib_ctx* ctx, int64_t nv, int64_t ne, const void* rowptr, int rowptr_bits,
                       const uint32_t* colidx, int src_on_device, gaib_graph** out);
@@ -183,6 +186,14 @@
                     int len_in, const float* d_in, float* d_agg, const float* d_W, int transW,
                     const float* d_rows2, const float* d_W2, int len_out, float* d_out, int flags);
 
+int gaib_spmm_gemm_zs_route(gaib_ctx* ctx, gaib_graph* g, int weight_kind, int len_in, const float* d_in, const void* d_zs,
+                            float* d_agg, const float* d_rows2, int len_out, float* d_out);
+int gaib_spmm_gemm_zs(gaib_ctx* ctx, gaib_graph* g, int weight_kind, const float* d_edge_w, int len_in, const float* d_in,
+                      const void* d_zs, float* d_agg, const float* d_W, int transW, int len_out, float* d_out, int flags);
+int gaib_spmm_gemm2_zs(gaib_ctx* ctx, gaib_graph* g, int weight_kind, const float* d_edge_w, int len_in, const float* d_in,
+                       const void* d_zs, float* d_agg, const float* d_W, int transW, const float* d_rows2, const float* d_W2,
+                       int len_out, float* d_out, int flags);
+
 int gaib_spmm_gemm_bf16(gaib_ctx* ctx, gaib_graph* g, int weight_kind, const float* d_edge_w, int len_in,
                         const uint16_t* d_in, float* d_agg, const float* d_W, int transW, int len_out, float* d_out,
                         int flags);
diff --git a/include/gnn/aggregator.h b/include/gnn/aggregator.h
--- a/include/gnn/aggregator.h
+++ b/include/gnn/aggregator.h
@@ -7,6 +7,8 @@
  public:
   aggregator() : n(0), length(0), fuse_relu(false) {}
   static bool bf16_tables();
+  static bool zs_tables();
+  static bool zs_paused();
   void set_vlen(int vlen) { length = vlen; }
   void fuse_relu_once() { fuse_relu = true; }
   void release() {}
@@ -14,7 +16,7 @@
  protected:
   void aggregate_then_matmul(int kind, int len, Graph& g, const float* in, float* agg, bool keep_agg,
                              const float* W, bool transW, int len_out, float* out, bool relu,
-                             const float* rows2 = NULL, const float* W2 = NULL);
+                             const float* rows2 = NULL, const float* W2 = NULL, bool relu_masked = false);
 
   int n;
   int length;
@@ -29,7 +31,7 @@
   void aggregate_matmul(int len, Graph& g, const float* in, float* agg, bool keep_agg, const float* W,
                         bool transW, int len_out, float* out, bool relu);
   void d_aggregate_matmul(int len, Graph& g, const float* grad_in, float* agg, bool keep_agg, const float* W,
-                          bool transW, int len_out, float* out);
+                          bool transW, int len_out, float* out, bool relu_masked = false);
 };
 
 class SAGE_Aggregator : public aggregator {
@@ -42,7 +44,7 @@
                         const float* W_self = NULL);
   void d_aggregate_matmul(int len, Graph& g, const float* grad_in, float* agg, bool keep_agg, const float* W,
                           bool transW, int len_out, float* out, const float* rows_self = NULL,
-                          const float* W_self = NULL);
+                          const float* W_self = NULL, bool relu_masked = false);
 };
 
 class GAT_Aggregator : public aggregator {
```

Measured after the change: 13.90 billion edges/s, median of 6. +1.2%, better.
